# ruc98/Distributed-Data-Parallel-ML-Training

Measured on AMD Instinct MI355X. Metric: images/sec (whole node) VGG-11 CIFAR-10, higher is better.
Workload: dtype bf16; 1 GPU; model=vgg11, global_batch=256, per_gpu_batch=256, parallelism=dp1, hipgraph=True, buckets=1, grad_comm=fp32, comm=inline, optimizer=SGD(lr=0.1, momentum=0.9, wd=1e-4) fused

## Files before the change

### distributed-data-parallel-ml-training_amd/_build.py

```python
import concurrent.futures as cf
import glob
import os
import shutil
import subprocess
import sys
import sysconfig

PKG_DIR = os.path.dirname(os.path.abspath(__file__))
REPO = os.path.dirname(PKG_DIR)
CSRC = os.path.join(PKG_DIR, "csrc")
ARCH = os.environ.get("DDP_AMD_ARCH", "gfx950")
ROCM = os.environ.get("ROCM_PATH", "/opt/rocm")


def _hipcc():
    for c in (os.path.join(ROCM, "bin", "hipcc"), shutil.which("hipcc")):
        if c and os.path.exists(c):
            return c
    raise RuntimeError("hipcc not found (ROCm toolchain required to build ddp_amd)")


def _includes():
    import pybind11
    return ["-I" + CSRC, "-I" + os.path.join(CSRC, "kernels"), "-I" + pybind11.get_include(),
            "-I" + sysconfig.get_paths()["include"], "-I" + os.path.join(ROCM, "include")]


VARIANTS = {"release": ("_native", "native", []),
            "det": ("_native_det", "native_det", ["-DDDP_AMD_DETERMINISTIC"])}


def ext_path(variant="release"):
    suffix = sysconfig.get_config_var("EXT_SUFFIX") or ".so"
    return os.path.join(PKG_DIR, VARIANTS[variant][0] + suffix)


def _newest_header():
    hs = glob.glob(os.path.join(CSRC, "**", "*.h"), recursive=True)
    return max((os.path.getmtime(h) for h in hs), default=0.0)


def _deps(obj):
    d = obj + ".d"
    if not os.path.exists(d):
        return None
    with open(d) as f:
        text = f.read().replace("\\\n", " ")
    parts = text.split(":", 1)
    return [t for t in parts[1].split()] if len(parts) == 2 else None


def _compile(cmd, src, obj, hdr_time, verbose):
    if os.path.exists(obj):
        t = os.path.getmtime(obj)
        deps = _deps(obj)
        newest = (max([os.path.getmtime(x) for x in deps if os.path.exists(x)] + [0.0])
                  if deps is not None else hdr_time)
        if deps is not None and any(not os.path.exists(x) for x in deps):
            newest = hdr_time
        if t >= os.path.getmtime(src) and t >= newest:
            return obj, False
    if verbose:
        print("[ddp_amd build]", os.path.relpath(src, PKG_DIR), flush=True)
    r = subprocess.run(cmd, capture_output=True, text=True)
    if r.returncode != 0:
        raise RuntimeError(f"compile failed: {src}\n{r.stdout}\n{r.stderr}")
    return obj, True


def _sources():
    return (sorted(glob.glob(os.path.join(CSRC, "kernels", "*.hip")))
            + sorted(glob.glob(os.path.join(CSRC, "runtime", "*.cpp"))) + [os.path.join(CSRC, "bind.cpp")])


def up_to_date(variant="release"):
    out = ext_path(variant)
    if not os.path.exists(out):
        return False
    newest = max([_newest_header()] + [os.path.getmtime(s) for s in _sources()])
    return os.path.getmtime(out) >= newest


def build(verbose=True, jobs=None, variants=("release", "det")):
    for v in variants:
        _build_variant(v, verbose, jobs)
    return ext_path()


def _build_variant(variant, verbose=True, jobs=None):
    stem, objdir, defines = VARIANTS[variant]
    BUILD = os.path.join(REPO, "build", objdir)
    if not os.path.isdir(BUILD) and up_to_date(variant):
        return ext_path(variant)
    hipcc = _hipcc()
    os.makedirs(BUILD, exist_ok=True)
    inc = _includes()
    debug = os.environ.get("DDP_AMD_DEBUG_BUILD", "0") == "1"
    common = (["-O1", "-g", "-DDDP_AMD_DEBUG"] if debug else ["-O3"]) + \
        ["-std=c++17", "-fPIC", "-Wno-unused-result"] + defines
    hdr_time = _newest_header()
    tasks = []
    for src in sorted(glob.glob(os.path.join(CSRC, "kernels", "*.hip"))):
        obj = os.path.join(BUILD, os.path.basename(src) + ".o")
        cmd = [hipcc, f"--offload-arch={ARCH}", "-x", "hip", *common, *inc, "-c", src, "-o", obj,
               "-MMD", "-MF", obj + ".d"]
        tasks.append((cmd, src, obj))
    host_srcs = sorted(glob.glob(os.path.join(CSRC, "runtime", "*.cpp"))) + [os.path.join(CSRC, "bind.cpp")]
    for src in host_srcs:
        obj = os.path.join(BUILD, os.path.basename(src) + ".o")
        cmd = [hipcc, "-x", "c++", "-D__HIP_PLATFORM_AMD__", *common, "-fvisibility=hidden", *inc,
               "-c", src, "-o", obj, "-MMD", "-MF", obj + ".d"]
        tasks.append((cmd, src, obj))
    jobs = jobs or min(8, os.cpu_count() or 4)
    changed = False
    with cf.ThreadPoolExecutor(max_workers=jobs) as ex:
        futs = [ex.submit(_compile, c, s, o, hdr_time, verbose) for c, s, o in tasks]
        objs = []
        for f in futs:
            o, ch = f.result()
            objs.append(o)
            changed |= ch
    out = ext_path(variant)
    if changed or not os.path.exists(out) or os.path.getmtime(out) < max(os.path.getmtime(o) for o in objs):
        tmp = out + ".tmp"
        cmd = [hipcc, f"--offload-arch={ARCH}", "-shared", "-fPIC", *objs, "-o", tmp,
               "-L" + os.path.join(ROCM, "lib"), "-lrccl", "-lamdhip64"]
        r = subprocess.run(cmd, capture_output=True, text=True)
        if r.returncode != 0:
            raise RuntimeError(f"link failed\n{r.stdout}\n{r.stderr}")
        os.replace(tmp, out)
        if verbose:
            print("[ddp_amd build] linked", os.path.relpath(out, REPO), flush=True)
    return out


if __name__ == "__main__":
    build(verbose=True)
    sys.exit(0)
```

### distributed-data-parallel-ml-training_amd/csrc/bind.cpp

```cpp
#include <hip/hip_runtime.h>
#include <pybind11/pybind11.h>
#include <pybind11/stl.h>

#include <stdexcept>
#include <string>
#include <tuple>
#include <vector>

#include "runtime/comm.h"

namespace py = pybind11;
using ddp_amd::BucketSpec;
using ddp_amd::RcclComm;
using ddp_amd::Reducer;

#include "kernels/api.h"

template <typename T>
static T* P(uintptr_t v) { return reinterpret_cast<T*>(v); }
static hipStream_t S(uintptr_t v) { return reinterpret_cast<hipStream_t>(v); }
static void check(int rc, const char* what) {
  if (rc != 0) {
    std::string msg = std::string(what) + " failed: ";
    msg += (rc > 0) ? hipGetErrorString((hipError_t)rc) : "invalid arguments";
// ... 307 lines not shown
    a.running_mean = P<float>(running_mean); a.running_var = P<float>(running_var);
    a.momentum = momentum; a.use_running = use_running;
    if (rcoef) {
      ddp_amd::BnArgs r{};
      r.C = C; r.eps = reps; r.momentum = rmomentum;
      r.stats = P<float>(rstats); r.gamma = P<float>(rgamma); r.beta = P<float>(rbeta);
      r.coef = P<float>(rcoef);
      r.running_mean = P<float>(rrunning_mean); r.running_var = P<float>(rrunning_var);
      a.rcoef = r.coef;
      check(ddp_bn_act_fwd_res(&a, &r, S(st)), "bn_act_fwd (shortcut BN)");
      return;
    }
    check(ddp_bn_act_fwd(&a, S(st)), "bn_act_fwd");
  }, py::arg("N"), py::arg("H"), py::arg("W"), py::arg("C"), py::arg("pool"), py::arg("relu"),
     py::arg("eps"), py::arg("z"), py::arg("res"), py::arg("stats"), py::arg("gamma"),
     py::arg("beta"), py::arg("out"), py::arg("stream"), py::arg("running_mean") = 0,
     py::arg("running_var") = 0, py::arg("momentum") = 0.1f, py::arg("use_running") = 0,
     py::arg("coef") = 0, py::arg("mask") = 0, py::arg("rstats") = 0, py::arg("rgamma") = 0,
     py::arg("rbeta") = 0, py::arg("rcoef") = 0, py::arg("rrunning_mean") = 0,
     py::arg("rrunning_var") = 0, py::arg("reps") = 1e-5f, py::arg("rmomentum") = 0.1f);
  m.def("maxpool_fwd", [](uintptr_t x, int N, int H, int W, int C, int KH, int KW, int stride,
                          int pad, int Ho, int Wo, uintptr_t y, uintptr_t idx, uintptr_t st) {
    check(ddp_maxpool_fwd(P<void>(x), N, H, W, C, KH, KW, stride, pad, Ho, Wo, P<void>(y),
                          P<void>(idx), S(st)), "maxpool_fwd");
  });
  m.def("maxpool_bwd", [](uintptr_t dy, uintptr_t idx, int N, int H, int W, int C, int KH, int KW,
                          int stride, int pad, int Ho, int Wo, uintptr_t dx, uintptr_t st) {
    check(ddp_maxpool_bwd(P<void>(dy), P<void>(idx), N, H, W, C, KH, KW, stride, pad, Ho, Wo,
                          P<void>(dx), S(st)), "maxpool_bwd");
  });
  m.def("avgpool_fwd", [](uintptr_t x, int N, int HW, int C, uintptr_t y, uintptr_t st) {
    check(ddp_avgpool_fwd(P<void>(x), N, HW, C, P<void>(y), S(st)), "avgpool_fwd");
  });
  m.def("avgpool_bwd", [](uintptr_t dy, int N, int HW, int C, uintptr_t dx, uintptr_t st) {
    check(ddp_avgpool_bwd(P<void>(dy), N, HW, C, P<void>(dx), S(st)), "avgpool_bwd");
  });
  m.def("colsum", [](uintptr_t dl, int B, int J, uintptr_t db, uintptr_t st) {
    check(ddp_colsum(P<void>(dl), B, J, P<float>(db), S(st)), "colsum");
  });
  m.def("bn_act_bwd", [](int N, int H, int W, int C, int pool, int relu, float eps, uintptr_t z,
                         uintptr_t res, uintptr_t stats, uintptr_t gamma, uintptr_t beta,
                         uintptr_t dout, uintptr_t sums, uintptr_t dz, uintptr_t dres,
                         uintptr_t dgamma, uintptr_t dbeta, uintptr_t dbias, uintptr_t st,
                         uintptr_t coef, int sums_ready, uintptr_t mask, uintptr_t rcoef,
                         uintptr_t rsums, uintptr_t rdz, uintptr_t rdgamma, uintptr_t rdbeta) {
    ddp_amd::BnArgs a{};
    a.coef = P<float>(coef);
    a.sums_ready = sums_ready;
    a.mask = P<unsigned char>(mask);
    a.N = N; a.H = H; a.W = W; a.C = C; a.pool = pool; a.relu = relu; a.eps = eps;
    a.z = P<unsigned short>(z); a.res = P<unsigned short>(res); a.stats = P<float>(stats);
    a.gamma = P<float>(gamma); a.beta = P<float>(beta); a.dout = P<unsigned short>(dout);
    a.sums = P<float>(sums); a.dz = P<unsigned short>(dz); a.dres = P<unsigned short>(dres);
    a.dgamma = P<float>(dgamma); a.dbeta = P<float>(dbeta); a.dbias = P<float>(dbias);
    if (rcoef) {
      a.rcoef = P<float>(rcoef); a.rsums = P<float>(rsums); a.rdz = P<unsigned short>(rdz);
      a.rdgamma = P<float>(rdgamma); a.rdbeta = P<float>(rdbeta);
      check(ddp_bn_act_bwd_res(&a, S(st)), "bn_act_bwd (shortcut BN)");
      return;
    }
    check(ddp_bn_act_bwd(&a, S(st)), "bn_act_bwd");
  }, py::arg("N"), py::arg("H"), py::arg("W"), py::arg("C"), py::arg("pool"), py::arg("relu"),
     py::arg("eps"), py::arg("z"), py::arg("res"), py::arg("stats"), py::arg("gamma"),
     py::arg("beta"), py::arg("dout"), py::arg("sums"), py::arg("dz"), py::arg("dres"),
     py::arg("dgamma"), py::arg("dbeta"), py::arg("dbias"), py::arg("stream"), py::arg("coef"),
     py::arg("sums_ready") = 0, py::arg("mask") = 0, py::arg("rcoef") = 0, py::arg("rsums") = 0,
     py::arg("rdz") = 0, py::arg("rdgamma") = 0, py::arg("rdbeta") = 0);
  m.def("bn_pool3_fwd", [](int N, int H, int W, int C, int relu, float eps, uintptr_t z,
                           uintptr_t stats, uintptr_t gamma, uintptr_t beta, uintptr_t out,
                           uintptr_t idx, uintptr_t st, uintptr_t running_mean,
                           uintptr_t running_var, float momentum, int use_running, uintptr_t coef) {
    ddp_amd::BnArgs a{};
    a.N = N; a.H = H; a.W = W; a.C = C; a.relu = relu; a.eps = eps;
    a.z = P<unsigned short>(z); a.stats = P<float>(stats); a.gamma = P<float>(gamma);
    a.beta = P<float>(beta); a.out = P<unsigned short>(out); a.coef = P<float>(coef);
    a.running_mean = P<float>(running_mean); a.running_var = P<float>(running_var);
    a.momentum = momentum; a.use_running = use_running;
    check(ddp_bn_pool3_fwd(&a, P<unsigned char>(idx), S(st)), "bn_pool3_fwd");
  });
  m.def("bn_pool3_bwd", [](int N, int H, int W, int C, int relu, float eps, uintptr_t z,
                           uintptr_t dout, uintptr_t idx, uintptr_t sums, uintptr_t dz,
                           uintptr_t dgamma, uintptr_t dbeta, uintptr_t st, uintptr_t coef) {
    ddp_amd::BnArgs a{};
    a.N = N; a.H = H; a.W = W; a.C = C; a.relu = relu; a.eps = eps;
    a.z = P<unsigned short>(z); a.dout = P<unsigned short>(dout); a.sums = P<float>(sums);
    a.dz = P<unsigned short>(dz); a.dgamma = P<float>(dgamma); a.dbeta = P<float>(dbeta);
    a.coef = P<float>(coef);
    check(ddp_bn_pool3_bwd(&a, P<unsigned char>(idx), S(st)), "bn_pool3_bwd");
  });
  m.def("bn_bwd_local_ok", [](int N, int H, int W, int C, int pool) {
    return ddp_bn_bwd_local_ok(N, H, W, C, pool) != 0;
  });
  m.def("bn_bwd_local_set", [](long long max_loads) { ddp_bn_bwd_local_set(max_loads); });
  m.def("conv_epi_stage_set", [](int on) { ddp_conv_epi_stage_set(on); });

  m.def("linear_ce_fwd", [](uintptr_t x, uintptr_t W, uintptr_t b, uintptr_t labels, int B, int F,
                            int J, uintptr_t logits, uintptr_t dlogits, uintptr_t loss_sum,
                            uintptr_t correct, uintptr_t st, uintptr_t loss_acc) {
    check(ddp_linear_ce_fwd(P<void>(x), P<float>(W), P<float>(b), P<long long>(labels), B, F, J,
                            P<float>(logits), P<float>(dlogits), P<float>(loss_sum),
                            P<int>(correct), P<float>(loss_acc), S(st)), "linear_ce_fwd");
  }, py::arg("x"), py::arg("W"), py::arg("b"), py::arg("labels"), py::arg("B"), py::arg("F"),
     py::arg("J"), py::arg("logits"), py::arg("dlogits"), py::arg("loss_sum"), py::arg("correct"),
     py::arg("stream"), py::arg("loss_acc") = 0);
  m.def("bn_pool_linear_ce_fwd", [](uintptr_t z, uintptr_t stats, uintptr_t gamma, uintptr_t beta,
                                    float eps, int relu, uintptr_t coef, uintptr_t y, uintptr_t W,
                                    uintptr_t b, uintptr_t labels, int B, int F, int J,
                                    uintptr_t dlogits, uintptr_t loss_sum, uintptr_t st,
                                    uintptr_t loss_acc) {
    ddp_amd::HeadBnIn h{P<unsigned short>(z), P<float>(stats), P<float>(gamma), P<float>(beta),
                        eps, relu, P<float>(coef), P<unsigned short>(y)};
    check(ddp_bn_pool_linear_ce_fwd(&h, P<float>(W), P<float>(b), P<long long>(labels), B, F, J,
                                    P<float>(dlogits), P<float>(loss_sum), nullptr,
                                    P<float>(loss_acc), S(st)), "bn_pool_linear_ce_fwd");
  }, py::arg("z"), py::arg("stats"), py::arg("gamma"), py::arg("beta"), py::arg("eps"),
     py::arg("relu"), py::arg("coef"), py::arg("y"), py::arg("W"), py::arg("b"), py::arg("labels"),
     py::arg("B"), py::arg("F"), py::arg("J"), py::arg("dlogits"), py::arg("loss_sum"),
     py::arg("stream"), py::arg("loss_acc") = 0);
  m.def("linear_bwd", [](uintptr_t dlogits, uintptr_t x, uintptr_t W, int B, int F, int J,
                         uintptr_t gscale, uintptr_t dx, uintptr_t dW, uintptr_t db,
                         uintptr_t st) {
    check(ddp_linear_bwd(P<float>(dlogits), P<void>(x), P<float>(W), B, F, J, P<float>(gscale),
                         P<void>(dx), P<float>(dW), P<float>(db), S(st)), "linear_bwd");
  });
  m.def("softmax_ce", [](uintptr_t logits, int bf16, uintptr_t labels, int B, int J,
                         uintptr_t loss_sum, uintptr_t correct, uintptr_t dlogits,
                         int dlogits_bf16, uintptr_t st) {
    check(ddp_softmax_ce(P<void>(logits), bf16, P<long long>(labels), B, J, P<float>(loss_sum),
                         P<int>(correct), P<void>(dlogits), dlogits_bf16, S(st)), "softmax_ce");
  });

  m.def("sgd", [](uintptr_t p, uintptr_t g, uintptr_t buf, size_t n, float lr, float momentum,
                  float wd, float grad_scale, int nesterov, uintptr_t st, uintptr_t sched) {
    check(ddp_sgd(P<float>(p), P<float>(g), P<float>(buf), n, lr, momentum, wd, grad_scale,
                  nesterov, P<const ddp_amd::LrSched>(sched), S(st)), "sgd");
  }, py::arg("p"), py::arg("g"), py::arg("buf"), py::arg("n"), py::arg("lr"), py::arg("momentum"),
     py::arg("wd"), py::arg("grad_scale"), py::arg("nesterov"), py::arg("stream"),
     py::arg("sched") = 0);
  m.def("conv_options", [](int stages) { ddp_conv_options(stages); }, py::arg("stages") = 2);
  m.def("conv_tune_set", [](int mode, int M, int N, int K, int tile, int splits, int stages) {
    ddp_conv_tune_set(mode, M, N, K, tile, splits, stages);
  }, py::arg("mode"), py::arg("M"), py::arg("N"), py::arg("K"), py::arg("tile"),
     py::arg("splits"), py::arg("stages") = 0);
  m.def("conv_tune_clear", []() { ddp_conv_tune_clear(); });
  m.def("conv_wgrad_pm_set", [](int on) { ddp_conv_wgrad_pm_set(on); });
  m.def("conv_rows_pm_set", [](int on) { ddp_conv_rows_pm_set(on); });
  m.def("bn_fold_bwd_mb", [](int mb) { ddp_bn_fold_bwd_mb(mb); });
  m.def("bn_fold_grid", [](int blocks) { ddp_bn_fold_grid(blocks); });
  m.def("conv_pair_tune_set", [](int M, int N, int K, int hw, int tile, int sd, int sw) {
    ddp_conv_pair_tune_set(M, N, K, hw, tile, sd, sw);
  });
  m.def("conv_force_tile", [](int t, int stages) { ddp_conv_force_tile(t, stages); },
        py::arg("tile_plus_one"), py::arg("stages") = 0);
  m.def("pack_conv_weights", [](std::vector<std::tuple<uintptr_t, uintptr_t, uintptr_t, int, int,
                                                       int, int, int, int>> descs, uintptr_t st) {
    std::vector<ddp_amd::PackDesc> d;
    for (auto& t : descs) {
      ddp_amd::PackDesc x;
      x.p = P<float>(std::get<0>(t));
      x.wc = P<unsigned short>(std::get<1>(t));
      x.wt = P<unsigned short>(std::get<2>(t));
      x.K = std::get<3>(t); x.Cr = std::get<4>(t); x.C = std::get<5>(t);
      x.R = std::get<6>(t); x.S = std::get<7>(t);
      x.krsc = std::get<8>(t);
      d.push_back(x);
    }
    check(ddp_pack_conv_weights(d.data(), (int)d.size(), S(st)), "pack_conv_weights");
  });
  m.def("sgd_pack", [](uintptr_t items, int n_items, uintptr_t descs, uintptr_t p, uintptr_t g,
                       uintptr_t buf, float lr, float momentum, float wd, float grad_scale,
                       int nesterov, uintptr_t st, int zero_grad, uintptr_t counter, int delta,
                       uintptr_t skip, uintptr_t shadow, uintptr_t slot, uintptr_t done,
                       uintptr_t signal, uintptr_t sched, int sched_advance, uintptr_t lars_side,
                       uintptr_t lars_tensors, uintptr_t lars_partial, uintptr_t lars_trust,
                       float lars_eta, float lars_eps) {
    check(ddp_sgd_pack(P<void>(items), n_items, P<long long>(descs), P<float>(p), P<float>(g),
                       P<float>(buf), lr, momentum, wd, grad_scale, nesterov, zero_grad,
                       P<int>(counter), delta, P<const unsigned>(skip), P<unsigned short>(shadow),
                       P<float>(slot), P<unsigned>(done), P<unsigned>(signal),
                       P<ddp_amd::LrSched>(sched), sched_advance, P<void>(lars_side),
                       P<void>(lars_tensors), P<void>(lars_partial), P<float>(lars_trust),
                       lars_eta, lars_eps, S(st)),
          "sgd_pack");
  }, py::arg("items"), py::arg("n_items"), py::arg("descs"), py::arg("p"), py::arg("g"),
     py::arg("buf"), py::arg("lr"), py::arg("momentum"), py::arg("wd"), py::arg("grad_scale"),
     py::arg("nesterov"), py::arg("stream"), py::arg("zero_grad") = 0, py::arg("counter") = 0,
     py::arg("delta") = 0, py::arg("skip") = 0, py::arg("shadow") = 0, py::arg("slot") = 0,
     py::arg("done") = 0, py::arg("signal") = 0, py::arg("sched") = 0,
     py::arg("sched_advance") = 0, py::arg("lars_side") = 0, py::arg("lars_tensors") = 0,
     py::arg("lars_partial") = 0, py::arg("lars_trust") = 0, py::arg("lars_eta") = 0.f,
     py::arg("lars_eps") = 0.f);
  m.def("lars_norms", [](uintptr_t items, int n_items, uintptr_t p, uintptr_t g, float grad_scale,
                         uintptr_t partial, uintptr_t st) {
    check(ddp_lars_norms(P<void>(items), n_items, P<float>(p), P<float>(g), grad_scale,
                         P<void>(partial), S(st)), "lars_norms");
  }, py::arg("items"), py::arg("n_items"), py::arg("p"), py::arg("g"), py::arg("grad_scale"),
     py::arg("partial"), py::arg("stream"));
  m.def("shard_tail", [](uintptr_t segs, int n_segs, uintptr_t src, uintptr_t dst,
                         std::vector<std::tuple<uintptr_t, uintptr_t, uintptr_t, int, int, int,
                                                int, int, int>> descs,
                         uintptr_t done, uintptr_t signal, uintptr_t skip, uintptr_t st) {
    std::vector<ddp_amd::PackDesc> d;
    for (auto& t : descs) {
      ddp_amd::PackDesc x;
      x.p = P<float>(std::get<0>(t));
      x.wc = P<unsigned short>(std::get<1>(t));
      x.wt = P<unsigned short>(std::get<2>(t));
      x.K = std::get<3>(t); x.Cr = std::get<4>(t); x.C = std::get<5>(t);
      x.R = std::get<6>(t); x.S = std::get<7>(t);
      x.krsc = std::get<8>(t);
      d.push_back(x);
    }
    check(ddp_shard_tail(P<void>(segs), n_segs, P<float>(src), P<float>(dst), d.data(),
                         (int)d.size(), P<unsigned>(done), P<unsigned>(signal),
                         P<const unsigned>(skip), S(st)), "shard_tail");
  });
  m.def("seg_copy_f32", [](uintptr_t table, int n, uintptr_t src, uintptr_t dst, uintptr_t st) {
    check(ddp_seg_copy_f32(P<void>(table), n, P<float>(src), P<float>(dst), S(st)), "seg_copy_f32");
  });
  m.def("sgd_tile_dims", [](int RS) {
    int tk, tc;
    ddp_sgd_tile_dims(RS, &tk, &tc);
    return std::make_pair(tk, tc);
  });
  m.def("counter_add", [](uintptr_t c, int delta, uintptr_t st, uintptr_t sched, int sched_mode) {
    check(ddp_counter_add(P<int>(c), delta, P<ddp_amd::LrSched>(sched), sched_mode, S(st)),
          "counter_add");
  }, py::arg("c"), py::arg("delta"), py::arg("stream"), py::arg("sched") = 0,
     py::arg("sched_mode") = 0);

  m.def("synth_generate", [](uintptr_t images, uintptr_t labels, int n, int pix_per_img,
                             unsigned int seed, int classes, uintptr_t st) {
    check(ddp_synth_generate(P<unsigned char>(images), P<int>(labels), n, pix_per_img, seed,
                             classes, S(st)), "synth_generate");
  });
  m.def("augment", [](uintptr_t images, uintptr_t labels, uintptr_t indices, uintptr_t cursor,
                      int L, int B, int H, int W, int Cp, int pad, int flip, unsigned int seed,
                      unsigned int epoch, std::vector<float> mean, std::vector<float> std_,
                      uintptr_t x, uintptr_t y, uintptr_t st, uintptr_t zero, size_t zero_n,
                      uintptr_t sched) {
    ddp_amd::AugArgs a{};
    a.sched = P<ddp_amd::LrSched>(sched);
    a.zero = P<float>(zero);
    a.zero_n = zero ? zero_n : 0;
    a.images = P<unsigned char>(images); a.labels = P<int>(labels); a.indices = P<int>(indices);
    a.cursor = P<int>(cursor); a.L = L; a.B = B; a.H = H; a.W = W; a.Cp = Cp; a.pad = pad;
    a.flip = flip; a.seed = seed; a.epoch = epoch;
    for (int c = 0; c < 3; ++c) { a.mean[c] = mean.at(c); a.inv_std[c] = 1.f / std_.at(c); }
    a.x = P<unsigned short>(x); a.y = P<long long>(y);
    check(ddp_augment(&a, S(st)), "augment");
  }, py::arg("images"), py::arg("labels"), py::arg("indices"), py::arg("cursor"), py::arg("L"),
     py::arg("B"), py::arg("H"), py::arg("W"), py::arg("Cp"), py::arg("pad"), py::arg("flip"),
     py::arg("seed"), py::arg("epoch"), py::arg("mean"), py::arg("std"), py::arg("x"),
     py::arg("y"), py::arg("stream"), py::arg("zero") = 0, py::arg("zero_n") = 0,
     py::arg("sched") = 0);
  m.def("nchw_to_nhwc", [](uintptr_t x, int N, int C, int H, int W, int Cp, uintptr_t out,
                           uintptr_t st) {
    check(ddp_nchw_to_nhwc(P<float>(x), N, C, H, W, Cp, P<void>(out), S(st)), "nchw_to_nhwc");
  });
  m.def("mean_ws", [](uintptr_t in, size_t n, int ws, uintptr_t out, uintptr_t st) {
    check(ddp_mean_ws(P<float>(in), n, ws, P<float>(out), S(st)), "mean_ws");
  });
  m.def("comm_standin", [](uintptr_t x, size_t n, int blocks, float usec, float scale, uintptr_t st,
                           int passes) {
    check(ddp_comm_standin(P<float>(x), n, blocks, usec, scale, passes, S(st)), "comm_standin");
  }, py::arg("x"), py::arg("n"), py::arg("blocks"), py::arg("usec"), py::arg("scale"),
     py::arg("stream"), py::arg("passes") = 1);
  m.def("flag_signal", [](uintptr_t flag, uintptr_t st) {
    check(ddp_flag_signal(P<unsigned>(flag), S(st)), "flag_signal");
  });
  m.def("flag_wait", [](uintptr_t flag, uintptr_t expected, uintptr_t err, float timeout_s,
                        uintptr_t st) {
    check(ddp_flag_wait(P<unsigned>(flag), P<unsigned>(expected), P<unsigned>(err), timeout_s,
                        S(st)),
          "flag_wait");
  });
  m.def("pack_bf16", [](uintptr_t x, size_t n, uintptr_t y, uintptr_t st) {
    check(ddp_pack_bf16(P<float>(x), n, P<unsigned short>(y), S(st)), "pack_bf16");
  });
  m.def("unpack_bf16", [](uintptr_t y, size_t n, uintptr_t x, uintptr_t st) {
    check(ddp_unpack_bf16(P<unsigned short>(y), n, P<float>(x), S(st)), "unpack_bf16");
  });
  m.def("memset_async", [](uintptr_t p, int value, size_t n, uintptr_t st) {
    check((int)hipMemsetAsync(P<void>(p), value, n, S(st)), "hipMemsetAsync");
  });
  m.def("memcpy_async", [](uintptr_t dst, uintptr_t src, size_t n, uintptr_t st) {
    check((int)hipMemcpyAsync(P<void>(dst), P<void>(src), n, hipMemcpyDeviceToDevice, S(st)),
          "hipMemcpyAsync");
  });
  m.def("copy_bytes", [](uintptr_t dst, uintptr_t src, size_t n, uintptr_t st) {
    check(ddp_copy_bytes(P<void>(dst), P<void>(src), n, S(st)), "copy_bytes");
  });
  m.def("fill_bytes", [](uintptr_t dst, int value, size_t n, uintptr_t st) {
    check(ddp_fill_bytes(P<void>(dst), value, n, S(st)), "fill_bytes");
  });
  m.def("scale", [](uintptr_t x, size_t n, float s, uintptr_t st) {
    check(ddp_scale(P<float>(x), n, s, S(st)), "scale");
  });

  m.def("plan_buckets", [](std::vector<size_t> offsets, std::vector<size_t> numels,
                           size_t elem_bytes, size_t cap, size_t cap_first) {
    auto b = ddp_amd::plan_buckets(offsets, numels, elem_bytes, cap, cap_first);
    std::vector<std::tuple<int, int, size_t, size_t>> out;
    for (auto& x : b) out.emplace_back(x.first_param, x.last_param, x.offset, x.count);
    return out;
  });
// ... 103 lines not shown
```

### distributed-data-parallel-ml-training_amd/csrc/kernels/api.h

```cpp
#pragma once
#include <hip/hip_runtime.h>
#include <stddef.h>
#include <stdint.h>

namespace ddp_amd {

#ifdef DDP_AMD_DETERMINISTIC
constexpr int kStatRep = 4096;
constexpr bool kDeterministic = true;
#else
constexpr int kStatRep = 16;
constexpr bool kDeterministic = false;
#endif

struct ConvGeom {
  int N, H, W, C;
  int K;
  int R, S, stride, pad;
  int P, Q;
  int Creal;
  int wkrsc;
};

struct BnArgs {
// ... 72 lines not shown
  const float* beta;
  float eps;
  int relu;
  float* coef;
  unsigned short* y;
};

struct LrSched {
  unsigned step;
  unsigned n;
  unsigned next;
  unsigned pad;
};

struct SgdFuse {
  float* p;
  float* buf;
  unsigned short* wc;
  float lr, momentum, wd, grad_scale;
  int nesterov;
  const LrSched* sched;
};

struct L0Io {
  const void* x;
  const void* wc;
  const float* bias;
  float eps;
  int relu;
  float* stats;
  const float* gamma;
  const float* beta;
  float* coef;
  void* y;
  const void* dy;
  float* sums;
  void* dz;
  void* code;
  void* zw;
  float* dgamma;
  float* dbeta;
  int sums_ready;
  float* dw;
  float* ws;
  size_t ws_elems;
};

struct PackDesc {
  const float* p;
  unsigned short* wc;
  unsigned short* wt;
  int K, Cr, C, R, S;
  int krsc;
};

struct AugArgs {
  const unsigned char* images;
  const int* labels;
  const int* indices;
  const int* cursor;
  int L, B, H, W, Cp, pad, flip;
  uint32_t seed, epoch;
  float mean[3], inv_std[3];
  unsigned short* x;
  long long* y;
  float* zero;
  size_t zero_n;
  LrSched* sched;
};

}

extern "C" {
int ddp_conv_fwd(const ddp_amd::ConvGeom* g, const void* x, const void* wc, const float* bias,
                 void* y, float* stats, float* ws, size_t ws_elems, int splits, hipStream_t st);
int ddp_conv_fwd_bn(const ddp_amd::ConvGeom* g, const void* x, const void* wc, const float* bias,
                    void* z, float* stats, float* ws, size_t ws_elems, const ddp_amd::BnFwdFuse* bn,
                    hipStream_t st);
int ddp_conv_fwd_finish(const ddp_amd::ConvGeom* g, float* ws, int splits, const float* bias,
                        void* z, float* stats, const ddp_amd::BnFwdFuse* bn, int* bn_done,
                        hipStream_t st);
int ddp_conv_fwd_tr(const ddp_amd::ConvGeom* g, const void* x, const void* wc, const float* bias,
                    void* z, float* stats, float* ws, size_t ws_elems,
                    const ddp_amd::BnFwdFuse* bn, int* bn_done, const ddp_amd::TrFwdIn* in,
                    hipStream_t st);
int ddp_conv_tr_would_serve(const ddp_amd::ConvGeom* g, size_t ws_elems, int in_mode);
void ddp_conv_tr_set(int mode, int M, int K, int C, int H, int bm, int bn, int splits, int stages);
int ddp_conv_tr_geometry(int BM, int N, int H, int W, int* out7);
int ddp_linear_head_bwd_bn(const float* dl, const float* W, const void* x, int B, int F, int J,
                           const float* gscale, const ddp_amd::BnBwdFuse* bn,
                           const ddp_amd::BnBwdApply* ba, float* dW, float* db, hipStream_t st);
void ddp_conv_bn_fuse_rows(int rows);
int ddp_conv_dgrad(const ddp_amd::ConvGeom* g, const void* dy, const void* wt, void* dx,
                   float* ws, size_t ws_elems, int splits, int accumulate, hipStream_t st);
int ddp_conv_dgrad_acc(const ddp_amd::ConvGeom* g, const void* dy, const void* wt, void* dx,
                       float* ws, size_t ws_elems, int splits, const void* acc_dy,
                       const unsigned char* acc_mask, hipStream_t st);
int ddp_conv_dgrad_bn(const ddp_amd::ConvGeom* g, const void* dy, const void* wt, void* dx,
                      float* ws, size_t ws_elems, int splits, const ddp_amd::BnBwdFuse* bn,
                      const ddp_amd::BnBwdApply* ba, int* bn_done, hipStream_t st);
int ddp_conv_wgrad(const ddp_amd::ConvGeom* g, const void* dy, const void* x, float* dw,
                   float* ws, size_t ws_elems, int splits, hipStream_t st);
int ddp_bn_act_fwd(const ddp_amd::BnArgs* a, hipStream_t st);
int ddp_bn_act_bwd(const ddp_amd::BnArgs* a, hipStream_t st);
int ddp_bn_act_fwd_res(const ddp_amd::BnArgs* a, const ddp_amd::BnArgs* r, hipStream_t st);
int ddp_bn_act_bwd_res(const ddp_amd::BnArgs* a, hipStream_t st);
int ddp_bn_bwd_local_ok(int N, int H, int W, int C, int pool);
void ddp_bn_bwd_local_set(long long max_loads);
int ddp_bn_pool_linear_ce_fwd(const ddp_amd::HeadBnIn* bn, const float* W, const float* b,
                              const long long* labels, int B, int F, int J, float* dlogits,
                              float* loss_sum, int* correct, float* loss_acc, hipStream_t st);
int ddp_linear_ce_fwd(const void* x, const float* W, const float* b, const long long* labels,
                      int B, int F, int J, float* logits, float* dlogits, float* loss_sum,
                      int* correct, float* loss_acc, hipStream_t st);
int ddp_linear_bwd(const float* dlogits, const void* x, const float* W, int B, int F, int J,
                   const float* gscale, void* dx, float* dW, float* db, hipStream_t st);
int ddp_softmax_ce(const void* logits, int logits_bf16, const long long* labels, int B, int J,
                   float* loss_sum, int* correct, void* dlogits, int dlogits_bf16,
                   hipStream_t st);
int ddp_sgd(float* p, const float* g, float* buf, size_t n, float lr, float momentum, float wd,
            float grad_scale, int nesterov, const ddp_amd::LrSched* sched, hipStream_t st);
int ddp_conv_fwd_smallk(const ddp_amd::ConvGeom* g, const void* x, const void* wc,
                        const float* bias, void* y, float* stats, hipStream_t st);
void ddp_conv_options(int stages);
void ddp_conv_epi_stage_set(int on);
int ddp_bn_pool3_fwd(const ddp_amd::BnArgs* a, unsigned char* idx, hipStream_t st);
int ddp_bn_pool3_bwd(const ddp_amd::BnArgs* a, const unsigned char* idx, hipStream_t st);
void ddp_conv_pair_mode(int mode, int items);
void ddp_sgd_fuse_register(float* dw, const ddp_amd::SgdFuse* f, int clear);
void ddp_sgd_fuse_begin();
int ddp_l0_ok(const ddp_amd::ConvGeom* g);
int ddp_l0_fwd(const ddp_amd::ConvGeom* g, const ddp_amd::L0Io* io, hipStream_t st);
int ddp_l0_bwd(const ddp_amd::ConvGeom* g, const ddp_amd::L0Io* io, hipStream_t st);
int ddp_conv_wgrad_final(const ddp_amd::ConvGeom* g, const void* dy, const void* x, float* dw,
                         float* ws, size_t ws_elems, int splits, hipStream_t st);
int ddp_sgd_fuse_taken(uintptr_t* out, int cap);
int ddp_sgd_fuse_take_final(const float* dw, ddp_amd::SgdFuse* out);
int ddp_sgd_fuse_taken_master(uintptr_t* out, int cap);
void ddp_conv_pair_force(int splits_dg, int splits_wg, int tile);
int ddp_conv_bwd_pair(const ddp_amd::ConvGeom* g, const void* dy, const void* wc, void* dx,
                      const void* x, float* dw, float* ws, size_t ws_elems,
                      const ddp_amd::BnBwdFuse* bn, const ddp_amd::BnBwdApply* ba, int* bn_done,
                      hipStream_t st);
void ddp_conv_tune_set(int mode, int M, int N, int K, int tile, int splits, int stages);
void ddp_conv_pair_tune_set(int M, int N, int K, int hw, int tile, int sd, int sw);
void ddp_conv_wgrad_pm_set(int on);
void ddp_conv_rows_pm_set(int on);
void ddp_bn_fold_bwd_mb(int mb);
void ddp_bn_fold_grid(int blocks);
int ddp_conv_dense2x2_ok(const ddp_amd::ConvGeom* g);
void ddp_conv_dense2x2_set(int on);
void ddp_conv_tune_clear();
void ddp_conv_force_tile(int tile_plus_one, int stages);
int ddp_pack_conv_weights(const ddp_amd::PackDesc* descs, int n, hipStream_t st);
int ddp_sgd_pack(const void* items, int n_items, const long long* descs, float* p, float* g,
                 float* buf, float lr, float momentum, float wd, float grad_scale, int nesterov,
                 int zero_grad, int* counter, int delta, const unsigned* skip,
                 unsigned short* shadow, float* slot, unsigned* done, unsigned* signal,
                 ddp_amd::LrSched* sched, int sched_advance, const void* lars_side,
                 const void* lars_tensors, const void* lars_partial, float* lars_trust,
                 float lars_eta, float lars_eps, hipStream_t st);
int ddp_lars_norms(const void* items, int n_items, const float* p, const float* g,
                   float grad_scale, void* partial, hipStream_t st);
int ddp_shard_tail(const void* segs, int n_segs, const float* src, float* dst,
                   const ddp_amd::PackDesc* pack, int n_pack, unsigned* done, unsigned* signal,
                   const unsigned* skip, hipStream_t st);
void ddp_sgd_tile_dims(int RS, int* TK, int* TC);
int ddp_counter_add(int* c, int delta, ddp_amd::LrSched* sched, int sched_mode, hipStream_t st);
int ddp_synth_generate(unsigned char* images, int* labels, int n, int pix_per_img,
                       unsigned int seed, int classes, hipStream_t st);
int ddp_augment(const ddp_amd::AugArgs* a, hipStream_t st);
int ddp_nchw_to_nhwc(const float* x, int N, int C, int H, int W, int Cp, void* out,
                     hipStream_t st);
int ddp_maxpool_fwd(const void* x, int N, int H, int W, int C, int KH, int KW, int stride,
                    int pad, int Ho, int Wo, void* y, void* idx, hipStream_t st);
int ddp_maxpool_bwd(const void* dy, const void* idx, int N, int H, int W, int C, int KH, int KW,
                    int stride, int pad, int Ho, int Wo, void* dx, hipStream_t st);
int ddp_avgpool_fwd(const void* x, int N, int HW, int C, void* y, hipStream_t st);
int ddp_avgpool_bwd(const void* dy, int N, int HW, int C, void* dx, hipStream_t st);
int ddp_colsum(const void* dl, int B, int J, float* db, hipStream_t st);
int ddp_mean_ws(const float* in, size_t n, int ws, float* out, hipStream_t st);
int ddp_scale(float* x, size_t n, float s, hipStream_t st);
int ddp_copy_bytes(void* dst, const void* src, size_t n, hipStream_t st);
int ddp_fill_bytes(void* dst, int value, size_t n, hipStream_t st);
int ddp_comm_standin(float* x, size_t n, int blocks, float usec, float scale, int passes,
                     hipStream_t st);
int ddp_flag_signal(unsigned* flag, hipStream_t st);
int ddp_flag_wait(const unsigned* flag, unsigned* expected, unsigned* err, float timeout_s,
                  hipStream_t st);
int ddp_pack_bf16(const float* x, size_t n, unsigned short* y, hipStream_t st);
int ddp_seg_copy_f32(const void* table, int n, const float* src, float* dst, hipStream_t st);
int ddp_unpack_bf16(const unsigned short* y, size_t n, float* x, hipStream_t st);
}
```

### distributed-data-parallel-ml-training_amd/csrc/kernels/common.h

```cpp
#pragma once
#include <hip/hip_runtime.h>
#include <stdint.h>
#include <cstdlib>

#include "api.h"

namespace ddp_amd {

typedef __bf16 bf16x8 __attribute__((ext_vector_type(8)));
typedef float f32x4 __attribute__((ext_vector_type(4)));
typedef float f32x16 __attribute__((ext_vector_type(16)));
typedef unsigned short u16x8 __attribute__((ext_vector_type(8)));

constexpr int kWave = 64;

#ifdef DDP_AMD_DEBUG
#define DDP_DEVICE_CHECK(cond)                                                              \
  do {                                                                                      \
    if (!(cond)) {                                                                          \
      printf("[ddp_amd debug] %s:%d check failed: %s (block %d thread %d)\n", __FILE__,     \
             __LINE__, #cond, (int)blockIdx.x, (int)threadIdx.x);                           \
      return;                                                                               \
    }                                                                                       \
  } while (0)
#else
#define DDP_DEVICE_CHECK(cond) \
  do {                        \
  } while (0)
#endif

__device__ __forceinline__ int stat_rep(int b) {
#ifdef DDP_AMD_DETERMINISTIC
  return b < kStatRep ? b : 0;
#else
  return b % kStatRep;
#endif
}
__device__ __forceinline__ float stat_val(float v, int b) {
#ifdef DDP_AMD_DETERMINISTIC
  return b < kStatRep ? v : __builtin_nanf("");
#else
  (void)b;
  return v;
#endif
}

__device__ __forceinline__ float sgd_update1(float p, float g, float& b, float lr, float momentum,
                                             float wd, float grad_scale, int nesterov) {
  float d = __builtin_fmaf(wd, p, g * grad_scale);
  if (momentum != 0.f) {
    b = __builtin_fmaf(momentum, b, d);
    d = nesterov ? __builtin_fmaf(momentum, b, d) : b;
  }
  return __builtin_fmaf(-lr, d, p);
}

__device__ __forceinline__ float sched_lr(const LrSched* s) {
  const unsigned k = __hip_atomic_load(&s->step, __ATOMIC_RELAXED, __HIP_MEMORY_SCOPE_AGENT);
  const unsigned n = s->n;
  return reinterpret_cast<const float*>(s + 1)[k < n ? k : n - 1];
}
__device__ __forceinline__ float sched_lr_block(const LrSched* s, float lr) {
  if (!s) return lr;
  __shared__ float s_lr;
  if (threadIdx.x == 0) s_lr = sched_lr(s);
  __syncthreads();
  return s_lr;
}

__device__ __forceinline__ float bf2f(unsigned short h) {
  return __uint_as_float(((unsigned int)h) << 16);
}
__device__ __forceinline__ unsigned short f2bf(float f) {
  __bf16 b = (__bf16)f;
  return __builtin_bit_cast(unsigned short, b);
}
__device__ __forceinline__ float round_bf(float f) { return bf2f(f2bf(f)); }

__device__ __forceinline__ u16x8 ld8(const unsigned short* p) {
  return *reinterpret_cast<const u16x8*>(p);
}
__device__ __forceinline__ void st8(unsigned short* p, u16x8 v) {
  *reinterpret_cast<u16x8*>(p) = v;
}

template <int CTRL>
__device__ __forceinline__ float dpp_f(float v) {
  return __int_as_float(__builtin_amdgcn_update_dpp(0, __float_as_int(v), CTRL, 0xF, 0xF, false));
}
__device__ __forceinline__ float dpp_sum16(float v) {
  v += dpp_f<0xB1>(v);
  v += dpp_f<0x4E>(v);
  v += dpp_f<0x141>(v);
  v += dpp_f<0x140>(v);
  return v;
}
__device__ __forceinline__ float lane_f(float v, int l) {
  return __int_as_float(__builtin_amdgcn_readlane(__float_as_int(v), l));
}
__device__ __forceinline__ float wave_sum(float v) {
  v = dpp_sum16(v);
  return (lane_f(v, 0) + lane_f(v, 16)) + (lane_f(v, 32) + lane_f(v, 48));
}
__device__ __forceinline__ float wave_max(float v) {
  v = fmaxf(v, dpp_f<0xB1>(v));
  v = fmaxf(v, dpp_f<0x4E>(v));
  v = fmaxf(v, dpp_f<0x141>(v));
  v = fmaxf(v, dpp_f<0x140>(v));
  return fmaxf(fmaxf(lane_f(v, 0), lane_f(v, 16)), fmaxf(lane_f(v, 32), lane_f(v, 48)));
}

__device__ __forceinline__ int xcd_remap(int orig, int nwg) {
  const int nx = 8;
  if (nwg < nx) return orig;
  const int q = nwg / nx, r = nwg % nx;
  const int xcd = orig % nx, idx = orig / nx;
  return (xcd < r ? xcd * (q + 1) : r * (q + 1) + (xcd - r) * q) + idx;
}

__host__ __device__ __forceinline__ uint32_t hash_u32(uint32_t x) {
  x ^= x >> 16; x *= 0x7feb352du;
  x ^= x >> 15; x *= 0x846ca68bu;
  x ^= x >> 16;
  return x;
}
__host__ __device__ __forceinline__ uint32_t hash3(uint32_t a, uint32_t b, uint32_t c) {
  return hash_u32(a ^ hash_u32(b ^ hash_u32(c + 0x9e3779b9u)));
}

}
```

### distributed-data-parallel-ml-training_amd/csrc/kernels/conv_igemm.hip

```cpp
#include "common.h"
#include "api.h"
#include "linear_blocks.h"
#include <algorithm>
#include <map>
#include <set>
#include <cstdlib>

namespace ddp_amd {

enum { MODE_FWD = 0, MODE_DGRAD = 1, MODE_WGRAD = 2 };

typedef short v4i16 __attribute__((ext_vector_type(4)));
typedef short short8_t __attribute__((ext_vector_type(8)));
typedef __attribute__((address_space(3))) v4i16 lds_v4i16;

struct FastDiv {
  unsigned mul;
  int sh;
};
__device__ __forceinline__ int fast_div(int x, FastDiv d) {
  return (int)((__umulhi((unsigned)x, d.mul) + (unsigned)x) >> d.sh);
}
__global__ __launch_bounds__(256) void zero16_kernel(uint4* __restrict__ p, size_t n16) {
  for (size_t i = blockIdx.x * 256ull + threadIdx.x; i < n16; i += (size_t)gridDim.x * 256)
    p[i] = (uint4){0u, 0u, 0u, 0u};
}

__device__ __forceinline__ void ld8f_conv(const float* p, float* v) {
  const float4 a = reinterpret_cast<const float4*>(p)[0];
  const float4 b = reinterpret_cast<const float4*>(p)[1];
  v[0] = a.x; v[1] = a.y; v[2] = a.z; v[3] = a.w;
  v[4] = b.x; v[5] = b.y; v[6] = b.z; v[7] = b.w;
}

struct ConvArgs {
  ConvGeom g;
  const unsigned short* a;
  const unsigned short* b;
  unsigned short* out;
  float* dw;
  float* ws;
  const float* bias;
  float* stats;
  int Mg, Ng, Kg;
  int splits;
  int ksteps_per_split;
  int phase;
  int pa, pb, Hp, Wp, r0, s0, Rt, St, qa, qb;
  int accumulate;
  int a_bytes, b_bytes;
  FastDiv dPQ, dQ;
  int has_bnf;
  BnBwdFuse bnf;
  const BnFwdFuse* bnfwd;
  int* bnfwd_done;
  const BnBwdApply* bnapply;
  int* bnapply_done;
  int epi_stage;
  int d2x2;
  int d2C, d2K;
  int no_finish;
  const unsigned short* acc_dy;
  const unsigned char* acc_mask;
  SgdFuse sgd;
  int pixmajor;
};

__device__ __forceinline__ uint2 acc_old4(const unsigned short* dx, const unsigned short* acc_dy,
                                          const unsigned char* acc_mask, size_t e) {
  if (!acc_mask) return *reinterpret_cast<const uint2*>(dx + e);
  uint2 v = *reinterpret_cast<const uint2*>(acc_dy + e);
  const unsigned mb = (unsigned)acc_mask[e >> 3] >> (e & 4);
  v.x &= ((mb & 1u) ? 0xFFFFu : 0u) | ((mb & 2u) ? 0xFFFF0000u : 0u);
  v.y &= ((mb & 4u) ? 0xFFFFu : 0u) | ((mb & 8u) ? 0xFFFF0000u : 0u);
  return v;
}
__device__ __forceinline__ u16x8 acc_old8(const unsigned short* dx, const unsigned short* acc_dy,
                                          const unsigned char* acc_mask, size_t e) {
  if (!acc_mask) return ld8(dx + e);
  u16x8 v = ld8(acc_dy + e);
  const unsigned mb = acc_mask[e >> 3];
#pragma unroll
  for (int i = 0; i < 8; ++i) v[i] = ((mb >> i) & 1u) ? v[i] : (unsigned short)0;
  return v;
}

__device__ __forceinline__ int fdiv(int x, int d, float inv) {
  int q = (int)((float)x * inv);
  const int r = x - q * d;
  q += (r < 0) ? -1 : (r >= d ? 1 : 0);
  return q;
}

struct RowInfo {
  int base;
  int h0, w0;
};

template <int MODE>
__device__ __forceinline__ RowInfo row_info(const ConvArgs& A, int row) {
  const ConvGeom& g = A.g;
  RowInfo ri{0, -(1 << 24), 0};
  if (row >= A.Mg) return ri;
  if (MODE == MODE_FWD) {
    const int pq = g.P * g.Q;
    const int n = fast_div(row, A.dPQ), rem = row - n * pq;
    const int p = fast_div(rem, A.dQ), q = rem - p * g.Q;
    ri.base = n * g.H * g.W * g.C;
    ri.h0 = p * g.stride - g.pad;
    ri.w0 = q * g.stride - g.pad;
  } else if (A.phase) {
    const int hw = A.Hp * A.Wp;
    const int n = fast_div(row, A.dPQ), rem = row - n * hw;
    const int i = fast_div(rem, A.dQ), j = rem - i * A.Wp;
    ri.base = n * g.P * g.Q * g.K;
    ri.h0 = i + A.qa;
    ri.w0 = j + A.qb;
  } else {
    const int hw = g.H * g.W;
    const int n = fast_div(row, A.dPQ), rem = row - n * hw;
    const int h = fast_div(rem, A.dQ), w = rem - h * g.W;
    ri.base = n * g.P * g.Q * g.K;
    ri.h0 = h + g.pad;
    ri.w0 = w + g.pad;
  }
  return ri;
}

struct KInfo {
  int r, s, c;
  bool ok;
};

__device__ __forceinline__ int rk_off(int row, int chunk) {
  return row * 64 + ((chunk ^ ((row >> 1) & 7)) << 3);
}
template <int NCOL>
__device__ __forceinline__ int mc_swz(int m) {
  if (NCOL >= 128) return (((m & 3) | (((m >> 3) & 1) << 2)) << 1) & (NCOL / 8 - 1);
  return ((((m >> 1) & 1) | (((m >> 3) & 1) << 1)) << 1);
}
template <int NCOL>
__device__ __forceinline__ int swz_row_step(int i) {
  return NCOL >= 256 ? ((i & 1) << 3) : 0;
}
template <int NCOL>
__device__ __forceinline__ int mc_off(int m, int col) {
  return m * NCOL + (((col >> 3) ^ mc_swz<NCOL>(m)) << 3) + (col & 7);
}

constexpr unsigned kOOB = 0x80000000u;
__device__ __forceinline__ __amdgpu_buffer_rsrc_t make_rsrc(const void* base, int bytes) {
  return __builtin_amdgcn_make_buffer_rsrc(const_cast<void*>(base), (short)0, bytes, 0x00020000);
}

typedef __attribute__((address_space(3))) void lds_void;

__device__ __forceinline__ void dma_buf(__amdgpu_buffer_rsrc_t rs, int byte_off,
                                        unsigned short* lds_wave_base) {
  __builtin_amdgcn_raw_ptr_buffer_load_lds(rs, (lds_void*)lds_wave_base, 16, byte_off, 0, 0, 0);
}
__device__ __forceinline__ void dma_buf_s(__amdgpu_buffer_rsrc_t rs, int byte_off, int soff,
                                          unsigned short* lds_wave_base) {
  __builtin_amdgcn_raw_ptr_buffer_load_lds(rs, (lds_void*)lds_wave_base, 16, byte_off,
                                           __builtin_amdgcn_readfirstlane(soff), 0, 0);
}

template <int N>
__device__ __forceinline__ void wait_dma_barrier() {
  asm volatile("s_waitcnt vmcnt(%0)\n\ts_barrier" ::"n"(N) : "memory");
}

template <int BM, int BN, int NST>
struct ConvSmem {
  static constexpr int elems = NST * (BM + BN) * 64;
};

template <int MODE, int BM, int BN, int NST, int BNF = 0, bool XSTAT = false, bool SGDM = false>
__device__ __forceinline__ void conv_igemm_body(const ConvArgs& args, unsigned short* smem,
                                                const int bid, const int nblk) {
  constexpr int BK = 64;
  constexpr int WTM = BM / 2, WTN = BN / 2;
  constexpr bool kOldBnf = BNF == 1 || (BNF == 2 && BM == 64 && BN == 64);
  constexpr int TM = WTM / 16, TN = WTN / 16;
  constexpr int CA = BM * BK / 8 / 256;
  constexpr int CB = BN * BK / 8 / 256;
  constexpr int TILE_A = BM * BK, TILE_B = BN * BK;
  constexpr int STAGE = TILE_A + TILE_B;
  static_assert(CA >= 1 && CB >= 1, "tile too small for 256 threads");
  static_assert(NST >= 2 && NST <= 4, "2..4 LDS stages");

  const int tid = threadIdx.x;
  const int lane = tid & 63;
  const int wid = __builtin_amdgcn_readfirstlane(tid >> 6);
  const int wm = wid >> 1, wn = wid & 1;
  DDP_DEVICE_CHECK(blockDim.x == 256 && args.g.C % 8 == 0 && args.g.K % 8 == 0);
  DDP_DEVICE_CHECK(args.splits >= 1 && args.ksteps_per_split >= 1);

  const int tiles_n = (args.Ng + BN - 1) / BN;
  const int tiles_m = (args.Mg + BM - 1) / BM;
  const int tiles = tiles_m * tiles_n;
  const int nitems = tiles * args.splits;
  const int ksteps = (args.Kg + BK - 1) / BK;

  f32x4 acc[TM][TN];
  const ConvGeom& gg = args.g;

  constexpr int NA = (MODE != MODE_WGRAD) ? CA : 1;
  int a_off[CA];
  int a_h0[NA], a_w0[NA];
  int b_off[CB];
  int kr = 0, ks_ = 0, kc = 0;
  KInfo xk;
  int xk_same = 0;
  int wp[CB], wq[CB];
  int w_rr = 0, w_ss = 0, w_lim = 0;
  const bool wsame = MODE == MODE_WGRAD && gg.stride == 1 && gg.P == gg.H && gg.Q == gg.W;
  const int w_dq = wsame ? BK % gg.Q : 0;
  const int w_dp = wsame ? (BK / gg.Q) % gg.P : 0;
  const int w_dm = wsame ? 2 * BK * gg.C : 0;
  const bool pm = MODE == MODE_WGRAD && args.pixmajor;
  const bool pmr = MODE != MODE_WGRAD && args.pixmajor;
  int pmr_pq = 0, pmr_n0 = 0, pmr_row0 = 0, pmr_t = 0;
  unsigned pmr_mask = 0;
  int pm_p = 0, pm_q = 0, pm_qlo = 0, pm_qhi = 0, pm_n0 = 0, pm_r = 0, pm_s = 0;
  int row0 = 0, col0 = 0, zsplit = 0, ks_begin = 0, ks_end = 0, cur_tile = 0;
  int d2pos = 0;
  const bool phase = MODE == MODE_DGRAD && args.phase;
  const int Sdec = phase ? args.St : gg.S;
  const int cdim = MODE == MODE_FWD ? gg.C : gg.K;
  const bool fast = MODE != MODE_WGRAD && (cdim % BK) == 0;
  const int lcA = (MODE != MODE_WGRAD) ? ((tid & 7) ^ ((tid >> 4) & 7))
                                       : ((tid % (BM / 8)) ^ mc_swz<BM>(tid / (BM / 8)));
  constexpr bool BKM = MODE != MODE_FWD;
  const int lcB = !BKM ? lcA : ((tid % (BN / 8)) ^ mc_swz<BN>(tid / (BN / 8)));
  const __amdgpu_buffer_rsrc_t rsA = make_rsrc(args.a, args.a_bytes);
  const __amdgpu_buffer_rsrc_t rsB = make_rsrc(args.b, args.b_bytes);

  auto setup = [&](int item) {
    zsplit = item / tiles;
    const int tile = xcd_remap(item - zsplit * tiles, tiles);
    cur_tile = tile;
    const int tm = tile / tiles_n;
    const int tn = tile - tm * tiles_n;
    row0 = tm * BM;
    col0 = tn * BN;
    ks_begin = zsplit * args.ksteps_per_split;
    ks_end = min(ksteps, ks_begin + args.ksteps_per_split);
    if (MODE != MODE_WGRAD) {
      if (pmr) {
        pmr_pq = row0 / gg.N;
        pmr_n0 = row0 - pmr_pq * gg.N;
        pmr_row0 = row0;
        const int img = MODE == MODE_FWD ? gg.H * gg.W * gg.C : gg.P * gg.Q * gg.K;
#pragma unroll
        for (int i = 0; i < CA; ++i) a_off[i] = 2 * (((tid >> 3) + 32 * i) * img + lcA * 8);
      } else {
#pragma unroll
        for (int i = 0; i < CA; ++i) {
          const RowInfo ri = row_info<MODE>(args, row0 + (tid >> 3) + 32 * i);
          a_h0[i] = ri.h0;
          a_w0[i] = ri.w0;
          const int e = (MODE == MODE_FWD) ? ri.base + (ri.h0 * gg.W + ri.w0) * gg.C
                                           : ri.base + (ri.h0 * gg.Q + ri.w0) * gg.K;
          a_off[i] = 2 * (e + (fast ? lcA * 8 : 0));
        }
      }
      if (MODE == MODE_FWD && args.d2x2) {
        d2pos = col0 / args.d2K;
#pragma unroll
        for (int i = 0; i < CB; ++i) {
          const int col = col0 + (tid >> 3) + 32 * i;
          b_off[i] = col < args.Ng ? 2 * ((col - d2pos * args.d2K) * 9 * args.d2C + lcB * 8)
                                   : (int)kOOB;
        }
      } else if (MODE == MODE_FWD) {
#pragma unroll
        for (int i = 0; i < CB; ++i) {
          const int col = col0 + (tid >> 3) + 32 * i;
          b_off[i] = col < args.Ng ? 2 * (col * args.Kg + lcB * 8) : (int)kOOB;
        }
      } else if (args.d2x2) {
        d2pos = col0 / args.d2C;
#pragma unroll
        for (int i = 0; i < CB; ++i) {
          const int col = col0 + (lcB ^ swz_row_step<BN>(i)) * 8;
          b_off[i] = col < args.Ng ? 2 * (((tid + i * 256) / (BN / 8)) * 9 * args.d2C + col -
                                          d2pos * args.d2C)
                                   : (int)kOOB;
        }
      } else {
#pragma unroll
        for (int i = 0; i < CB; ++i) {
          const int col = col0 + (lcB ^ swz_row_step<BN>(i)) * 8;
          b_off[i] = col < args.Ng ? 2 * (((tid + i * 256) / (BN / 8)) * gg.R * gg.S * gg.C + col)
                                   : (int)kOOB;
        }
      }
      if (pmr) {
        const int pp = pmr_pq / gg.Q, qq = pmr_pq - pp * gg.Q, kb = cdim / BK;
        unsigned m = 0;
        for (int r = 0; r < gg.R; ++r)
          for (int s2 = 0; s2 < gg.S; ++s2) {
            const bool ok = MODE == MODE_FWD
                ? (unsigned)(pp + r - gg.pad) < (unsigned)gg.H && (unsigned)(qq + s2 - gg.pad) < (unsigned)gg.W
                : (unsigned)(pp - r + gg.pad) < (unsigned)gg.P && (unsigned)(qq - s2 + gg.pad) < (unsigned)gg.Q;
            if (ok) m |= 1u << (r * gg.S + s2);
          }
        pmr_mask = m;
        const int V = __builtin_popcount(m) * kb;
        const int per = (V + args.splits - 1) / args.splits;
        ks_begin = min(V, zsplit * per);
        ks_end = min(V, ks_begin + per);
        int jv = ks_begin / kb;
        unsigned mm = m;
        for (; jv > 0 && mm; --jv) mm &= mm - 1;
        pmr_t = mm ? __builtin_ctz(mm) : 0;
        kc = (ks_begin - (ks_begin / kb) * kb) * BK;
        kr = pmr_t / gg.S;
        ks_ = pmr_t - kr * gg.S;
      } else {
        const int kk = ks_begin * BK + (fast ? 0 : lcA * 8);
        const int rs = kk / cdim;
        kc = kk - rs * cdim;
        kr = rs / Sdec;
        ks_ = rs - kr * Sdec;
      }
    } else {
      constexpr int NCA = BM / 8;
#pragma unroll
      for (int i = 0; i < CA; ++i) {
        const int kout = row0 + (lcA ^ swz_row_step<BM>(i)) * 8;
        a_off[i] = kout < args.Mg ? 2 * (((tid + i * 256) / NCA) * gg.K + kout) : (int)kOOB;
      }
      const int j = col0 + lcB * 8;
      const int rs = j / gg.C;
      xk.c = j - rs * gg.C;
      xk.r = rs / gg.S;
      xk.s = rs - xk.r * gg.S;
      xk.ok = j < args.Ng;
      if (pm) {
        const int t = col0 / gg.C;
        pm_r = t / gg.S;
        pm_s = t - pm_r * gg.S;
        const int PQ = gg.P * gg.Q, nb = gg.N / BK;
        const int p_lo = max(0, gg.pad - pm_r), p_hi = min(gg.P, gg.H + gg.pad - pm_r);
        pm_qlo = max(0, gg.pad - pm_s);
        pm_qhi = min(gg.Q, gg.W + gg.pad - pm_s);
        const int nq = max(0, pm_qhi - pm_qlo);
        const int V = max(0, p_hi - p_lo) * nq * nb;
        const int per = (V + args.splits - 1) / args.splits;
        ks_begin = min(V, zsplit * per);
        ks_end = min(V, ks_begin + per);
        const int jv = ks_begin / nb;
        pm_p = p_lo + (nq ? jv / nq : 0);
        pm_q = pm_qlo + (nq ? jv - (jv / nq) * nq : 0);
        pm_n0 = (ks_begin - jv * nb) * BK;
        constexpr int NCA = BM / 8;
        constexpr int NCB = BN / 8;
#pragma unroll
        for (int i = 0; i < CA; ++i) {
          const int kout = row0 + (lcA ^ swz_row_step<BM>(i)) * 8;
          a_off[i] = kout < args.Mg ? 2 * (((tid + i * 256) / NCA) * PQ * gg.K + kout) : (int)kOOB;
        }
#pragma unroll
        for (int i = 0; i < CB; ++i)
          b_off[i] = 2 * (((tid + i * 256) / NCB) * gg.H * gg.W * gg.C + (j - t * gg.C));
      }
      if (!xk.ok) xk.r = -(1 << 20);
      xk_same = xk.ok ? 2 * (((xk.r - gg.pad) * gg.W + (xk.s - gg.pad)) * gg.C + xk.c) : 0;
      if (wsame && !pm) {
        constexpr int NCB = BN / 8;
        const int pq = gg.P * gg.Q;
        w_rr = xk.r - gg.pad;
        w_ss = xk.s - gg.pad;
        w_lim = args.Kg * (2 * gg.C) + xk_same;
#pragma unroll
        for (int i = 0; i < CB; ++i) {
          const int m = ks_begin * BK + (tid + i * 256) / NCB;
          const int rem = m % pq;
          wp[i] = rem / gg.Q;
          wq[i] = rem - wp[i] * gg.Q;
          b_off[i] = m * (2 * gg.C) + xk_same;
        }
      }
    }
  };

  auto issue = [&](int ks, int buf) {
    unsigned short* As = smem + buf * STAGE;
    unsigned short* Bs = As + TILE_A;
    const int k0 = ks * BK;
    if (MODE != MODE_WGRAD && pmr) {
      const int pp = pmr_pq / gg.Q, qq = pmr_pq - pp * gg.Q;
      const int hh = MODE == MODE_FWD ? pp + kr - gg.pad : pp - kr + gg.pad;
      const int ww = MODE == MODE_FWD ? qq + ks_ - gg.pad : qq - ks_ + gg.pad;
      const int sa = MODE == MODE_FWD ? 2 * (((pmr_n0 * gg.H + hh) * gg.W + ww) * cdim + kc)
                                      : 2 * (((pmr_n0 * gg.P + hh) * gg.Q + ww) * cdim + kc);
#pragma unroll
      for (int i = 0; i < CA; ++i) dma_buf_s(rsA, a_off[i], sa, As + (wid * 64 + 256 * i) * 8);
      const int boff = MODE == MODE_FWD ? 2 * (pmr_t * cdim + kc)
                                        : 2 * ((kc * gg.R * gg.S + kr * gg.S + ks_) * gg.C);
#pragma unroll
      for (int i = 0; i < CB; ++i) dma_buf(rsB, b_off[i] + boff, Bs + (wid * 64 + 256 * i) * 8);
      kc += BK;
      if (kc == cdim) {
        kc = 0;
        const unsigned rest = pmr_mask & ~((2u << pmr_t) - 1u);
        pmr_t = rest ? __builtin_ctz(rest) : pmr_t;
        kr = pmr_t / gg.S;
        ks_ = pmr_t - kr * gg.S;
      }
    } else if (MODE != MODE_WGRAD) {
      const int W_ = MODE == MODE_FWD ? gg.W : gg.Q;
      if (fast) {
        const int tap = 2 * (MODE == MODE_FWD ? (kr * W_ + ks_) * cdim + kc : kc - (kr * W_ + ks_) * cdim);
#pragma unroll
        for (int i = 0; i < CA; ++i) {
          bool ok;
          if (MODE == MODE_FWD)
            ok = (unsigned)(a_h0[i] + kr) < (unsigned)gg.H && (unsigned)(a_w0[i] + ks_) < (unsigned)gg.W;
          else
            ok = (unsigned)(a_h0[i] - kr) < (unsigned)gg.P && (unsigned)(a_w0[i] - ks_) < (unsigned)gg.Q;
          dma_buf(rsA, ok ? a_off[i] + tap : (int)kOOB, As + (wid * 64 + 256 * i) * 8);
        }
        int boff;
        if (args.d2x2) {
          const int pix = MODE == MODE_FWD ? kc / args.d2C : kc / args.d2K;
          const int ch = kc - pix * (MODE == MODE_FWD ? args.d2C : args.d2K);
          const int pq = MODE == MODE_FWD ? d2pos : pix, hw = MODE == MODE_FWD ? pix : d2pos;
          const int tap = ((hw >> 1) - (pq >> 1) + 1) * 3 + ((hw & 1) - (pq & 1) + 1);
          boff = MODE == MODE_FWD ? 2 * (tap * args.d2C + ch) : 2 * ((ch * 9 + tap) * args.d2C);
        } else if (MODE == MODE_FWD) {
          boff = 2 * k0;
        } else {
          const int rr = phase ? args.r0 + gg.stride * kr : kr, ss = phase ? args.s0 + gg.stride * ks_ : ks_;
          boff = 2 * ((kc * gg.R * gg.S + rr * gg.S + ss) * gg.C);
        }
#pragma unroll
        for (int i = 0; i < CB; ++i) dma_buf(rsB, b_off[i] + boff, Bs + (wid * 64 + 256 * i) * 8);
        kc += BK;
        if (kc == cdim) {
          kc = 0;
          if (++ks_ == Sdec) { ks_ = 0; ++kr; }
        }
      } else {
        const int kk = k0 + lcA * 8;
        const bool kok = kk < args.Kg;
        const int tap = 2 * (MODE == MODE_FWD ? (kr * W_ + ks_) * cdim + kc : kc - (kr * W_ + ks_) * cdim);
#pragma unroll
        for (int i = 0; i < CA; ++i) {
          bool ok;
          if (MODE == MODE_FWD)
            ok = (unsigned)(a_h0[i] + kr) < (unsigned)gg.H && (unsigned)(a_w0[i] + ks_) < (unsigned)gg.W;
          else
            ok = (unsigned)(a_h0[i] - kr) < (unsigned)gg.P && (unsigned)(a_w0[i] - ks_) < (unsigned)gg.Q;
          dma_buf(rsA, (kok && ok) ? a_off[i] + tap : (int)kOOB, As + (wid * 64 + 256 * i) * 8);
        }
        if (MODE == MODE_FWD) {
#pragma unroll
          for (int i = 0; i < CB; ++i)
            dma_buf(rsB, kok ? b_off[i] + 2 * k0 : (int)kOOB, Bs + (wid * 64 + 256 * i) * 8);
        } else {
          const int RSC = gg.R * gg.S * gg.C;
#pragma unroll
          for (int i = 0; i < CB; ++i) {
            const int m = (tid + i * 256) / (BN / 8);
            const int kkr = k0 + m;
            const int tap = kkr / gg.K, kout = kkr - tap * gg.K;
            const int tr = tap / Sdec, ts = tap - tr * Sdec;
            const int rr = phase ? args.r0 + gg.stride * tr : tr, ss = phase ? args.s0 + gg.stride * ts : ts;
            const int off = b_off[i] - 2 * m * RSC + 2 * ((kout * gg.R * gg.S + rr * gg.S + ss) * gg.C);
            dma_buf(rsB, (kkr < args.Kg && b_off[i] != (int)kOOB) ? off : (int)kOOB,
                    Bs + (wid * 64 + 256 * i) * 8);
          }
        }
        kc += BK;
        while (kc >= cdim) {
          kc -= cdim;
          if (++ks_ == Sdec) { ks_ = 0; ++kr; }
        }
      }
    } else {
      constexpr int NCB = BN / 8;
      if (pm) {
        const int PQ = gg.P * gg.Q;
        const int sa = 2 * ((pm_n0 * PQ + pm_p * gg.Q + pm_q) * gg.K);
        const int sb = 2 * ((pm_n0 * gg.H + pm_p + pm_r - gg.pad) * gg.W + pm_q + pm_s - gg.pad) * gg.C;
#pragma unroll
        for (int i = 0; i < CA; ++i) dma_buf_s(rsA, a_off[i], sa, As + (wid * 64 + 256 * i) * 8);
#pragma unroll
        for (int i = 0; i < CB; ++i) dma_buf_s(rsB, b_off[i], sb, Bs + (wid * 64 + 256 * i) * 8);
        pm_n0 += BK;
        if (pm_n0 == gg.N) {
          pm_n0 = 0;
          if (++pm_q == pm_qhi) {
            pm_q = pm_qlo;
            ++pm_p;
          }
        }
        return;
      }
      const int ka = 2 * k0 * gg.K;
#pragma unroll
      for (int i = 0; i < CA; ++i)
        dma_buf(rsA, a_off[i] + ka, As + (wid * 64 + 256 * i) * 8);
      if (wsame) {
#pragma unroll
        for (int i = 0; i < CB; ++i) {
          const bool ok = b_off[i] < w_lim && (unsigned)(wp[i] + w_rr) < (unsigned)gg.H &&
                          (unsigned)(wq[i] + w_ss) < (unsigned)gg.W;
          dma_buf(rsB, ok ? b_off[i] : (int)kOOB, Bs + (wid * 64 + 256 * i) * 8);
          b_off[i] += w_dm;
          int q = wq[i] + w_dq;
          const int cq = q >= gg.Q ? 1 : 0;
          q -= cq ? gg.Q : 0;
          int pp = wp[i] + w_dp + cq;
          pp -= pp >= gg.P ? gg.P : 0;
          wq[i] = q;
          wp[i] = pp;
        }
      } else {
#pragma unroll
        for (int i = 0; i < CB; ++i) {
          const int m = k0 + (tid + i * 256) / NCB;
          const int n = fast_div(m, args.dPQ);
          const int rem = m - n * (gg.P * gg.Q);
          const int p = fast_div(rem, args.dQ);
          const int q = rem - p * gg.Q;
          const int h = p * gg.stride - gg.pad + xk.r, w = q * gg.stride - gg.pad + xk.s;
          const bool ok = m < args.Kg && (unsigned)h < (unsigned)gg.H && (unsigned)w < (unsigned)gg.W;
          dma_buf(rsB, ok ? 2 * (((n * gg.H + h) * gg.W + w) * gg.C + xk.c) : (int)kOOB,
                  Bs + (wid * 64 + 256 * i) * 8);
        }
      }
    }
  };

  int fa_off[TM], fb_off[TN];
  {
    const int g = lane >> 4, q = (lane >> 2) & 3, p = lane & 3;
    const int m0 = 8 * g + q;
#pragma unroll
    for (int i = 0; i < TM; ++i)
      fa_off[i] = MODE != MODE_WGRAD ? rk_off(wm * WTM + i * 16 + (lane & 15), lane >> 4)
                                     : mc_off<BM>(m0, wm * WTM + i * 16 + 4 * p);
#pragma unroll
    for (int j = 0; j < TN; ++j)
      fb_off[j] = !BKM ? rk_off(wn * WTN + j * 16 + (lane & 15), lane >> 4)
                       : mc_off<BN>(m0, wn * WTN + j * 16 + 4 * p);
  }

  auto load_frags = [&](int buf, int kk, bf16x8 (&fa)[TM], bf16x8 (&fb)[TN]) {
    const unsigned short* As = smem + buf * STAGE;
    const unsigned short* Bs = As + TILE_A;
    if (MODE != MODE_WGRAD) {
#pragma unroll
      for (int i = 0; i < TM; ++i)
        fa[i] = *reinterpret_cast<const bf16x8*>(As + (fa_off[i] ^ (kk ? 32 : 0)));
    } else {
#pragma unroll
      for (int i = 0; i < TM; ++i) {
        const unsigned short* base = As + fa_off[i] + kk * BM;
        v4i16 lo = __builtin_amdgcn_ds_read_tr16_b64_v4i16((lds_v4i16*)base);
        v4i16 hi = __builtin_amdgcn_ds_read_tr16_b64_v4i16((lds_v4i16*)(base + 4 * BM));
        const short8_t v = __builtin_shufflevector(lo, hi, 0, 1, 2, 3, 4, 5, 6, 7);
        fa[i] = __builtin_bit_cast(bf16x8, v);
      }
    }
    if (!BKM) {
#pragma unroll
      for (int j = 0; j < TN; ++j)
        fb[j] = *reinterpret_cast<const bf16x8*>(Bs + (fb_off[j] ^ (kk ? 32 : 0)));
    } else {
#pragma unroll
      for (int j = 0; j < TN; ++j) {
        const unsigned short* base = Bs + fb_off[j] + kk * BN;
        v4i16 lo = __builtin_amdgcn_ds_read_tr16_b64_v4i16((lds_v4i16*)base);
        v4i16 hi = __builtin_amdgcn_ds_read_tr16_b64_v4i16((lds_v4i16*)(base + 4 * BN));
        const short8_t v = __builtin_shufflevector(lo, hi, 0, 1, 2, 3, 4, 5, 6, 7);
        fb[j] = __builtin_bit_cast(bf16x8, v);
      }
    }
  };
  auto mma = [&](const bf16x8 (&fa)[TM], const bf16x8 (&fb)[TN]) {
#pragma unroll
    for (int i = 0; i < TM; ++i)
#pragma unroll
      for (int j = 0; j < TN; ++j)
        acc[i][j] = __builtin_amdgcn_mfma_f32_16x16x32_bf16(fb[j], fa[i], acc[i][j], 0, 0, 0);
  };

  constexpr int SCPR = BN / 8;
  float run_s[XSTAT ? 8 : 1], run_ss[XSTAT ? 8 : 1];
#pragma unroll
  for (int e = 0; e < (XSTAT ? 8 : 1); ++e) { run_s[e] = 0.f; run_ss[e] = 0.f; }
  int run_col = -1;
  auto flush_stats = [&](const int c0, float (&fs)[8], float (&fss)[8]) {
#pragma unroll
    for (int m = SCPR; m < 64; m *= 2)
#pragma unroll
      for (int e = 0; e < 8; ++e) {
        fs[e] += __shfl_xor(fs[e], m);
        fss[e] += __shfl_xor(fss[e], m);
      }
    __syncthreads();
    float* sl = reinterpret_cast<float*>(smem);
    if (lane < SCPR) {
#pragma unroll
      for (int e = 0; e < 8; ++e) {
        sl[(wid * 2 + 0) * BN + lane * 8 + e] = fs[e];
        sl[(wid * 2 + 1) * BN + lane * 8 + e] = fss[e];
      }
    }
    __syncthreads();
    float* st = args.stats + stat_rep(bid) * 2 * args.Ng;
    for (int k = tid; k < 2 * BN; k += 256) {
      const int which = k / BN, cl = k - which * BN;
      if (c0 + cl >= args.Ng) continue;
      const float t = sl[(0 * 2 + which) * BN + cl] + sl[(1 * 2 + which) * BN + cl] +
                      sl[(2 * 2 + which) * BN + cl] + sl[(3 * 2 + which) * BN + cl];
      atomicAdd(st + which * args.Ng + c0 + cl, stat_val(t, bid));
    }
// ... 66 lines not shown
        }
        unsigned short* dst = args.out + orow * args.Ng + col;
        u16x8 o;
        if (MODE == MODE_DGRAD && args.accumulate) {
          const u16x8 old = acc_old8(args.out, args.acc_dy, args.acc_mask, orow * args.Ng + col);
#pragma unroll
          for (int e = 0; e < 8; ++e) o[e] = f2bf(v[e] + bf2f(old[e]));
        } else {
#pragma unroll
          for (int e = 0; e < 8; ++e) o[e] = f2bf(v[e] + bv[e]);
        }
        st8(dst, o);
        if (MODE == MODE_FWD && red) {
#pragma unroll
          for (int e = 0; e < 8; ++e) {
            const float rv = bf2f(o[e]);
            if constexpr (XSTAT) {
              run_s[e] += rv;
              run_ss[e] += rv * rv;
            } else {
              s[e] += rv;
              ss[e] += rv * rv;
            }
          }
        }
      }
    }
    if (!XSTAT && MODE == MODE_FWD && red) flush_stats(col0, s, ss);
    return;
  }
  if (red) __syncthreads();
  if (MODE != MODE_WGRAD && !(BM == 64 && BN == 64) && !split &&
      !(MODE == MODE_DGRAD && args.accumulate) && BNF == 2) {
    const int cbase = col0 + wn * WTN + cq;
    const bool has_bias = MODE == MODE_FWD && args.bias != nullptr;
    int ro[TM];
#pragma unroll
    for (int i = 0; i < TM; ++i) {
      const int row = row0 + wm * WTM + i * 16 + rl;
      int orow = row;
      if (phase) {
        const int hw = args.Hp * args.Wp;
        const int n = fast_div(row, args.dPQ), rem = row - n * hw;
        const int pi = fast_div(rem, args.dQ), pj = rem - pi * args.Wp;
        orow = (n * g.H + args.pa + g.stride * pi) * g.W + args.pb + g.stride * pj;
      } else if (pmr) {
        orow = (pmr_n0 + row - pmr_row0) * (g.P * g.Q) + pmr_pq;
      }
      ro[i] = row < args.Mg ? orow * args.Ng + cbase : -1;
    }
    float* sl = reinterpret_cast<float*>(smem);
#pragma unroll
    for (int j = 0; j < TN; ++j) {
      if (cbase + j * 16 >= args.Ng) continue;
      float4 bj = {0.f, 0.f, 0.f, 0.f};
      if (has_bias) bj = *reinterpret_cast<const float4*>(args.bias + cbase + j * 16);
      float s[4] = {0.f, 0.f, 0.f, 0.f}, ss[4] = {0.f, 0.f, 0.f, 0.f};
      float4 bsc = {0.f, 0.f, 0.f, 0.f}, bsh = bsc, bmu = bsc, bis = bsc;
      if (MODE == MODE_DGRAD && BNF == 2 && red) {
        const float* cf = args.bnf.coef + cbase + j * 16;
        bsc = *reinterpret_cast<const float4*>(cf + 0 * args.Ng);
        bsh = *reinterpret_cast<const float4*>(cf + 1 * args.Ng);
        bmu = *reinterpret_cast<const float4*>(cf + 2 * args.Ng);
        bis = *reinterpret_cast<const float4*>(cf + 3 * args.Ng);
      }
#pragma unroll
      for (int i = 0; i < TM; ++i) {
        if (ro[i] < 0) continue;
        const f32x4 v = acc[i][j];
        uint2 pk;
        pk.x = (unsigned)f2bf(v[0] + bj.x) | ((unsigned)f2bf(v[1] + bj.y) << 16);
        pk.y = (unsigned)f2bf(v[2] + bj.z) | ((unsigned)f2bf(v[3] + bj.w) << 16);
        *reinterpret_cast<uint2*>(args.out + ro[i] + j * 16) = pk;
        if (MODE == MODE_FWD && red) {
          const float r0 = __uint_as_float(pk.x << 16), r1 = __uint_as_float(pk.x & 0xffff0000u);
          const float r2 = __uint_as_float(pk.y << 16), r3 = __uint_as_float(pk.y & 0xffff0000u);
          s[0] += r0; s[1] += r1; s[2] += r2; s[3] += r3;
          ss[0] += r0 * r0; ss[1] += r1 * r1; ss[2] += r2 * r2; ss[3] += r3 * r3;
        }
        if (MODE == MODE_DGRAD && BNF == 2 && red) {
          const uint2 zz = *reinterpret_cast<const uint2*>(args.bnf.z + ro[i] + j * 16);
          const float gv[4] = {__uint_as_float(pk.x << 16), __uint_as_float(pk.x & 0xffff0000u),
                               __uint_as_float(pk.y << 16), __uint_as_float(pk.y & 0xffff0000u)};
          const float zf[4] = {__uint_as_float(zz.x << 16), __uint_as_float(zz.x & 0xffff0000u),
                               __uint_as_float(zz.y << 16), __uint_as_float(zz.y & 0xffff0000u)};
          const float fsc[4] = {bsc.x, bsc.y, bsc.z, bsc.w}, fsh[4] = {bsh.x, bsh.y, bsh.z, bsh.w};
          const float fmu[4] = {bmu.x, bmu.y, bmu.z, bmu.w}, fis[4] = {bis.x, bis.y, bis.z, bis.w};
#pragma unroll
          for (int t = 0; t < 4; ++t) {
            const float y = zf[t] * fsc[t] + fsh[t];
            const float dyb = (args.bnf.relu && !(y > 0.f)) ? 0.f : gv[t];
            s[t] += dyb;
            ss[t] += dyb * ((zf[t] - fmu[t]) * fis[t]);
          }
        }
      }
      if (red) {
#pragma unroll
        for (int t = 0; t < 4; ++t) {
          s[t] = dpp_sum16(s[t]);
          ss[t] = dpp_sum16(ss[t]);
        }
        float* slot = sl + ((((wm * 2 + wn) * TN + j) * 4 + (lane >> 4)) * 8);
        if (rl == 0) {
#pragma unroll
          for (int t = 0; t < 4; ++t) {
            slot[t] = s[t];
            slot[4 + t] = ss[t];
          }
        }
      }
    }
    if (red) {
      __syncthreads();
      if (wm == 0 && rl == 0) {
        float* st = (MODE == MODE_FWD ? args.stats : args.bnf.sums) +
                    stat_rep(bid) * 2 * args.Ng;
#pragma unroll
        for (int j = 0; j < TN; ++j) {
          const int col = cbase + j * 16;
          if (col >= args.Ng) continue;
          const float* s0 = sl + (((wn * TN + j) * 4 + (lane >> 4)) * 8);
          const float* s1 = sl + ((((2 + wn) * TN + j) * 4 + (lane >> 4)) * 8);
#pragma unroll
          for (int t = 0; t < 4; ++t) {
            atomicAdd(st + col + t, stat_val(s0[t] + s1[t], bid));
            atomicAdd(st + args.Ng + col + t, stat_val(s0[4 + t] + s1[4 + t], bid));
          }
        }
      }
    }
    return;
  }
  float sgd_lr = 0.f;
  if (SGDM && MODE == MODE_WGRAD) sgd_lr = args.sgd.sched ? sched_lr(args.sgd.sched) : args.sgd.lr;
#pragma unroll
  for (int j = 0; j < TN; ++j) {
    const int col = col0 + wn * WTN + j * 16 + cq;
    const bool cok = col < args.Ng;
    float4 bias = {0.f, 0.f, 0.f, 0.f};
    if (MODE == MODE_FWD && !split && args.bias && cok)
      bias = (float4){args.bias[col], args.bias[col + 1], args.bias[col + 2], args.bias[col + 3]};
    float s[4] = {0.f, 0.f, 0.f, 0.f}, ss[4] = {0.f, 0.f, 0.f, 0.f};
    float4 bsc = {0.f, 0.f, 0.f, 0.f}, bsh = bsc, bmu = bsc, bis = bsc;
    if (MODE == MODE_DGRAD && kOldBnf && red && cok) {
      const float* cf = args.bnf.coef;
      bsc = *reinterpret_cast<const float4*>(cf + 0 * args.Ng + col);
      bsh = *reinterpret_cast<const float4*>(cf + 1 * args.Ng + col);
      bmu = *reinterpret_cast<const float4*>(cf + 2 * args.Ng + col);
      bis = *reinterpret_cast<const float4*>(cf + 3 * args.Ng + col);
    }
    int wrs = 0, wc = 0;
    if (MODE == MODE_WGRAD) {
      wrs = col / g.C;
      wc = col - wrs * g.C;
    }
#pragma unroll
    for (int i = 0; i < TM; ++i) {
      const int row = row0 + wm * WTM + i * 16 + rl;
      if (!cok || row >= args.Mg) continue;
      const f32x4 v = acc[i][j];
      if (MODE == MODE_WGRAD && !split) {
        if (SGDM && g.wkrsc && g.Creal == g.C && args.sgd.p) {
          const size_t e = ((size_t)row * g.R * g.S + wrs) * g.C + wc;
          float4 pv = *reinterpret_cast<const float4*>(args.sgd.p + e);
          float4 bv = *reinterpret_cast<const float4*>(args.sgd.buf + e);
          const SgdFuse& h = args.sgd;
          pv.x = sgd_update1(pv.x, v[0], bv.x, sgd_lr, h.momentum, h.wd, h.grad_scale, h.nesterov);
          pv.y = sgd_update1(pv.y, v[1], bv.y, sgd_lr, h.momentum, h.wd, h.grad_scale, h.nesterov);
          pv.z = sgd_update1(pv.z, v[2], bv.z, sgd_lr, h.momentum, h.wd, h.grad_scale, h.nesterov);
          pv.w = sgd_update1(pv.w, v[3], bv.w, sgd_lr, h.momentum, h.wd, h.grad_scale, h.nesterov);
          *reinterpret_cast<float4*>(args.sgd.p + e) = pv;
          *reinterpret_cast<float4*>(args.sgd.buf + e) = bv;
        } else if (g.wkrsc && g.Creal == g.C) {
          float* d = args.dw + ((size_t)row * g.R * g.S + wrs) * g.C + wc;
          float4 o = *reinterpret_cast<float4*>(d);
          o.x += v[0]; o.y += v[1]; o.z += v[2]; o.w += v[3];
          *reinterpret_cast<float4*>(d) = o;
        } else {
#pragma unroll
          for (int t = 0; t < 4; ++t) {
            if (wc + t >= g.Creal) break;
            const size_t di = g.wkrsc ? ((size_t)row * g.R * g.S + wrs) * g.Creal + wc + t
                                      : ((size_t)row * g.Creal + wc + t) * g.R * g.S + wrs;
            args.dw[di] += v[t];
          }
        }
      } else if (split) {
        const size_t srow = pmr ? (size_t)(pmr_n0 + row - pmr_row0) * (g.P * g.Q) + pmr_pq : (size_t)row;
        *reinterpret_cast<float4*>(slab + srow * args.Ng + col) = (float4){v[0], v[1], v[2], v[3]};
      } else {
        const unsigned short h0 = f2bf(v[0] + bias.x), h1 = f2bf(v[1] + bias.y);
        const unsigned short h2 = f2bf(v[2] + bias.z), h3 = f2bf(v[3] + bias.w);
        uint2 pk;
        pk.x = (unsigned)h0 | ((unsigned)h1 << 16);
        pk.y = (unsigned)h2 | ((unsigned)h3 << 16);
        size_t orow = row;
        if (phase) {
          const int hw = args.Hp * args.Wp;
          const int n = fast_div(row, args.dPQ), rem = row - n * hw;
          const int i = fast_div(rem, args.dQ), j = rem - i * args.Wp;
          orow = ((size_t)n * gg.H + args.pa + gg.stride * i) * gg.W + args.pb + gg.stride * j;
        } else if (pmr) {
          orow = (size_t)(pmr_n0 + row - pmr_row0) * (gg.P * gg.Q) + pmr_pq;
        }
        if (MODE == MODE_DGRAD && args.accumulate) {
          uint2* dst = reinterpret_cast<uint2*>(args.out + orow * args.Ng + col);
          const uint2 old = acc_old4(args.out, args.acc_dy, args.acc_mask, orow * args.Ng + col);
          pk.x = (unsigned)f2bf(v[0] + bf2f((unsigned short)(old.x & 0xffff))) |
                 ((unsigned)f2bf(v[1] + bf2f((unsigned short)(old.x >> 16))) << 16);
          pk.y = (unsigned)f2bf(v[2] + bf2f((unsigned short)(old.y & 0xffff))) |
                 ((unsigned)f2bf(v[3] + bf2f((unsigned short)(old.y >> 16))) << 16);
          *dst = pk;
        } else {
          *reinterpret_cast<uint2*>(args.out + orow * args.Ng + col) = pk;
        }
        if (MODE == MODE_FWD) {
          const float r0 = bf2f(h0), r1 = bf2f(h1), r2 = bf2f(h2), r3 = bf2f(h3);
          s[0] += r0; s[1] += r1; s[2] += r2; s[3] += r3;
          ss[0] += r0 * r0; ss[1] += r1 * r1; ss[2] += r2 * r2; ss[3] += r3 * r3;
        }
        if (MODE == MODE_DGRAD && kOldBnf && red) {
          const float gv[4] = {bf2f(h0), bf2f(h1), bf2f(h2), bf2f(h3)};
          const float fsc[4] = {bsc.x, bsc.y, bsc.z, bsc.w}, fsh[4] = {bsh.x, bsh.y, bsh.z, bsh.w};
          const float fmu[4] = {bmu.x, bmu.y, bmu.z, bmu.w}, fis[4] = {bis.x, bis.y, bis.z, bis.w};
          const BnBwdFuse& f = args.bnf;
          const int hw = g.H * g.W;
          const int n = fast_div((int)orow, args.dPQ), rem = (int)orow - n * hw;
          const int h = fast_div(rem, args.dQ), w = rem - h * g.W;
          const int np = f.pool ? 4 : 1;
          float zf[4][4];
#pragma unroll
          for (int d = 0; d < 4; ++d) {
            if (d >= np) break;
            const int zh = f.pool ? 2 * h + (d >> 1) : h, zw = f.pool ? 2 * w + (d & 1) : w;
            const uint2 zz = *reinterpret_cast<const uint2*>(
                f.z + (((size_t)n * f.Hz + zh) * f.Wz + zw) * args.Ng + col);
            zf[d][0] = bf2f((unsigned short)(zz.x & 0xffff));
            zf[d][1] = bf2f((unsigned short)(zz.x >> 16));
            zf[d][2] = bf2f((unsigned short)(zz.y & 0xffff));
            zf[d][3] = bf2f((unsigned short)(zz.y >> 16));
          }
#pragma unroll
          for (int t = 0; t < 4; ++t) {
            float best = -INFINITY, yarg = 0.f, zarg = 0.f;
#pragma unroll
            for (int d = 0; d < 4; ++d) {
              if (d >= np) break;
              const float y = zf[d][t] * fsc[t] + fsh[t];
              const float yr = f.relu ? fmaxf(y, 0.f) : y;
              if (d == 0 || yr > best || yr != yr) { best = yr; yarg = y; zarg = zf[d][t]; }
            }
            const float dyb = (f.relu && !(yarg > 0.f)) ? 0.f : gv[t];
            s[t] += dyb;
            ss[t] += dyb * ((zarg - fmu[t]) * fis[t]);
          }
        }
      }
    }
    if (red) {
#pragma unroll
      for (int t = 0; t < 4; ++t) {
        s[t] = dpp_sum16(s[t]);
        ss[t] = dpp_sum16(ss[t]);
      }
      float* slot = reinterpret_cast<float*>(smem) + (((wn * TN + j) * 4 + (lane >> 4)) * 8);
      if (wm == 1 && rl == 0) {
#pragma unroll
        for (int t = 0; t < 4; ++t) {
          slot[t] = s[t];
          slot[4 + t] = ss[t];
        }
      }
      stat_s[j][0] = s[0]; stat_s[j][1] = s[1]; stat_s[j][2] = s[2]; stat_s[j][3] = s[3];
      stat_ss[j][0] = ss[0]; stat_ss[j][1] = ss[1]; stat_ss[j][2] = ss[2]; stat_ss[j][3] = ss[3];
    }
  }
  if (red) {
    __syncthreads();
    if (wm == 0 && rl == 0) {
      float* st = (MODE == MODE_FWD ? args.stats : args.bnf.sums) +
                  stat_rep(bid) * 2 * args.Ng;
#pragma unroll
      for (int j = 0; j < TN; ++j) {
        const int col = col0 + wn * WTN + j * 16 + cq;
        if (col >= args.Ng) continue;
        const float* slot = reinterpret_cast<const float*>(smem) + (((wn * TN + j) * 4 + (lane >> 4)) * 8);
#pragma unroll
        for (int t = 0; t < 4; ++t) {
          atomicAdd(st + col + t, stat_val(stat_s[j][t] + slot[t], bid));
          atomicAdd(st + args.Ng + col + t, stat_val(stat_ss[j][t] + slot[4 + t], bid));
        }
      }
    }
  }
  };

  constexpr int DMA = CA + CB;
  for (int item = bid; item < nitems; item += nblk) {
    setup(item);
#pragma unroll
    for (int i = 0; i < TM; ++i)
#pragma unroll
      for (int j = 0; j < TN; ++j) acc[i][j] = (f32x4){0.f, 0.f, 0.f, 0.f};
    const int kb = ks_begin, ke = ks_end;
#pragma unroll
    for (int s = 0; s < NST - 1; ++s)
      if (kb + s < ke) issue(kb + s, s);
    int stage = 0;
    for (int ks = kb; ks < ke; ++ks) {
      const int ahead = ke - 1 - ks;
      if (NST >= 4 && ahead >= 2) wait_dma_barrier<(NST >= 4 ? 2 : 0) * DMA>();
      else if (NST >= 3 && ahead >= 1) wait_dma_barrier<(NST >= 3 ? 1 : 0) * DMA>();
      else wait_dma_barrier<0>();
      bf16x8 fa0[TM], fb0[TN], fa1[TM], fb1[TN];
      load_frags(stage, 0, fa0, fb0);
      if (ks + NST - 1 < ke) issue(ks + NST - 1, stage == 0 ? NST - 1 : stage - 1);
      load_frags(stage, 32, fa1, fb1);
      mma(fa0, fb0);
      mma(fa1, fb1);
      stage = stage + 1 == NST ? 0 : stage + 1;
    }
    epilogue(row0, col0, zsplit, args.splits > 1);
    if (item + nblk < nitems) wait_dma_barrier<0>();
  }
  if constexpr (XSTAT) {
    if (MODE == MODE_FWD && run_col >= 0)
      flush_stats(run_col, *reinterpret_cast<float(*)[8]>(run_s),
                  *reinterpret_cast<float(*)[8]>(run_ss));
  }
}

#ifndef DDP_CONV_WAVES_PER_EU
#define DDP_CONV_WAVES_PER_EU 2
#endif
template <int MODE, int BM, int BN, int NST, int BNF = 0, bool XSTAT = false>
__global__ __launch_bounds__(256) __attribute__((amdgpu_waves_per_eu(DDP_CONV_WAVES_PER_EU)))
void conv_igemm_kernel(ConvArgs args) {
  extern __shared__ __attribute__((aligned(16))) unsigned short smem[];
  conv_igemm_body<MODE, BM, BN, NST, BNF, XSTAT>(args, smem, blockIdx.x, gridDim.x);
}

template <int MODE, int BM, int BN, int NST>
__global__ __launch_bounds__(256) __attribute__((amdgpu_waves_per_eu(2)))
void conv_igemm_bnf2_kernel(ConvArgs args) {
  extern __shared__ __attribute__((aligned(16))) unsigned short smem[];
  conv_igemm_body<MODE, BM, BN, NST, 2>(args, smem, blockIdx.x, gridDim.x);
}

template <int BM, int BN, int NST, int BNF, bool SGDM = false>
__global__ __launch_bounds__(256) void conv_bwd_pair_kernel(ConvArgs dg, ConvArgs wg, int n_dg) {
  __shared__ __attribute__((aligned(16))) unsigned short smem[ConvSmem<BM, BN, NST>::elems];
  if ((int)blockIdx.x < n_dg)
    conv_igemm_body<MODE_DGRAD, BM, BN, NST, BNF>(dg, smem, blockIdx.x, n_dg);
  else
    conv_igemm_body<MODE_WGRAD, BM, BN, NST, 0, false, SGDM>(wg, smem, blockIdx.x - n_dg,
                                                           gridDim.x - n_dg);
}
struct RowMap {
  int stride, Hp, Wp, H, W, pa, pb;
};

__device__ __forceinline__ size_t map_row(const RowMap& m, int row) {
  if (m.stride == 0) return row;
  const int hw = m.Hp * m.Wp;
  const int n = row / hw, rem = row - n * hw;
  const int i = rem / m.Wp, j = rem - i * m.Wp;
  return ((size_t)n * m.H + m.pa + m.stride * i) * m.W + m.pb + m.stride * j;
}

constexpr int kSlabBatch = 8;
__device__ __forceinline__ void sum_slabs8(const float* p, size_t slab, int z0, int z1, float* v) {
  for (int zb = z0; zb < z1; zb += kSlabBatch) {
    float4 a[kSlabBatch], b[kSlabBatch];
#pragma unroll
    for (int u = 0; u < kSlabBatch; ++u) {
      if (zb + u < z1) {
        const float4* src = reinterpret_cast<const float4*>(p + (size_t)(zb + u) * slab);
        a[u] = src[0];
        b[u] = src[1];
      }
    }
#pragma unroll
    for (int u = 0; u < kSlabBatch; ++u) {
      if (zb + u < z1) {
        v[0] += a[u].x; v[1] += a[u].y; v[2] += a[u].z; v[3] += a[u].w;
        v[4] += b[u].x; v[5] += b[u].y; v[6] += b[u].z; v[7] += b[u].w;
      }
    }
  }
}

struct FinishArgs {
  const float* ws;
  int splits;
  unsigned short* out;
  const float* bias;
  float* stats;
  int Mg, Ng;
  RowMap rmap;
  int accumulate;
  BnBwdFuse bnf;
  int H, W;
  const unsigned short* acc_dy;
  const unsigned char* acc_mask;
};

template <bool BNF>
__device__ __forceinline__ void splitk_finish_body(const FinishArgs& fa, float* red_, int bx,
                                                   int by, int gx) {
  const float* ws = fa.ws;
  const int splits = fa.splits, Mg = fa.Mg, Ng = fa.Ng, accumulate = fa.accumulate;
  const int H = fa.H, W = fa.W;
  unsigned short* out = fa.out;
  const float* bias = fa.bias;
  float* stats = fa.stats;
  const RowMap rmap = fa.rmap;
  const BnBwdFuse& bnf = fa.bnf;
  float (*red)[8][256] = reinterpret_cast<float (*)[8][256]>(red_);
  constexpr bool has_bnf = BNF;
  const int G = Ng / 8;
  const int Gb = G < 256 ? G : 256;
  const int cgl = threadIdx.x % Gb, prow = threadIdx.x / Gb, prows = 256 / Gb;
  const int cg = by * Gb + cgl;
  const bool active = prow < prows && cg < G;
  const size_t slab = (size_t)Mg * Ng;
  float s[8], ss[8], bv[8];
  float fsc[8], fsh[8], fmu[8], fis[8];
#pragma unroll
  for (int e = 0; e < 8; ++e) {
    s[e] = 0.f;
    ss[e] = 0.f;
    bv[e] = (bias && cg < G) ? bias[cg * 8 + e] : 0.f;
    fsc[e] = fsh[e] = fmu[e] = fis[e] = 0.f;
  }
  if (has_bnf && cg < G) {
#pragma unroll
    for (int e = 0; e < 8; ++e) {
      fsc[e] = bnf.coef[0 * Ng + cg * 8 + e];
      fsh[e] = bnf.coef[1 * Ng + cg * 8 + e];
      fmu[e] = bnf.coef[2 * Ng + cg * 8 + e];
      fis[e] = bnf.coef[3 * Ng + cg * 8 + e];
    }
    stats = bnf.sums;
  }
  for (int row = bx * prows + prow; active && row < Mg; row += gx * prows) {
    float v[8];
#pragma unroll
    for (int e = 0; e < 8; ++e) v[e] = bv[e];
    sum_slabs8(ws + (size_t)row * Ng + cg * 8, slab, 0, splits, v);
    unsigned short* dst = out + map_row(rmap, row) * Ng + cg * 8;
    if (accumulate) {
      const u16x8 old = acc_old8(out, fa.acc_dy, fa.acc_mask, map_row(rmap, row) * Ng + cg * 8);
#pragma unroll
      for (int e = 0; e < 8; ++e) v[e] += bf2f(old[e]);
    }
    u16x8 o;
#pragma unroll
    for (int e = 0; e < 8; ++e) {
      o[e] = f2bf(v[e]);
      const float r = bf2f(o[e]);
      if (!has_bnf) {
        s[e] += r;
        ss[e] += r * r;
      }
    }
    st8(dst, o);
    if (has_bnf && bnf.code) {
      const int c0 = cg * 8;
      const unsigned* cw = bnf.code + (size_t)row * 16 + ((c0 & 15) >> 2) * 4 + (c0 >> 4);
      const unsigned w0 = cw[0], w1 = cw[4];
      const u16x8 zz = ld8(bnf.z + (size_t)row * Ng + c0);
#pragma unroll
      for (int e = 0; e < 8; ++e) {
        const unsigned code = ((e < 4 ? w0 : w1) >> (8 * (e & 3))) & 0xFFu;
        const float d = code < 4u ? bf2f(o[e]) : 0.f;
// ... 380 lines not shown
                                                              int ndx, int nfx) {
  if ((int)blockIdx.x < ndx) {
    linear_dx_bnbwd_body<RPT>(dl, Wt, B, F, J, gscale, bn, ba, blockIdx.x);
  } else {
    const int t = blockIdx.x - ndx;
    linear_dw_block(dl, x, B, F, J, gscale, dW, db, t % nfx, t / nfx);
  }
}

constexpr int kWgFinishGroup = kDeterministic ? (1 << 30) : 32;
__global__ __launch_bounds__(256) void wgrad_finish_kernel(const float* ws, int splits, int K,
                                                           int R, int S, int C, int Creal,
                                                           float* dw) {
  extern __shared__ __attribute__((aligned(16))) float row[];
  const int k = blockIdx.x;
  const int RS = R * S, RSC = RS * C;
  const size_t slab = (size_t)K * RSC;
  const int z0 = blockIdx.y * kWgFinishGroup, z1 = min(splits, z0 + kWgFinishGroup);
  for (int j = threadIdx.x; j < RSC; j += blockDim.x) {
    float v = 0.f;
    for (int z = z0; z < z1; ++z) v += ws[z * slab + (size_t)k * RSC + j];
    row[j] = v;
  }
  __syncthreads();
  float* out = dw + (size_t)k * Creal * RS;
  const bool single = gridDim.y == 1;
  for (int c = threadIdx.x; c < Creal; c += blockDim.x) {
    for (int rs = 0; rs < RS; ++rs) {
      const float v = row[rs * C + c];
      if (single) out[c * RS + rs] += v;
      else atomicAdd(out + c * RS + rs, v);
    }
  }
}

__device__ __forceinline__ float sgd_step1(float p, float g, float& b, const SgdFuse& h,
                                           float lr) {
  return sgd_update1(p, g, b, lr, h.momentum, h.wd, h.grad_scale, h.nesterov);
}

constexpr int kWgFinishGroupKrsc = kDeterministic ? (1 << 30) : 16;
__device__ __forceinline__ void wgrad_finish_krsc_body(const float* __restrict__ ws, int splits,
                                                       int K, int RS, int C, int Creal,
                                                       float* __restrict__ dw, int bx, int by,
                                                       int gx, int gy, const SgdFuse& sg) {
  const size_t slab = (size_t)K * RS * C;
  const size_t n4 = slab / 4;
  const int z0 = by * kWgFinishGroupKrsc, z1 = min(splits, z0 + kWgFinishGroupKrsc);
  const bool single = gy == 1;
  const bool opt = single && sg.p != nullptr;
  const float lr = opt ? sched_lr_block(sg.sched, sg.lr) : sg.lr;
  for (size_t i = bx * (size_t)blockDim.x + threadIdx.x; i < n4;
       i += (size_t)gx * blockDim.x) {
    float4 v = reinterpret_cast<const float4*>(ws + z0 * slab)[i];
    for (int zb = z0 + 1; zb < z1; zb += kSlabBatch) {
      float4 a[kSlabBatch];
#pragma unroll
      for (int u = 0; u < kSlabBatch; ++u)
        if (zb + u < z1) a[u] = reinterpret_cast<const float4*>(ws + (size_t)(zb + u) * slab)[i];
#pragma unroll
      for (int u = 0; u < kSlabBatch; ++u)
        if (zb + u < z1) { v.x += a[u].x; v.y += a[u].y; v.z += a[u].z; v.w += a[u].w; }
    }
    const float vv[4] = {v.x, v.y, v.z, v.w};
    if (opt) {
      if (Creal == C) {
        float4 pv = reinterpret_cast<float4*>(sg.p)[i];
        float4 bv = reinterpret_cast<float4*>(sg.buf)[i];
        pv.x = sgd_step1(pv.x, v.x, bv.x, sg, lr);
        pv.y = sgd_step1(pv.y, v.y, bv.y, sg, lr);
        pv.z = sgd_step1(pv.z, v.z, bv.z, sg, lr);
        pv.w = sgd_step1(pv.w, v.w, bv.w, sg, lr);
        reinterpret_cast<float4*>(sg.p)[i] = pv;
        reinterpret_cast<float4*>(sg.buf)[i] = bv;
        uint2 pk;
        pk.x = (unsigned)f2bf(pv.x) | ((unsigned)f2bf(pv.y) << 16);
        pk.y = (unsigned)f2bf(pv.z) | ((unsigned)f2bf(pv.w) << 16);
        *reinterpret_cast<uint2*>(sg.wc + i * 4) = pk;
      } else {
        const size_t e = i * 4;
        const int c = (int)(e % C);
        const size_t krs = e / C;
#pragma unroll
        for (int t = 0; t < 4; ++t) {
          if (c + t >= Creal) continue;
          const size_t mi = krs * Creal + c + t;
          float b = sg.buf[mi];
          const float np = sgd_step1(sg.p[mi], vv[t], b, sg, lr);
          sg.p[mi] = np;
          sg.buf[mi] = b;
          sg.wc[e + t] = f2bf(np);
        }
      }
      continue;
    }
    if (Creal == C) {
      if (single) {
        float4* o = reinterpret_cast<float4*>(dw) + i;
        float4 d = *o;
        d.x += v.x; d.y += v.y; d.z += v.z; d.w += v.w;
        *o = d;
      } else {
#pragma unroll
        for (int t = 0; t < 4; ++t) unsafeAtomicAdd(dw + i * 4 + t, vv[t]);
      }
    } else {
      const size_t e = i * 4;
      const int c = (int)(e % C);
      const size_t krs = e / C;
#pragma unroll
      for (int t = 0; t < 4; ++t) {
        if (c + t >= Creal) continue;
        if (single) dw[krs * Creal + c + t] += vv[t];
        else unsafeAtomicAdd(dw + krs * Creal + c + t, vv[t]);
      }
    }
  }
}

__global__ __launch_bounds__(256) void wgrad_finish_krsc_kernel(const float* __restrict__ ws,
                                                                int splits, int K, int RS, int C,
                                                                int Creal, float* __restrict__ dw,
                                                                SgdFuse sg) {
  wgrad_finish_krsc_body(ws, splits, K, RS, C, Creal, dw, blockIdx.x, blockIdx.y, gridDim.x,
                         gridDim.y, sg);
}

struct WgFinishArgs {
  const float* ws;
  int splits, K, RS, C, Creal;
  float* dw;
  int gx, gy;
  SgdFuse sgd;
};

template <bool BNF>
__global__ __launch_bounds__(256) void bwd_pair_finish_kernel(FinishArgs fa, int dgx, int dgy,
                                                              WgFinishArgs wa) {
  __shared__ float red[2 * 8 * 256];
  const int b = blockIdx.x;
  if (b < dgx * dgy) {
    splitk_finish_body<BNF>(fa, red, b % dgx, b / dgx, dgx);
  } else {
    const int w = b - dgx * dgy;
    wgrad_finish_krsc_body(wa.ws, wa.splits, wa.K, wa.RS, wa.C, wa.Creal, wa.dw, w % wa.gx,
                           w / wa.gx, wa.gx, wa.gy, wa.sgd);
  }
}

}

using namespace ddp_amd;

static FastDiv make_fastdiv(int d) {
  FastDiv f;
  int sh = 0;
  while ((1ll << sh) < d) ++sh;
  f.sh = sh;
  f.mul = (unsigned)((((1ull << sh) - (unsigned long long)d) << 32) / (unsigned long long)d + 1);
  return f;
}

static bool fits_buffer(size_t elems) { return elems * 2 < (size_t)kOOB; }

static int g_stages = 2;
constexpr int kNumCUs = 256;
static int g_epi_stage = 1;
static bool epi_stage_enabled() { return g_epi_stage != 0; }
extern "C" void ddp_conv_epi_stage_set(int on) { g_epi_stage = on ? 1 : 0; }

static int pick_splits(int tiles, int ksteps, size_t slab, const ConvArgs& a, size_t ws_elems) {
  if (a.splits > 0) return std::max(1, std::min(a.splits, ksteps));

  if (a.ws == nullptr) return 1;
  int s = (512 + tiles - 1) / tiles;
  s = std::max(1, std::min(s, ksteps / 4));
  s = (int)std::min<size_t>((size_t)s, std::max<size_t>(1, ws_elems / slab));
  return s;
}

static double tile_cost(int BM, int BN, const ConvArgs& a, size_t ws_elems, int* splits_out) {
  const int tiles = ((a.Mg + BM - 1) / BM) * ((a.Ng + BN - 1) / BN);
  const int ksteps = (a.Kg + 63) / 64;
  const size_t slab = (size_t)a.Mg * a.Ng;
  const int splits = pick_splits(tiles, ksteps, slab, a, ws_elems);
  *splits_out = splits;
  const double eff = (BM == 128 && BN == 128) ? 1.0 : ((BM == 64 && BN == 64) ? 0.55 : 0.8);
  const int resident = (BM == 128 && BN == 128) ? 2 : ((BM == 64 && BN == 64) ? 4 : 3);
  const double blocks = (double)tiles * splits;
  const double fill = std::min(1.0, blocks / (256.0 * resident));
  const double work = (double)tiles * BM * BN * ksteps * 64.0;
  const double t_mfma = work / (eff * fill) / 1.0e15 * 2.0;
  double t_split = 0.0;
  if (splits > 1) t_split = 8.0 * splits * (double)slab / 4.0e12 + 3.0e-6;
  return t_mfma + t_split;
}

static int stages_for(int BM, int BN) {
  if (g_stages <= 2) return 2;
  if (BM == 128 && BN == 128) return g_stages >= 4 ? 4 : 2;
  if (BM == 64 && BN == 64) return g_stages >= 4 ? 4 : 3;
  return 3;
}

static int fwd_stat_grid() {
  constexpr int g = 2048;
  return (kDeterministic ? std::min(g, kStatRep) : g) / 8 * 8;
}

template <int MODE, int BM, int BN, int NST, int BNF>
static void launch_gemm_t(const ConvArgs& a, int items, hipStream_t st) {
  constexpr int kStageBytes = (BM + BN) * 64 * 2;
  constexpr int kTileBytes = BM * BN * 2;
  const int stages = std::max(1, std::min(NST, a.ksteps_per_split));
  size_t lds = (size_t)stages * kStageBytes;
  if (a.epi_stage && lds < (size_t)kTileBytes) lds = kTileBytes;
  int grid = items;
  if (MODE == MODE_FWD && a.stats && a.splits <= 1 && a.epi_stage && !(BM == 64 && BN == 64) &&
      fwd_stat_grid() > 0 && items > fwd_stat_grid())
    grid = fwd_stat_grid();
  void (*kern)(ConvArgs);
  if constexpr (BNF == 2 && MODE == MODE_DGRAD) kern = conv_igemm_bnf2_kernel<MODE, BM, BN, NST>;
  else if constexpr (MODE == MODE_FWD && BNF == 0 && !(BM == 64 && BN == 64))
    kern = grid < items ? conv_igemm_kernel<MODE, BM, BN, NST, 0, true>
                        : conv_igemm_kernel<MODE, BM, BN, NST, 0, false>;
  else kern = conv_igemm_kernel<MODE, BM, BN, NST, BNF>;
  static bool attr[2] = {false, false};
  if (!attr[grid < items]) {
    (void)hipFuncSetAttribute(reinterpret_cast<const void*>(kern),
                              hipFuncAttributeMaxDynamicSharedMemorySize,
                              std::max(NST * kStageBytes, kTileBytes));
    attr[grid < items] = true;
  }
  hipLaunchKernelGGL(kern, dim3(grid), dim3(256), lds, st, a);
}

template <int MODE, int BM, int BN, int NST>
static void launch_gemm(const ConvArgs& a, int items, hipStream_t st) {
  if constexpr (MODE == MODE_DGRAD) {
    if (a.has_bnf && a.splits <= 1)
      return a.bnf.pool ? launch_gemm_t<MODE, BM, BN, NST, 1>(a, items, st)
                        : launch_gemm_t<MODE, BM, BN, NST, 2>(a, items, st);
  }
  launch_gemm_t<MODE, BM, BN, NST, 0>(a, items, st);
}

static int g_wgrad_pm = 1, g_rows_pm = 1;
extern "C" void ddp_conv_wgrad_pm_set(int mode) { g_wgrad_pm = std::max(0, std::min(2, mode)); }
extern "C" void ddp_conv_rows_pm_set(int mode) { g_rows_pm = std::max(0, std::min(4, mode)); }
template <int MODE>
static bool rows_pixmajor_ok(const ConvArgs& a, int BM) {
  const ConvGeom& g = a.g;
  const int cdim = MODE == MODE_FWD ? g.C : g.K;
  const bool any_pq = g_rows_pm == 2 || g_rows_pm == 4;
  if (g_rows_pm >= 3 && g.R * g.S == 1) return false;
  return g_rows_pm && !a.d2x2 && !a.phase && !a.accumulate && g.stride == 1 && g.P == g.H &&
         g.Q == g.W && cdim % 64 == 0 && g.N % BM == 0 && (any_pq || g.P * g.Q <= 64) &&
         g.R * g.S <= 32 && g.Creal == g.C && a.Mg == g.N * g.P * g.Q;
}
static bool wgrad_pixmajor_ok(const ConvArgs& a, int BN) {
  const ConvGeom& g = a.g;
  return g_wgrad_pm && g.stride == 1 && g.P == g.H && g.Q == g.W && g.N % 64 == 0 &&
         (g_wgrad_pm == 2 || g.P * g.Q <= 64) && g.C % BN == 0 && g.Creal == g.C && a.Ng == g.R * g.S * g.C &&
         a.Kg == g.N * g.P * g.Q;
}

template <int MODE, int BM, int BN>
static int prepare_cfg(ConvArgs& a, int splits) {
  constexpr int BK = 64;
  const int tiles = ((a.Mg + BM - 1) / BM) * ((a.Ng + BN - 1) / BN);
  const int ksteps = (a.Kg + BK - 1) / BK;
  const int per = (ksteps + splits - 1) / splits;
  splits = (ksteps + per - 1) / per;
  a.splits = splits;
  a.ksteps_per_split = per;
  a.epi_stage = MODE != MODE_WGRAD && epi_stage_enabled();
  a.pixmajor = MODE == MODE_WGRAD ? wgrad_pixmajor_ok(a, BN) : rows_pixmajor_ok<MODE>(a, BM);
  if (MODE == MODE_DGRAD) {
    const int hh = a.phase ? a.Hp : a.g.H, ww = a.phase ? a.Wp : a.g.W;
    a.dPQ = make_fastdiv(std::max(1, hh * ww));
    a.dQ = make_fastdiv(std::max(1, ww));
  } else {
    a.dPQ = make_fastdiv(std::max(1, a.g.P * a.g.Q));
    a.dQ = make_fastdiv(std::max(1, a.g.Q));
  }
  return tiles * splits;
}

static bool needs_finish(int mode, const ConvArgs& a) {
  (void)mode;
  return a.splits > 1;
}

static int finish_rows_per_thread(int Mg, int rows_per_block) {
  return (Mg + rows_per_block - 1) / rows_per_block <= 128 ? 1 : 2;
}

static void dg_finish_grid(const ConvArgs& a, int* bx_out, int* chunks_out) {
  const int G = a.Ng / 8;
  const int Gb = G < 256 ? G : 256;
  const int chunks = (G + Gb - 1) / Gb;
  const int rows_per_block = std::max(1, 256 / Gb);
  const int rpt = finish_rows_per_thread(a.Mg, rows_per_block);
  int bx = (a.Mg + rows_per_block * rpt - 1) / (rows_per_block * rpt);
  *bx_out = std::max(1, std::min(bx, 2048 / chunks + 1));
  *chunks_out = chunks;
}

static FinishArgs finish_args(int mode, const ConvArgs& a) {
  RowMap rm{0, 0, 0, 0, 0, 0, 0};
  if (a.phase) rm = RowMap{a.g.stride, a.Hp, a.Wp, a.g.H, a.g.W, a.pa, a.pb};
  const bool fwd = mode == MODE_FWD;
  return FinishArgs{a.ws, a.splits, a.out, fwd ? a.bias : nullptr, fwd ? a.stats : nullptr,
                    a.Mg, a.Ng, rm, a.accumulate, a.bnf, a.g.H, a.g.W, a.acc_dy, a.acc_mask};
}

static std::map<const float*, SgdFuse> g_sgd_reg;
static std::set<const float*> g_sgd_taken;
static std::set<const float*> g_sgd_master;
static SgdFuse sgd_fuse_master(const float* dw) {
  if (g_sgd_reg.empty()) return SgdFuse{};
  auto it = g_sgd_reg.find(dw);
  if (it == g_sgd_reg.end()) return SgdFuse{};
  g_sgd_master.insert(dw);
  return it->second;
}
static bool g_sgd_allow = false;
static SgdFuse sgd_fuse_for(const float* dw, int groups) {
  if (!g_sgd_allow || groups != 1 || g_sgd_reg.empty()) return SgdFuse{};
  auto it = g_sgd_reg.find(dw);
  if (it == g_sgd_reg.end()) return SgdFuse{};
  g_sgd_taken.insert(dw);
  return it->second;
}

static WgFinishArgs wg_finish_args(const ConvArgs& a) {
  const size_t n4 = (size_t)a.Mg * a.Ng / 4;
  const int groups = (a.splits + kWgFinishGroupKrsc - 1) / kWgFinishGroupKrsc;
  const int bx = (int)std::min<size_t>((n4 + 255) / 256, std::max(1, 2048 / groups));
  return WgFinishArgs{a.ws, a.splits, a.g.K, a.g.R * a.g.S, a.g.C, a.g.Creal, a.dw, bx, groups,
                      sgd_fuse_for(a.dw, groups)};
}

static int g_bn_fuse_rows = 128;
static int bn_fuse_max_rows() { return g_bn_fuse_rows; }
static int bn_bwd_fuse_max_rows() { return bn_fuse_max_rows(); }

static bool bnbwd_fusable(const ConvArgs& a) {
  return a.has_bnf && a.bnapply && a.splits > 1 && !a.phase && !a.accumulate &&
         a.Mg <= bn_bwd_fuse_max_rows() && a.Mg <= kBnBwdFuseMaxRows && a.Ng % 16 == 0 &&
         a.g.stride == 1 &&
         (!a.bnf.pool || (a.bnf.Hz == 2 * a.g.H && a.bnf.Wz == 2 * a.g.W)) &&
         (a.bnf.pool || (a.bnf.Hz == a.g.H && a.bnf.Wz == a.g.W));
}

template <int RPT, bool POOL>
__global__ __launch_bounds__(256) void bwd_pair_finish_bnbwd_kernel(FinishArgs fa, BnBwdApply ba,
                                                                    int dgx, WgFinishArgs wa) {
  __shared__ float wred[4][2][8];
  const int b = blockIdx.x;
  if (b < dgx) {
    finish_bnbwd_body<RPT, POOL>(fa, ba, wred, b);
  } else {
    const int w = b - dgx;
    wgrad_finish_krsc_body(wa.ws, wa.splits, wa.K, wa.RS, wa.C, wa.Creal, wa.dw, w % wa.gx,
                           w / wa.gx, wa.gx, wa.gy, wa.sgd);
  }
}

template <int RPT, bool POOL>
static void launch_bnbwd_t(const FinishArgs& fa, const BnBwdApply& ba, int dgx,
                           const WgFinishArgs* wa, hipStream_t st) {
  if (wa)
    hipLaunchKernelGGL((bwd_pair_finish_bnbwd_kernel<RPT, POOL>), dim3(dgx + wa->gx * wa->gy),
                       dim3(256), 0, st, fa, ba, dgx, *wa);
  else
    hipLaunchKernelGGL((splitk_finish_bnbwd_kernel<RPT, POOL>), dim3(dgx), dim3(256), 0, st, fa, ba);
}

static bool launch_finish_bnbwd(const ConvArgs& a, hipStream_t st, const WgFinishArgs* wa) {
  if (!bnbwd_fusable(a)) return false;
  const FinishArgs fa = finish_args(MODE_DGRAD, a);
  const BnBwdApply& ba = *a.bnapply;
  const int dgx = a.Ng / 16, rpt = (a.Mg + 127) / 128;
  if (a.bnf.pool) {
    if (rpt <= 1) launch_bnbwd_t<1, true>(fa, ba, dgx, wa, st);
    else if (rpt <= 2) launch_bnbwd_t<2, true>(fa, ba, dgx, wa, st);
    else launch_bnbwd_t<4, true>(fa, ba, dgx, wa, st);
  } else {
    if (rpt <= 1) launch_bnbwd_t<1, false>(fa, ba, dgx, wa, st);
    else if (rpt <= 2) launch_bnbwd_t<2, false>(fa, ba, dgx, wa, st);
    else launch_bnbwd_t<4, false>(fa, ba, dgx, wa, st);
  }
  if (a.bnapply_done) *a.bnapply_done = 1;
  return true;
}

static bool launch_finish_bnfwd(const ConvArgs& a, hipStream_t st) {
  const BnFwdFuse& bf = *a.bnfwd;
  if (a.Mg > kBnFwdFuseMaxRows || a.Mg > bn_fuse_max_rows() || a.Ng % 16 || a.accumulate ||
      a.phase)
    return false;
  if (bf.P * bf.Q <= 0 || a.Mg % (bf.P * bf.Q)) return false;
  if (bf.pool && (bf.P % 2 || bf.Q % 2)) return false;
  const FinishArgs fa = finish_args(MODE_FWD, a);
  const dim3 grid(a.Ng / 16);
  const size_t lds = bf.pool ? (size_t)a.Mg * 16 * sizeof(float) : 0;
  static const bool attr = [] {
    (void)hipFuncSetAttribute(reinterpret_cast<const void*>(splitk_finish_bnfwd_kernel<8>),
                              hipFuncAttributeMaxDynamicSharedMemorySize,
                              kBnFwdFuseMaxRows * 16 * sizeof(float));
    return true;
  }();
  (void)attr;
  const int rpt = (a.Mg + 127) / 128;
  if (rpt <= 1) hipLaunchKernelGGL(splitk_finish_bnfwd_kernel<1>, grid, dim3(256), lds, st, fa, bf);
  else if (rpt <= 2) hipLaunchKernelGGL(splitk_finish_bnfwd_kernel<2>, grid, dim3(256), lds, st, fa, bf);
  else if (rpt <= 4) hipLaunchKernelGGL(splitk_finish_bnfwd_kernel<4>, grid, dim3(256), lds, st, fa, bf);
  else hipLaunchKernelGGL(splitk_finish_bnfwd_kernel<8>, grid, dim3(256), lds, st, fa, bf);
  if (a.bnfwd_done) *a.bnfwd_done = 1;
  return true;
}

template <int MODE>
static void launch_finish(const ConvArgs& a, hipStream_t st) {
  if (!needs_finish(MODE, a)) return;
  if (MODE == MODE_WGRAD && a.g.wkrsc) {
    const WgFinishArgs w = wg_finish_args(a);
    hipLaunchKernelGGL(wgrad_finish_krsc_kernel, dim3(w.gx, w.gy), dim3(256), 0, st, a.ws,
                       a.splits, a.g.K, a.g.R * a.g.S, a.g.C, a.g.Creal, a.dw, w.sgd);
  } else if (MODE == MODE_WGRAD) {
    const int groups = (a.splits + kWgFinishGroup - 1) / kWgFinishGroup;
    const size_t lds = sizeof(float) * a.g.R * a.g.S * a.g.C;
    hipLaunchKernelGGL(wgrad_finish_kernel, dim3(a.g.K, groups), dim3(256), lds, st, a.ws,
                       a.splits, a.g.K, a.g.R, a.g.S, a.g.C, a.g.Creal, a.dw);
  } else {
    if (MODE == MODE_FWD && a.bnfwd && launch_finish_bnfwd(a, st)) return;
    if (MODE == MODE_DGRAD && a.has_bnf && a.bnapply && launch_finish_bnbwd(a, st, nullptr)) return;
    int bx, chunks;
    dg_finish_grid(a, &bx, &chunks);
    const FinishArgs fa = finish_args(MODE, a);
    if (MODE == MODE_DGRAD && a.has_bnf)
      hipLaunchKernelGGL(splitk_finish_kernel<true>, dim3(bx, chunks), dim3(256), 0, st, fa);
    else
      hipLaunchKernelGGL(splitk_finish_kernel<false>, dim3(bx, chunks), dim3(256), 0, st, fa);
  }
}

template <int MODE, int BM, int BN>
static void launch_cfg(ConvArgs& a, int splits, hipStream_t st, int nst_req = 0) {
  const int items = prepare_cfg<MODE, BM, BN>(a, splits);
  constexpr int kStageBytes = (BM + BN) * 64 * 2;
  constexpr int kMaxStages = kStageBytes * 4 <= 163840 ? 4 : (kStageBytes * 3 <= 163840 ? 3 : 2);
  int nst = nst_req >= 2 && nst_req <= 4 ? nst_req : stages_for(BM, BN);
  nst = std::min(nst, kMaxStages);
  if constexpr (kMaxStages >= 4) {
    if (nst == 4) { launch_gemm<MODE, BM, BN, 4>(a, items, st); goto launched; }
  }
  if constexpr (kMaxStages >= 3) {
    if (nst == 3) { launch_gemm<MODE, BM, BN, 3>(a, items, st); goto launched; }
  }
  launch_gemm<MODE, BM, BN, 2>(a, items, st);
launched:
  if (!a.no_finish) launch_finish<MODE>(a, st);
}

struct TuneKey {
  int mode, M, N, K;
  int hw = 0;
  bool operator<(const TuneKey& o) const {
    if (mode != o.mode) return mode < o.mode;
    if (M != o.M) return M < o.M;
    if (N != o.N) return N < o.N;
    if (K != o.K) return K < o.K;
    return hw < o.hw;
  }
};
struct TuneVal {
  int tile, splits, stages;
};
static std::map<TuneKey, TuneVal> g_tuned;
static std::map<TuneKey, TuneVal> g_pair_tuned;
static int g_pair_force_dg = 0, g_pair_force_wg = 0;
static int g_force_tile = 0;
static int g_force_stages = 0;

constexpr int kNumTiles = 8;

template <int MODE>
static bool tile_ok(int tile) {
  if (MODE == MODE_WGRAD && (tile == 5 || tile == 7)) return false;
  return tile >= 0 && tile < kNumTiles;
}

template <int MODE>
static void plan_mode(ConvArgs& a, size_t ws_elems, int* best_out, int* sp, int* nst_out) {
  const double c[4] = {tile_cost(128, 128, a, ws_elems, &sp[0]), tile_cost(128, 64, a, ws_elems, &sp[1]),
                       tile_cost(64, 128, a, ws_elems, &sp[2]), tile_cost(64, 64, a, ws_elems, &sp[3])};
  int best = 0, nst = g_force_stages;
  for (int i = 1; i < 4; ++i)
    if (c[i] < c[best]) best = i;
  if (g_force_tile >= 1 && g_force_tile <= kNumTiles && tile_ok<MODE>(g_force_tile - 1)) {
    best = g_force_tile - 1;
    if (best >= 4) {
      static const int bmn[4][2] = {{256, 64}, {64, 256}, {256, 128}, {128, 256}};
      tile_cost(bmn[best - 4][0], bmn[best - 4][1], a, ws_elems, &sp[best]);
    }
  } else if (a.splits <= 0) {
    auto it = g_tuned.find(TuneKey{MODE, a.Mg, a.Ng, a.Kg});
    if (it != g_tuned.end() && tile_ok<MODE>(it->second.tile)) {
      const size_t slab = (size_t)a.Mg * a.Ng;
      const int ksteps = (a.Kg + 63) / 64;
      int spl = std::max(1, std::min(it->second.splits, ksteps));
      if (spl > 1 && (size_t)spl * slab > ws_elems) spl = std::max<int>(1, (int)(ws_elems / slab));
      if (ws_elems == 0) spl = 1;
      best = it->second.tile;
      sp[best] = spl;
      nst = it->second.stages;
    }
  }
  *best_out = best;
  *nst_out = nst;
}

template <int MODE>
static void launch_mode(ConvArgs& a, size_t ws_elems, hipStream_t st) {
  int sp[kNumTiles], best, nst;
  plan_mode<MODE>(a, ws_elems, &best, sp, &nst);
  switch (best) {
    case 0: launch_cfg<MODE, 128, 128>(a, sp[0], st, nst); break;
    case 1: launch_cfg<MODE, 128, 64>(a, sp[1], st, nst); break;
    case 2: launch_cfg<MODE, 64, 128>(a, sp[2], st, nst); break;
    case 3: launch_cfg<MODE, 64, 64>(a, sp[3], st, nst); break;
    case 4: launch_cfg<MODE, 256, 64>(a, sp[4], st, nst); break;
    case 6: launch_cfg<MODE, 256, 128>(a, sp[6], st, nst); break;
    default:
      if constexpr (MODE != MODE_WGRAD) {
        if (best == 5) launch_cfg<MODE, 64, 256>(a, sp[5], st, nst);
        else launch_cfg<MODE, 128, 256>(a, sp[7], st, nst);
      }
      break;
  }
}

extern "C" void ddp_conv_options(int stages) { g_stages = stages; }

extern "C" void ddp_conv_tune_set(int mode, int M, int N, int K, int tile, int splits, int stages) {
  if (mode == 3) {
    g_pair_tuned[TuneKey{MODE_DGRAD, M, N, K}] = {tile >= 0 && tile < 6 ? tile : 1,
                                                  std::max(1, splits), std::max(1, stages)};
    return;
  }
  if (tile < 0 || tile >= kNumTiles) return;
  g_tuned[TuneKey{mode, M, N, K}] = {tile, std::max(1, splits), stages};
}
extern "C" void ddp_conv_pair_tune_set(int M, int N, int K, int hw, int tile, int sd, int sw) {
  g_pair_tuned[TuneKey{MODE_DGRAD, M, N, K, hw}] = {tile >= 0 && tile < 6 ? tile : 1,
                                                    std::max(1, sd), std::max(1, sw)};
}
extern "C" void ddp_conv_tune_clear() {
  g_tuned.clear();
  g_pair_tuned.clear();
}
static int g_pair_force_tile_req = 0;
extern "C" void ddp_conv_pair_force(int splits_dg, int splits_wg, int tile) {
  g_pair_force_dg = splits_dg;
  g_pair_force_wg = splits_wg;
  g_pair_force_tile_req = tile;
}
extern "C" void ddp_conv_force_tile(int tile_plus_one, int stages) {
  g_force_tile = tile_plus_one;
  g_force_stages = stages;
}

static int g_dense2x2 = 1;
static bool dense2x2_on() { return g_dense2x2 != 0; }
extern "C" void ddp_conv_dense2x2_set(int on) { g_dense2x2 = on ? 1 : 0; }
extern "C" int ddp_conv_dense2x2_ok(const ConvGeom* g) {
  return dense2x2_on() && g->R == 3 && g->S == 3 && g->stride == 1 && g->pad == 1 &&
         g->H == 2 && g->W == 2 && g->P == 2 && g->Q == 2 && g->C % 64 == 0 && g->K % 64 == 0 &&
         g->Creal == g->C && fits_buffer((size_t)g->K * 9 * g->C) &&
         fits_buffer((size_t)g->N * 4 * std::max(g->C, g->K));
}
static void dense2x2_args(ConvArgs& a, const ConvGeom* g, int mode) {
  a.g = *g;
  a.g.H = a.g.W = a.g.P = a.g.Q = 1;
  a.g.R = a.g.S = 1;
  a.g.pad = 0;
  a.g.C = a.g.Creal = 4 * g->C;
  a.g.K = 4 * g->K;
  a.Mg = g->N;
  a.Ng = mode == MODE_FWD ? 4 * g->K : 4 * g->C;
  a.Kg = mode == MODE_FWD ? 4 * g->C : 4 * g->K;
  a.d2x2 = 1;
  a.d2C = g->C;
  a.d2K = g->K;
  a.a_bytes = (int)(2 * (size_t)g->N * a.Kg);
  a.b_bytes = (int)(2 * (size_t)g->K * 9 * g->C);
}
static int dense2x2_splits(const ConvArgs& a, size_t ws_elems) {
  const int tiles = ((a.Mg + 63) / 64) * ((a.Ng + 63) / 64), ksteps = a.Kg / 64;
  int sp = std::max(2, std::min((512 + tiles - 1) / tiles, ksteps / 4));
  const size_t slab = (size_t)a.Mg * a.Ng;
  if ((size_t)sp * slab > ws_elems) sp = (int)(ws_elems / slab);
  return sp >= 2 ? sp : 0;
}
static ConvArgs finish_view(const ConvArgs& a, const ConvGeom* g, int mode) {
  if (!a.d2x2) return a;
  ConvArgs f = a;
  f.g = *g;
  f.d2x2 = 0;
  f.Mg = g->N * g->P * g->Q;
  f.Ng = mode == MODE_FWD ? g->K : g->C;
  f.Kg = 9 * (mode == MODE_FWD ? g->C : g->K);
  return f;
}

static int conv_fwd_dense(const ConvGeom* g, const void* x, const void* wc, const float* bias,
                          void* y, float* stats, float* ws, size_t ws_elems, const BnFwdFuse* bn,
                          int* bn_done, hipStream_t st) {
  if (!ddp_conv_dense2x2_ok(g) || ws == nullptr) return -1;
  ConvArgs a{};
  dense2x2_args(a, g, MODE_FWD);
  a.a = (const unsigned short*)x;
  a.b = (const unsigned short*)wc;
  a.out = (unsigned short*)y;
  a.ws = ws;
  a.splits = dense2x2_splits(a, ws_elems);
  if (a.splits < 2) return -1;
  a.no_finish = 1;
  launch_mode<MODE_FWD>(a, ws_elems, st);
  ConvArgs f = finish_view(a, g, MODE_FWD);
  f.no_finish = 0;
  f.bias = bias;
  f.stats = stats;
  if (bn && f.Mg <= kBnFwdFuseMaxRows) {
    f.bnfwd = bn;
    f.bnfwd_done = bn_done;
  }
  launch_finish<MODE_FWD>(f, st);
  return (int)hipGetLastError();
}

extern "C" int ddp_conv_fwd(const ConvGeom* g, const void* x, const void* wc, const float* bias,
                            void* y, float* stats, float* ws, size_t ws_elems, int splits,
                            hipStream_t st) {
  if (g->C % 8 || g->K % 8) return -1;
  {
    const int r = conv_fwd_dense(g, x, wc, bias, y, stats, ws, ws_elems, nullptr, nullptr, st);
    if (r >= 0) return r;
  }
  ConvArgs a{};
  a.g = *g;
  a.a = (const unsigned short*)x;
  a.b = (const unsigned short*)wc;
  a.out = (unsigned short*)y;
  a.ws = ws;
  a.bias = bias;
  a.stats = stats;
  a.Mg = g->N * g->P * g->Q;
  a.Ng = g->K;
  a.Kg = g->R * g->S * g->C;
  a.splits = splits;
// ... 442 lines not shown
```

### distributed-data-parallel-ml-training_amd/csrc/kernels/conv_tr.hip

```cpp
#include "common.h"
#include "api.h"

#include <algorithm>
#include <cstdlib>
#include <map>
#include <tuple>

namespace ddp_amd {
namespace tr {

typedef __attribute__((address_space(3))) void lds_void;

constexpr unsigned kOOB = 0x80000000u;

__device__ __forceinline__ __amdgpu_buffer_rsrc_t make_rsrc(const void* base, int bytes) {
  return __builtin_amdgcn_make_buffer_rsrc(const_cast<void*>(base), (short)0, bytes, 0x00020000);
}

__device__ __forceinline__ void dma(__amdgpu_buffer_rsrc_t rs, unsigned byte_off, unsigned short* lds) {
  __builtin_amdgcn_raw_ptr_buffer_load_lds(rs, (lds_void*)lds, 16, (int)byte_off, 0, 0, 0);
}

template <int N>
__device__ __forceinline__ void wait_dma_barrier() {
  asm volatile("s_waitcnt vmcnt(%0)\n\ts_barrier" ::"n"(N) : "memory");
}

template <int NBMAX, int CBn, int NLn>
__device__ __forceinline__ void wait_stage(int bafter, bool anext) {
  if constexpr (NBMAX > 0) {
    if (bafter >= NBMAX) {
      if (anext) wait_dma_barrier<NBMAX * CBn + NLn>();
      else wait_dma_barrier<NBMAX * CBn>();
      return;
    }
    wait_stage<NBMAX - 1, CBn, NLn>(bafter, anext);
  } else {
    wait_dma_barrier<0>();
  }
}

__device__ __forceinline__ int rk_off(int row, int chunk) {
  return row * 64 + ((chunk ^ ((row >> 1) & 7)) << 3);
}

__host__ __device__ __forceinline__ int plane_base(int c, int plane) { return c * plane + 4 * (c >> 1); }

struct Args {
  int N, H, W, C, K;
  const unsigned short* x;
  const unsigned short* wc;
  const float* bias;
  unsigned short* z;
  float* stats;
  float* ws;
  int splits, cbps;
  int imgs, rows, bands;
  int imgp, plane, zslot;
  int x_bytes, w_bytes;
  int tiles_m, tiles_n;
  int abuf_elems;
  const unsigned short* zin;
  const float* in_stats;
  const float* in_gamma;
  const float* in_beta;
  float in_eps;
  int in_relu;
  float* in_coef;
  unsigned short* y_out;
  int z_bytes;
};

template <int BM, int BN, int NST, int NL, int IN>
#ifndef DDP_TR_WAVES_PER_EU
#define DDP_TR_WAVES_PER_EU 1
#endif
__global__ __launch_bounds__(256) __attribute__((amdgpu_waves_per_eu(DDP_TR_WAVES_PER_EU)))
void conv_tr_fwd_kernel(Args a) {
  constexpr int WTM = BM / 2, WTN = BN / 2, TM = WTM / 16, TN = WTN / 16;
  constexpr int CB = BN * 64 / 8 / 256;
  constexpr int BTILE = BN * 64;
  static_assert(CB >= 1 && TM >= 1 && TN >= 1, "tile");
  static_assert(NST >= 3 && NST <= 9, "the next patch is issued at tap 0: at most one in the window");
  extern __shared__ __attribute__((aligned(16))) unsigned short smem[];
  const int aelems = a.abuf_elems;
  unsigned short* abuf = smem;
  unsigned short* bring = smem + 2 * aelems;
  float* cf = reinterpret_cast<float*>(bring + NST * BTILE);
  constexpr int NP = IN == 2 ? 4 : 1;
  constexpr bool BNIN = IN == 1 || IN == 2;

  const int tid = threadIdx.x, lane = tid & 63;
  const int wid = __builtin_amdgcn_readfirstlane(tid >> 6);
  const int wm = wid >> 1, wn = wid & 1;
  const int W = a.W, H = a.H, C = a.C, K = a.K;
  const int M = a.N * H * W;
  const int ncb = C / 64;

  const int tiles = a.tiles_m * a.tiles_n;
  const int item = blockIdx.x;
  const int sp = item / tiles;
  const int tile = xcd_remap(item - sp * tiles, tiles);
  const int tm = tile / a.tiles_n;
  const int tn = tile - tm * a.tiles_n;
  const int row0 = tm * BM, col0 = tn * BN;
  const int cb0 = sp * a.cbps, cb1 = min(ncb, cb0 + a.cbps);
  const int nsteps = (cb1 - cb0) * 9;
  const int n0 = (tm / a.bands) * a.imgs;
  const int h0 = (tm % a.bands) * a.rows;

  const __amdgpu_buffer_rsrc_t rsA = IN ? make_rsrc(a.zin, a.z_bytes) : make_rsrc(a.x, a.x_bytes);
  if (BNIN) {
    const int Hz = IN == 2 ? 2 * H : H, Wz = IN == 2 ? 2 * W : W;
    const float Mz = (float)a.N * Hz * Wz;
    for (int c = tid; c < C; c += 256) {
      float s1 = 0.f, s2 = 0.f;
#pragma unroll
      for (int r = 0; r < kStatRep; ++r) {
        s1 += a.in_stats[r * 2 * C + c];
        s2 += a.in_stats[r * 2 * C + C + c];
      }
      const float mu = s1 / Mz;
      const float var = fmaxf(s2 / Mz - mu * mu, 0.f);
      const float is = rsqrtf(var + a.in_eps);
      const float sc = a.in_gamma[c] * is, sh = a.in_beta[c] - mu * sc;
      cf[c] = sc;
      cf[C + c] = sh;
      if (blockIdx.x == 0) {
        a.in_coef[0 * C + c] = sc;
        a.in_coef[1 * C + c] = sh;
        a.in_coef[2 * C + c] = mu;
        a.in_coef[3 * C + c] = is;
      }
    }
    __syncthreads();
  }
  const __amdgpu_buffer_rsrc_t rsB = make_rsrc(a.wc, a.w_bytes);

  unsigned asrc[NL];
  int adst[NL];
  int ydst[NL];
  const bool write_y = BNIN && tn == 0;
  {
    const int pw = (a.rows + 2) * W;
    const int npix = a.imgs * pw;
#pragma unroll
    for (int u = 0; u < NL; ++u) {
      const int it = u * 256 + tid;
      const int px = it >> 3, c = it & 7;
      unsigned off = kOOB;
      int dst = -1, yd = -1;
      if (px < npix) {
        const int img = px / pw, loc = px - img * pw;
        const int hr = loc / W, wc = loc - hr * W;
        const int h = h0 + hr - 1;
        if (h >= 0 && h < H) {
          const int n = n0 + img;
          if (IN == 2)
            off = (unsigned)(2 * (((n * 2 * H + 2 * h) * 2 * W + 2 * wc) * C + c * 8));
          else
            off = (unsigned)(2 * (((n * H + h) * W + wc) * C + c * 8));
          if (write_y && hr >= 1 && hr <= a.rows) yd = ((n * H + h) * W + wc) * C + c * 8;
        }
        dst = (plane_base(c, a.plane) + img * a.imgp + loc) * 16;
      }
      asrc[u] = off;
      adst[u] = dst;
      ydst[u] = yd;
    }
  }
  typedef int v4i __attribute__((ext_vector_type(4)));
  v4i areg[NL][NP];
  const unsigned pofs[4] = {0u, (unsigned)(2 * C), (unsigned)(2 * 2 * W * C),
                            (unsigned)(2 * (2 * W * C + C))};
  auto load_a = [&](int cb) {
    const unsigned coff = (unsigned)(cb * 128);
#pragma unroll
    for (int u = 0; u < NL; ++u)
#pragma unroll
      for (int d = 0; d < NP; ++d)
        areg[u][d] = __builtin_amdgcn_raw_buffer_load_b128(rsA, (int)(asrc[u] + coff + pofs[d]), 0, 0);
  };
  auto store_a = [&](int buf, int cb) {
    char* dst = reinterpret_cast<char*>(abuf + buf * aelems);
    float sc[8], sh[8];
    if (BNIN) {
      const int c0 = cb * 64 + (tid & 7) * 8;
#pragma unroll
      for (int e = 0; e < 8; ++e) {
        sc[e] = cf[c0 + e];
        sh[e] = cf[C + c0 + e];
      }
    }
#pragma unroll
    for (int u = 0; u < NL; ++u) {
      if (adst[u] < 0) continue;
      v4i v = areg[u][0];
      if (BNIN) {
        if (asrc[u] == kOOB) {
          v = (v4i){0, 0, 0, 0};
        } else {
          float best[8];
#pragma unroll
          for (int d = 0; d < NP; ++d) {
            const v4i q = areg[u][d];
#pragma unroll
            for (int e = 0; e < 8; ++e) {
              const unsigned w32 = (unsigned)q[e >> 1];
              const float zf = __uint_as_float((e & 1) ? (w32 & 0xffff0000u) : (w32 << 16));
              float y = zf * sc[e] + sh[e];
              if (a.in_relu) y = fmaxf(y, 0.f);
              if (d == 0 || y > best[e] || y != y) best[e] = y;
            }
          }
#pragma unroll
          for (int e = 0; e < 4; ++e)
            v[e] = (int)((unsigned)f2bf(best[2 * e]) | ((unsigned)f2bf(best[2 * e + 1]) << 16));
          if (ydst[u] >= 0)
            *reinterpret_cast<v4i*>(a.y_out + ydst[u] + cb * 64) = v;
        }
      }
      *reinterpret_cast<v4i*>(dst + adst[u]) = v;
    }
  };
  const int lcB = (tid & 7) ^ ((tid >> 4) & 7);
  unsigned boff[CB];
#pragma unroll
  for (int i = 0; i < CB; ++i) {
    const int col = col0 + (tid >> 3) + 32 * i;
    boff[i] = col < K ? (unsigned)(2 * (col * 9 * C + lcB * 8)) : kOOB;
  }

  auto issue_b = [&](int j, int slot) {
    const int cb = cb0 + j / 9, t = j - (j / 9) * 9;
    const unsigned k0 = (unsigned)(2 * (t * C + cb * 64));
    unsigned short* dst = bring + slot * BTILE;
#pragma unroll
    for (int i = 0; i < CB; ++i) dma(rsB, boff[i] + k0, dst + (wid * 64 + 256 * i) * 8);
  };

  int fa_base[TM];
  unsigned col_ok[TM];
#pragma unroll
  for (int i = 0; i < TM; ++i) {
    const int m = wm * WTM + i * 16 + (lane & 15);
    const int per_img = a.rows * W;
    const int img = m / per_img, rem = m - img * per_img;
    const int rr = rem / W, cc = rem - rr * W;
    const int pix = img * a.imgp + rr * W + cc;
    fa_base[i] = (plane_base(lane >> 4, a.plane) + pix) * 16;
    col_ok[i] = (cc >= 1 ? 1u : 0u) | (cc <= W - 2 ? 2u : 0u);
  }
  const int kk_a = (plane_base(4, a.plane) - plane_base(0, a.plane)) * 16;
  int fb_off[TN];
#pragma unroll
  for (int j = 0; j < TN; ++j) fb_off[j] = rk_off(wn * WTN + j * 16 + (lane & 15), lane >> 4);

  f32x4 acc[TM][TN];
#pragma unroll
  for (int i = 0; i < TM; ++i)
#pragma unroll
    for (int j = 0; j < TN; ++j) acc[i][j] = (f32x4){0.f, 0.f, 0.f, 0.f};

  auto compute = [&](int t, int abuf_i, int slot) {
    const char* Ab = reinterpret_cast<const char*>(abuf + abuf_i * aelems);
    const unsigned short* Bs = bring + slot * BTILE;
    const int r = t / 3, s = t - r * 3;
    const int trow = r * W * 16, tcol = (s - 1) * 16;
#pragma unroll
    for (int kk = 0; kk < 64; kk += 32) {
      bf16x8 fa[TM], fb[TN];
#pragma unroll
      for (int i = 0; i < TM; ++i) {
        const bool ok = s == 1 || (col_ok[i] & (s == 0 ? 1u : 2u));
        const int off = fa_base[i] + trow + (ok ? tcol : 0) + (kk ? kk_a : 0);
        fa[i] = *reinterpret_cast<const bf16x8*>(Ab + off);
        if (s != 1 && !ok) fa[i] = (bf16x8){};
      }
#pragma unroll
      for (int j = 0; j < TN; ++j) fb[j] = *reinterpret_cast<const bf16x8*>(Bs + (fb_off[j] ^ (kk ? 32 : 0)));
#pragma unroll
      for (int i = 0; i < TM; ++i)
#pragma unroll
        for (int j = 0; j < TN; ++j)
          acc[i][j] = __builtin_amdgcn_mfma_f32_16x16x32_bf16(fb[j], fa[i], acc[i][j], 0, 0, 0);
    }
  };

  load_a(cb0);
#pragma unroll
  for (int s = 0; s < NST - 1; ++s)
    if (s < nsteps) issue_b(s, s);
  store_a(0, cb0);

  const int ncbl = cb1 - cb0;
  int slot = 0;
  for (int cbl = 0; cbl < ncbl; ++cbl) {
    const bool more = cbl + 1 < ncbl;
#pragma unroll
    for (int t = 0; t < 9; ++t) {
      const int j = cbl * 9 + t;
      const int bafter = min(NST - 2, nsteps - 1 - j);
      const bool anext = (t >= 1 && t <= NST - 2) && more;
      if (t == 0) asm volatile("s_waitcnt lgkmcnt(0)" ::: "memory");
      wait_stage<NST - 2, CB, NL * NP>(bafter, anext);
      if (t == 0 && more) load_a(cb0 + cbl + 1);
      if (j + NST - 1 < nsteps) issue_b(j + NST - 1, slot == 0 ? NST - 1 : slot - 1);
      compute(t, cbl & 1, slot);
      if (t == 8 && more) store_a((cbl + 1) & 1, cb0 + cbl + 1);
      slot = slot + 1 == NST ? 0 : slot + 1;
    }
  }

  const int rl = lane & 15, cq = 4 * (lane >> 4);
  const int cbase = col0 + wn * WTN + cq;
  if (a.splits > 1) {
    float* slab = a.ws + (size_t)sp * M * K;
#pragma unroll
    for (int i = 0; i < TM; ++i) {
      const int row = row0 + wm * WTM + i * 16 + rl;
      if (row >= M) continue;
#pragma unroll
      for (int j = 0; j < TN; ++j) {
        const int col = cbase + j * 16;
        if (col >= K) continue;
        const f32x4 v = acc[i][j];
        *reinterpret_cast<float4*>(slab + (size_t)row * K + col) = (float4){v[0], v[1], v[2], v[3]};
      }
    }
    return;
  }
  const bool red = a.stats != nullptr;
  float* sl = reinterpret_cast<float*>(smem);
  if (red) __syncthreads();
#pragma unroll
  for (int j = 0; j < TN; ++j) {
    const int col = cbase + j * 16;
    float4 bj = {0.f, 0.f, 0.f, 0.f};
    if (a.bias != nullptr && col < K) bj = *reinterpret_cast<const float4*>(a.bias + col);
    float s[4] = {0.f, 0.f, 0.f, 0.f}, ss[4] = {0.f, 0.f, 0.f, 0.f};
#pragma unroll
    for (int i = 0; i < TM; ++i) {
      const int row = row0 + wm * WTM + i * 16 + rl;
      if (row >= M || col >= K) continue;
      const f32x4 v = acc[i][j];
      uint2 pk;
      pk.x = (unsigned)f2bf(v[0] + bj.x) | ((unsigned)f2bf(v[1] + bj.y) << 16);
      pk.y = (unsigned)f2bf(v[2] + bj.z) | ((unsigned)f2bf(v[3] + bj.w) << 16);
      *reinterpret_cast<uint2*>(a.z + (size_t)row * K + col) = pk;
      if (red) {
        const float r0 = __uint_as_float(pk.x << 16), r1 = __uint_as_float(pk.x & 0xffff0000u);
        const float r2 = __uint_as_float(pk.y << 16), r3 = __uint_as_float(pk.y & 0xffff0000u);
        s[0] += r0; s[1] += r1; s[2] += r2; s[3] += r3;
        ss[0] += r0 * r0; ss[1] += r1 * r1; ss[2] += r2 * r2; ss[3] += r3 * r3;
      }
    }
    if (red) {
#pragma unroll
      for (int q = 0; q < 4; ++q) {
        s[q] = dpp_sum16(s[q]);
        ss[q] = dpp_sum16(ss[q]);
      }
      float* st = sl + ((((wm * 2 + wn) * TN + j) * 4 + (lane >> 4)) * 8);
      if (rl == 0) {
#pragma unroll
        for (int q = 0; q < 4; ++q) {
          st[q] = s[q];
          st[4 + q] = ss[q];
        }
      }
    }
  }
  if (!red) return;
  __syncthreads();
  if (wm == 0 && rl == 0) {
    float* st = a.stats + stat_rep(blockIdx.x) * 2 * K;
#pragma unroll
    for (int j = 0; j < TN; ++j) {
      const int col = cbase + j * 16;
      if (col >= K) continue;
      const float* s0 = sl + (((wn * TN + j) * 4 + (lane >> 4)) * 8);
      const float* s1 = sl + ((((2 + wn) * TN + j) * 4 + (lane >> 4)) * 8);
#pragma unroll
      for (int q = 0; q < 4; ++q) {
        atomicAdd(st + col + q, stat_val(s0[q] + s1[q], blockIdx.x));
        atomicAdd(st + K + col + q, stat_val(s0[4 + q] + s1[4 + q], blockIdx.x));
      }
    }
  }
}

struct Geo {
  int imgs, rows, bands, imgp, plane, zslot, nl, abuf;
  bool ok;
};

static const int kGroups[4][16] = {
    {0, 1, 2, 3, 12, 13, 14, 15, 20, 21, 22, 23, 24, 25, 26, 27},
    {4, 5, 6, 7, 8, 9, 10, 11, 16, 17, 18, 19, 28, 29, 30, 31},
    {32, 33, 34, 35, 44, 45, 46, 47, 52, 53, 54, 55, 56, 57, 58, 59},
    {36, 37, 38, 39, 40, 41, 42, 43, 48, 49, 50, 51, 60, 61, 62, 63}};

static bool conflict_free(int BM, int W, int rows, int imgp, int plane) {
  const int per_img = rows * W;
  for (int m0 = 0; m0 < BM; m0 += 16)
    for (int t = 0; t < 9; ++t) {
      const int r = t / 3, s = t % 3;
      for (int kk = 0; kk < 2; ++kk)
        for (int g = 0; g < 4; ++g) {
          bool used[16] = {false};
          for (int e = 0; e < 16; ++e) {
            const int l = kGroups[g][e];
            const int m = m0 + (l & 15), cp = (l >> 4) + 4 * kk;
            const int img = m / per_img, rem = m % per_img, rr = rem / W, cc = rem % W;
            const bool ok = (s == 1) || (s == 0 && cc >= 1) || (s == 2 && cc <= W - 2);
            if (!ok) continue;
            const int pix = img * imgp + (rr + r) * W + cc + s - 1;
            const int q = (plane_base(cp, plane) + pix) & 15;
            if (used[q]) return false;
            used[q] = true;
          }
        }
    }
  return true;
}

static Geo geometry_uncached(int BM, int N, int H, int W) {
  Geo g{};
  g.ok = false;
  const int hw = H * W;
  if (W < 2 || BM % 16) return g;
  if (hw <= BM) {
    if (BM % hw || N % (BM / hw)) return g;
    g.imgs = BM / hw;
    g.rows = H;
    g.bands = 1;
  } else {
    if (BM % W) return g;
    g.rows = BM / W;
    if (H % g.rows) return g;
    g.imgs = 1;
    g.bands = H / g.rows;
  }
  const int pw = (g.rows + 2) * W;
  for (int imgp = pw; imgp < pw + 32; ++imgp) {
    const int npix = g.imgs * imgp;
    const int plane = (npix + 1 + 15) / 16 * 16;
    if (conflict_free(BM, W, g.rows, imgp, plane)) {
      g.imgp = imgp;
      g.plane = plane;
      g.zslot = npix;
      g.nl = (g.imgs * pw * 8 + 255) / 256;
      g.abuf = (plane_base(7, plane) + plane) * 8;
      g.ok = true;
      return g;
    }
    if (g.imgs == 1) break;
  }
  return g;
}

static Geo geometry(int BM, int N, int H, int W) {
  static std::map<std::tuple<int, int, int, int>, Geo> cache;
  const auto key = std::make_tuple(BM, N, H, W);
  auto it = cache.find(key);
  if (it != cache.end()) return it->second;
  const Geo g = geometry_uncached(BM, N, H, W);
  cache[key] = g;
  return g;
}

static size_t lds_bytes(const Args& a, int nst, int bn, int in) {
  const size_t table = in ? 2 * (size_t)a.C * 4 : 0;
  return 2 * (size_t)a.abuf_elems * 2 + (size_t)nst * bn * 64 * 2 + table;
}

template <int BM, int BN, int NST, int NL, int IN>
static void launch_t(const Args& a, int items, hipStream_t st) {
  const size_t lds = lds_bytes(a, NST, BN, IN);
  static bool attr = false;
  if (!attr) {
    (void)hipFuncSetAttribute(reinterpret_cast<const void*>(conv_tr_fwd_kernel<BM, BN, NST, NL, IN>),
                              hipFuncAttributeMaxDynamicSharedMemorySize, 160 * 1024);
    attr = true;
  }
  hipLaunchKernelGGL((conv_tr_fwd_kernel<BM, BN, NST, NL, IN>), dim3(items), dim3(256), lds, st, a);
}

template <int BM, int BN, int NST, int IN>
static bool launch_nl(const Args& a, int nl, int items, hipStream_t st) {
  if (lds_bytes(a, NST, BN, IN) > 160 * 1024) return false;
  switch (nl) {
    case 1: launch_t<BM, BN, NST, 1, IN>(a, items, st); return true;
    case 2: launch_t<BM, BN, NST, 2, IN>(a, items, st); return true;
    case 3: launch_t<BM, BN, NST, 3, IN>(a, items, st); return true;
    case 4: launch_t<BM, BN, NST, 4, IN>(a, items, st); return true;
    case 5: launch_t<BM, BN, NST, 5, IN>(a, items, st); return true;
    case 6: launch_t<BM, BN, NST, 6, IN>(a, items, st); return true;
    default: return false;
  }
}

template <int BM, int BN>
static bool launch_bmbn(int nst, int in, const Args& a, int nl, int items, hipStream_t st) {
  if (in == 1) return nst == 3 && launch_nl<BM, BN, 3, 1>(a, nl, items, st);
  if (in == 2) return nst == 3 && launch_nl<BM, BN, 3, 2>(a, nl, items, st);
  switch (nst) {
    case 3: return launch_nl<BM, BN, 3, 0>(a, nl, items, st);
    case 5: return launch_nl<BM, BN, 5, 0>(a, nl, items, st);
    case 8: return launch_nl<BM, BN, 8, 0>(a, nl, items, st);
    default: return false;
  }
}

struct Cfg {
  int bm, bn, splits, stages;
};

static bool launch_stages(const Cfg& c, int in, const Args& a, int nl, int items, hipStream_t st) {
  const int n = in ? 3 : (c.stages ? c.stages : 3);
  if (c.bm == 128 && c.bn == 128) return launch_bmbn<128, 128>(n, in, a, nl, items, st);
  if (c.bm == 128 && c.bn == 64) return launch_bmbn<128, 64>(n, in, a, nl, items, st);
  if (c.bm == 64 && c.bn == 128) return launch_bmbn<64, 128>(n, in, a, nl, items, st);
  if (c.bm == 64 && c.bn == 64) return launch_bmbn<64, 64>(n, in, a, nl, items, st);
  return false;
}
static std::map<std::tuple<int, int, int, int>, Cfg> g_tr_tuned;
static int g_tr_mode = 1;
static Cfg g_tr_force{0, 0, 0, 0};

static Cfg heuristic(int N, int H, int W, int C, int K) {
  const int M = N * H * W;
  const int ncb = C / 64;
  Cfg c{128, K % 128 == 0 && K >= 256 ? 128 : 64, 1, 0};
  if (M / 128 * (K / c.bn) < 256) c.bm = 64;
  if (!geometry(c.bm, N, H, W).ok) c.bm = c.bm == 128 ? 64 : 128;
  const int tiles = (M / c.bm) * (K / c.bn);
  int s = 1;
  while (tiles * s < 256 && s * 2 <= ncb) s *= 2;
  c.splits = s;
  return c;
}

}
}

using namespace ddp_amd;

extern "C" int ddp_conv_fwd_finish(const ConvGeom* g, float* ws, int splits, const float* bias,
                                   void* z, float* stats, const BnFwdFuse* bn, int* bn_done,
                                   hipStream_t st);

extern "C" void ddp_conv_tr_set(int mode, int M, int K, int C, int H, int bm, int bn, int splits,
                                int stages) {
  if (mode == -1) { tr::g_tr_tuned.clear(); return; }
  if (mode == 0 || mode == 1 || mode == 4) { tr::g_tr_mode = mode == 4 ? 2 : mode; return; }
  if (mode == 2) { tr::g_tr_tuned[std::make_tuple(M, K, C, H)] = tr::Cfg{bm, bn, splits, stages}; return; }
  if (mode == 3) tr::g_tr_force = tr::Cfg{bm, bn, splits, stages};
}

namespace ddp_amd {
namespace tr {
struct Plan {
  Cfg c;
  Geo geo;
  int splits, cbps;
};

static bool plan(const ConvGeom* g, float* ws, size_t ws_elems, int in_mode, Plan* p) {
  if (!g_tr_mode) return false;
  if (g->R != 3 || g->S != 3 || g->stride != 1 || g->pad != 1 || g->P != g->H || g->Q != g->W)
    return false;
  if (g->C % 64 || g->K % 64 || g->Creal != g->C) return false;
  if (!g_tr_force.bm && ddp_conv_dense2x2_ok(g)) return false;
  const int N = g->N, H = g->H, W = g->W, C = g->C, K = g->K;
  const size_t M = (size_t)N * H * W;
  const size_t xe = M * C * (in_mode == 2 ? 4 : 1), we = (size_t)K * 9 * C;
  if (2 * xe >= kOOB || 2 * we >= kOOB || M * K >= kOOB) return false;
  Cfg c;
  auto it = g_tr_tuned.find(std::make_tuple((int)M, K, C, H));
  if (g_tr_force.bm) c = g_tr_force;
  else if (it != g_tr_tuned.end()) c = it->second;
  else if (g_tr_mode == 2) c = heuristic(N, H, W, C, K);
  else return false;
  if (c.bm == 0) return false;
  if (K % c.bn || M % c.bm) return false;
  const Geo geo = geometry(c.bm, N, H, W);
  if (!geo.ok || geo.nl < 1 || geo.nl > 6) return false;
  const int nst = in_mode ? 3 : (c.stages ? c.stages : 3);
  const size_t lds = 2 * (size_t)geo.abuf * 2 + (size_t)nst * c.bn * 64 * 2 +
                     (in_mode ? 2 * (size_t)C * 4 : 0);
  if (lds > 160 * 1024) return false;
  const int ncb = C / 64;
  int splits = std::max(1, std::min(c.splits, ncb));
  int cbps = (ncb + splits - 1) / splits;
  splits = (ncb + cbps - 1) / cbps;
  if (splits > 1 && (ws == nullptr || (size_t)splits * M * K > ws_elems)) {
    splits = 1;
    cbps = ncb;
  }
  p->c = c;
  p->geo = geo;
  p->splits = splits;
  p->cbps = cbps;
  return true;
}
}
}

extern "C" int ddp_conv_fwd_tr(const ConvGeom* g, const void* x, const void* wc, const float* bias,
                               void* z, float* stats, float* ws, size_t ws_elems,
                               const BnFwdFuse* bn, int* bn_done, const TrFwdIn* in,
                               hipStream_t st) {
  using namespace ddp_amd::tr;
  if (bn_done) *bn_done = 0;
  const int in_mode = in ? (in->pool ? 2 : 1) : 0;
  if (in && (!in->z || !in->stats || !in->gamma || !in->beta || !in->coef || !in->y)) return -1;
  Plan pl;
  if (!plan(g, ws, ws_elems, in_mode, &pl)) return 0;
  const Cfg& c = pl.c;
  const Geo& geo = pl.geo;
  const int N = g->N, H = g->H, W = g->W, C = g->C, K = g->K;
  const size_t M = (size_t)N * H * W;
  Args a{};
  a.N = N; a.H = H; a.W = W; a.C = C; a.K = K;
  a.x = (const unsigned short*)x;
  a.wc = (const unsigned short*)wc;
  a.bias = bias;
  a.z = (unsigned short*)z;
  a.stats = stats;
  a.ws = ws;
  a.splits = pl.splits;
  a.cbps = pl.cbps;
  a.imgs = geo.imgs; a.rows = geo.rows; a.bands = geo.bands;
  a.imgp = geo.imgp; a.plane = geo.plane; a.zslot = geo.zslot;
  a.x_bytes = (int)(2 * M * C);
  a.w_bytes = (int)(2 * (size_t)K * 9 * C);
  a.abuf_elems = geo.abuf;
  a.tiles_m = (int)(M / c.bm);
  a.tiles_n = K / c.bn;
  if (in) {
    a.zin = (const unsigned short*)in->z;
    a.in_stats = in->stats;
    a.in_gamma = in->gamma;
    a.in_beta = in->beta;
    a.in_eps = in->eps;
    a.in_relu = in->relu;
    a.in_coef = in->coef;
    a.y_out = (unsigned short*)in->y;
    a.z_bytes = (int)(2 * M * C * (in->pool ? 4 : 1));
  }
  const int items = a.tiles_m * a.tiles_n * pl.splits;
  if (!launch_stages(c, in_mode, a, geo.nl, items, st)) return 0;
  int e = (int)hipGetLastError();
  if (e) return 2 + e;
  if (pl.splits > 1) {
    e = ddp_conv_fwd_finish(g, ws, pl.splits, bias, z, stats, bn, bn_done, st);
    if (e) return 2 + e;
  }
  return 1;
}

extern "C" int ddp_conv_tr_would_serve(const ConvGeom* g, size_t ws_elems, int in_mode) {
  ddp_amd::tr::Plan pl;
  float dummy;
  if (in_mode < 0) return 0;
  return ddp_amd::tr::plan(g, ws_elems ? &dummy : nullptr, ws_elems, in_mode, &pl) ? 1 : 0;
}

extern "C" int ddp_conv_tr_geometry(int BM, int N, int H, int W, int* out7) {
  const ddp_amd::tr::Geo g = ddp_amd::tr::geometry(BM, N, H, W);
  out7[0] = g.ok; out7[1] = g.imgs; out7[2] = g.rows; out7[3] = g.bands;
  out7[4] = g.imgp; out7[5] = g.plane; out7[6] = g.nl;
  return g.ok ? 1 : 0;
}
```

Before: 364,900 images/s.

## Replace integer divisions with fast-div, add stamp profiling, restructure wgrad epilogue

```diff
diff --git a/distributed-data-parallel-ml-training_amd/_build.py b/distributed-data-parallel-ml-training_amd/_build.py
--- a/distributed-data-parallel-ml-training_amd/_build.py
+++ b/distributed-data-parallel-ml-training_amd/_build.py
@@ -27,7 +27,8 @@
 
 
 VARIANTS = {"release": ("_native", "native", []),
-            "det": ("_native_det", "native_det", ["-DDDP_AMD_DETERMINISTIC"])}
+            "det": ("_native_det", "native_det", ["-DDDP_AMD_DETERMINISTIC"]),
+            "stamps": ("_native_stamps", "native_stamps", ["-DDDP_CONV_STAMPS"])}
 
 
 def ext_path(variant="release"):
@@ -135,5 +136,5 @@
 
 
 if __name__ == "__main__":
-    build(verbose=True)
+    build(verbose=True, variants=tuple(sys.argv[1:]) or ("release", "det"))
     sys.exit(0)
diff --git a/distributed-data-parallel-ml-training_amd/csrc/bind.cpp b/distributed-data-parallel-ml-training_amd/csrc/bind.cpp
--- a/distributed-data-parallel-ml-training_amd/csrc/bind.cpp
+++ b/distributed-data-parallel-ml-training_amd/csrc/bind.cpp
@@ -483,6 +483,9 @@
   });
   m.def("conv_force_tile", [](int t, int stages) { ddp_conv_force_tile(t, stages); },
         py::arg("tile_plus_one"), py::arg("stages") = 0);
+#ifdef DDP_CONV_STAMPS
+  m.def("conv_stamps_set", [](uintptr_t buf, int cap) { ddp_conv_stamps_set(P<void>(buf), cap); });
+#endif
   m.def("pack_conv_weights", [](std::vector<std::tuple<uintptr_t, uintptr_t, uintptr_t, int, int,
                                                        int, int, int, int>> descs, uintptr_t st) {
     std::vector<ddp_amd::PackDesc> d;
diff --git a/distributed-data-parallel-ml-training_amd/csrc/kernels/api.h b/distributed-data-parallel-ml-training_amd/csrc/kernels/api.h
--- a/distributed-data-parallel-ml-training_amd/csrc/kernels/api.h
+++ b/distributed-data-parallel-ml-training_amd/csrc/kernels/api.h
@@ -248,6 +248,9 @@
 void ddp_conv_dense2x2_set(int on);
 void ddp_conv_tune_clear();
 void ddp_conv_force_tile(int tile_plus_one, int stages);
+#ifdef DDP_CONV_STAMPS
+void ddp_conv_stamps_set(void* buf, int cap);
+#endif
 int ddp_pack_conv_weights(const ddp_amd::PackDesc* descs, int n, hipStream_t st);
 int ddp_sgd_pack(const void* items, int n_items, const long long* descs, float* p, float* g,
                  float* buf, float lr, float momentum, float wd, float grad_scale, int nesterov,
diff --git a/distributed-data-parallel-ml-training_amd/csrc/kernels/common.h b/distributed-data-parallel-ml-training_amd/csrc/kernels/common.h
--- a/distributed-data-parallel-ml-training_amd/csrc/kernels/common.h
+++ b/distributed-data-parallel-ml-training_amd/csrc/kernels/common.h
@@ -118,6 +118,48 @@
   return (xcd < r ? xcd * (q + 1) : r * (q + 1) + (xcd - r) * q) + idx;
 }
 
+struct FastDiv {
+  unsigned mul;
+  int sh;
+};
+__device__ __forceinline__ int fast_div(int x, FastDiv d) {
+  return (int)((__umulhi((unsigned)x, d.mul) + (unsigned)x) >> d.sh);
+}
+inline FastDiv make_fastdiv(int d) {
+  FastDiv f;
+  int sh = 0;
+  while ((1ll << sh) < d) ++sh;
+  f.sh = sh;
+  f.mul = (unsigned)((((1ull << sh) - (unsigned long long)d) << 32) / (unsigned long long)d + 1);
+  return f;
+}
+
+#ifdef DDP_CONV_STAMPS
+struct ConvStampBuf {
+  unsigned* buf;
+  int cap;
+};
+extern ConvStampBuf g_conv_stamps;
+__device__ __forceinline__ unsigned long long stamp_now() {
+  __builtin_amdgcn_sched_barrier(0);
+  const unsigned long long t = __builtin_readcyclecounter();
+  __builtin_amdgcn_sched_barrier(0);
+  return t;
+}
+__device__ __forceinline__ void stamp_put(const ConvStampBuf& s, unsigned tag, unsigned long long t0,
+                                          unsigned long long t1, unsigned long long t2,
+                                          unsigned long long t3) {
+  if (!s.buf || threadIdx.x != 0) return;
+  const unsigned i = atomicAdd(s.buf, 1u);
+  if (i >= (unsigned)s.cap) return;
+  unsigned* r = s.buf + 4 + 4 * (size_t)i;
+  r[0] = tag;
+  r[1] = (unsigned)(t1 - t0);
+  r[2] = (unsigned)(t2 - t1);
+  r[3] = (unsigned)(t3 - t2);
+}
+#endif
+
 __host__ __device__ __forceinline__ uint32_t hash_u32(uint32_t x) {
   x ^= x >> 16; x *= 0x7feb352du;
   x ^= x >> 15; x *= 0x846ca68bu;
diff --git a/distributed-data-parallel-ml-training_amd/csrc/kernels/conv_igemm.hip b/distributed-data-parallel-ml-training_amd/csrc/kernels/conv_igemm.hip
--- a/distributed-data-parallel-ml-training_amd/csrc/kernels/conv_igemm.hip
+++ b/distributed-data-parallel-ml-training_amd/csrc/kernels/conv_igemm.hip
@@ -14,13 +14,6 @@
 typedef short short8_t __attribute__((ext_vector_type(8)));
 typedef __attribute__((address_space(3))) v4i16 lds_v4i16;
 
-struct FastDiv {
-  unsigned mul;
-  int sh;
-};
-__device__ __forceinline__ int fast_div(int x, FastDiv d) {
-  return (int)((__umulhi((unsigned)x, d.mul) + (unsigned)x) >> d.sh);
-}
 __global__ __launch_bounds__(256) void zero16_kernel(uint4* __restrict__ p, size_t n16) {
   for (size_t i = blockIdx.x * 256ull + threadIdx.x; i < n16; i += (size_t)gridDim.x * 256)
     p[i] = (uint4){0u, 0u, 0u, 0u};
@@ -64,6 +57,11 @@
   const unsigned char* acc_mask;
   SgdFuse sgd;
   int pixmajor;
+  FastDiv dTiles, dTilesN, dN, dCdim, dKb, dSdec, dS, dC, dNb, dD2C, dD2K, dSplits;
+  int w_dq, w_dp;
+#ifdef DDP_CONV_STAMPS
+  ConvStampBuf stamps;
+#endif
 };
 
 __device__ __forceinline__ uint2 acc_old4(const unsigned short* dx, const unsigned short* acc_dy,
@@ -216,12 +214,13 @@
   int wp[CB], wq[CB];
   int w_rr = 0, w_ss = 0, w_lim = 0;
   const bool wsame = MODE == MODE_WGRAD && gg.stride == 1 && gg.P == gg.H && gg.Q == gg.W;
-  const int w_dq = wsame ? BK % gg.Q : 0;
-  const int w_dp = wsame ? (BK / gg.Q) % gg.P : 0;
+  const int w_dq = args.w_dq;
+  const int w_dp = args.w_dp;
   const int w_dm = wsame ? 2 * BK * gg.C : 0;
   const bool pm = MODE == MODE_WGRAD && args.pixmajor;
   const bool pmr = MODE != MODE_WGRAD && args.pixmajor;
   int pmr_pq = 0, pmr_n0 = 0, pmr_row0 = 0, pmr_t = 0;
+  int pmr_pp = 0, pmr_qq = 0;
   unsigned pmr_mask = 0;
   int pm_p = 0, pm_q = 0, pm_qlo = 0, pm_qhi = 0, pm_n0 = 0, pm_r = 0, pm_s = 0;
   int row0 = 0, col0 = 0, zsplit = 0, ks_begin = 0, ks_end = 0, cur_tile = 0;
@@ -238,10 +237,10 @@
   const __amdgpu_buffer_rsrc_t rsB = make_rsrc(args.b, args.b_bytes);
 
   auto setup = [&](int item) {
-    zsplit = item / tiles;
+    zsplit = fast_div(item, args.dTiles);
     const int tile = xcd_remap(item - zsplit * tiles, tiles);
     cur_tile = tile;
-    const int tm = tile / tiles_n;
+    const int tm = fast_div(tile, args.dTilesN);
     const int tn = tile - tm * tiles_n;
     row0 = tm * BM;
     col0 = tn * BN;
@@ -249,9 +248,11 @@
     ks_end = min(ksteps, ks_begin + args.ksteps_per_split);
     if (MODE != MODE_WGRAD) {
       if (pmr) {
-        pmr_pq = row0 / gg.N;
+        pmr_pq = fast_div(row0, args.dN);
         pmr_n0 = row0 - pmr_pq * gg.N;
         pmr_row0 = row0;
+        pmr_pp = fast_div(pmr_pq, args.dQ);
+        pmr_qq = pmr_pq - pmr_pp * gg.Q;
         const int img = MODE == MODE_FWD ? gg.H * gg.W * gg.C : gg.P * gg.Q * gg.K;
 #pragma unroll
         for (int i = 0; i < CA; ++i) a_off[i] = 2 * (((tid >> 3) + 32 * i) * img + lcA * 8);
@@ -267,7 +268,7 @@
         }
       }
       if (MODE == MODE_FWD && args.d2x2) {
-        d2pos = col0 / args.d2K;
+        d2pos = fast_div(col0, args.dD2K);
 #pragma unroll
         for (int i = 0; i < CB; ++i) {
           const int col = col0 + (tid >> 3) + 32 * i;
@@ -281,7 +282,7 @@
           b_off[i] = col < args.Ng ? 2 * (col * args.Kg + lcB * 8) : (int)kOOB;
         }
       } else if (args.d2x2) {
-        d2pos = col0 / args.d2C;
+        d2pos = fast_div(col0, args.dD2C);
 #pragma unroll
         for (int i = 0; i < CB; ++i) {
           const int col = col0 + (lcB ^ swz_row_step<BN>(i)) * 8;
@@ -298,7 +299,7 @@
         }
       }
       if (pmr) {
-        const int pp = pmr_pq / gg.Q, qq = pmr_pq - pp * gg.Q, kb = cdim / BK;
+        const int pp = pmr_pp, qq = pmr_qq, kb = cdim / BK;
         unsigned m = 0;
         for (int r = 0; r < gg.R; ++r)
           for (int s2 = 0; s2 < gg.S; ++s2) {
@@ -309,21 +310,22 @@
           }
         pmr_mask = m;
         const int V = __builtin_popcount(m) * kb;
-        const int per = (V + args.splits - 1) / args.splits;
+        const int per = fast_div(V + args.splits - 1, args.dSplits);
         ks_begin = min(V, zsplit * per);
         ks_end = min(V, ks_begin + per);
-        int jv = ks_begin / kb;
+        const int jv0 = fast_div(ks_begin, args.dKb);
+        int jv = jv0;
         unsigned mm = m;
         for (; jv > 0 && mm; --jv) mm &= mm - 1;
         pmr_t = mm ? __builtin_ctz(mm) : 0;
-        kc = (ks_begin - (ks_begin / kb) * kb) * BK;
-        kr = pmr_t / gg.S;
+        kc = (ks_begin - jv0 * kb) * BK;
+        kr = fast_div(pmr_t, args.dS);
         ks_ = pmr_t - kr * gg.S;
       } else {
         const int kk = ks_begin * BK + (fast ? 0 : lcA * 8);
-        const int rs = kk / cdim;
+        const int rs = fast_div(kk, args.dCdim);
         kc = kk - rs * cdim;
-        kr = rs / Sdec;
+        kr = fast_div(rs, args.dSdec);
         ks_ = rs - kr * Sdec;
       }
     } else {
@@ -334,14 +336,14 @@
         a_off[i] = kout < args.Mg ? 2 * (((tid + i * 256) / NCA) * gg.K + kout) : (int)kOOB;
       }
       const int j = col0 + lcB * 8;
-      const int rs = j / gg.C;
+      const int rs = fast_div(j, args.dC);
       xk.c = j - rs * gg.C;
-      xk.r = rs / gg.S;
+      xk.r = fast_div(rs, args.dS);
       xk.s = rs - xk.r * gg.S;
       xk.ok = j < args.Ng;
       if (pm) {
-        const int t = col0 / gg.C;
-        pm_r = t / gg.S;
+        const int t = fast_div(col0, args.dC);
+        pm_r = fast_div(t, args.dS);
         pm_s = t - pm_r * gg.S;
         const int PQ = gg.P * gg.Q, nb = gg.N / BK;
         const int p_lo = max(0, gg.pad - pm_r), p_hi = min(gg.P, gg.H + gg.pad - pm_r);
@@ -349,12 +351,13 @@
         pm_qhi = min(gg.Q, gg.W + gg.pad - pm_s);
         const int nq = max(0, pm_qhi - pm_qlo);
         const int V = max(0, p_hi - p_lo) * nq * nb;
-        const int per = (V + args.splits - 1) / args.splits;
+        const int per = fast_div(V + args.splits - 1, args.dSplits);
         ks_begin = min(V, zsplit * per);
         ks_end = min(V, ks_begin + per);
-        const int jv = ks_begin / nb;
-        pm_p = p_lo + (nq ? jv / nq : 0);
-        pm_q = pm_qlo + (nq ? jv - (jv / nq) * nq : 0);
+        const int jv = fast_div(ks_begin, args.dNb);
+        const int jp = nq ? jv / nq : 0;
+        pm_p = p_lo + jp;
+        pm_q = pm_qlo + (nq ? jv - jp * nq : 0);
         pm_n0 = (ks_begin - jv * nb) * BK;
         constexpr int NCA = BM / 8;
         constexpr int NCB = BN / 8;
@@ -378,8 +381,8 @@
 #pragma unroll
         for (int i = 0; i < CB; ++i) {
           const int m = ks_begin * BK + (tid + i * 256) / NCB;
-          const int rem = m % pq;
-          wp[i] = rem / gg.Q;
+          const int rem = m - fast_div(m, args.dPQ) * pq;
+          wp[i] = fast_div(rem, args.dQ);
           wq[i] = rem - wp[i] * gg.Q;
           b_off[i] = m * (2 * gg.C) + xk_same;
         }
@@ -392,7 +395,7 @@
     unsigned short* Bs = As + TILE_A;
     const int k0 = ks * BK;
     if (MODE != MODE_WGRAD && pmr) {
-      const int pp = pmr_pq / gg.Q, qq = pmr_pq - pp * gg.Q;
+      const int pp = pmr_pp, qq = pmr_qq;
       const int hh = MODE == MODE_FWD ? pp + kr - gg.pad : pp - kr + gg.pad;
       const int ww = MODE == MODE_FWD ? qq + ks_ - gg.pad : qq - ks_ + gg.pad;
       const int sa = MODE == MODE_FWD ? 2 * (((pmr_n0 * gg.H + hh) * gg.W + ww) * cdim + kc)
@@ -408,7 +411,7 @@
         kc = 0;
         const unsigned rest = pmr_mask & ~((2u << pmr_t) - 1u);
         pmr_t = rest ? __builtin_ctz(rest) : pmr_t;
-        kr = pmr_t / gg.S;
+        kr = fast_div(pmr_t, args.dS);
         ks_ = pmr_t - kr * gg.S;
       }
     } else if (MODE != MODE_WGRAD) {
@@ -426,7 +429,7 @@
         }
         int boff;
         if (args.d2x2) {
-          const int pix = MODE == MODE_FWD ? kc / args.d2C : kc / args.d2K;
+          const int pix = fast_div(kc, MODE == MODE_FWD ? args.dD2C : args.dD2K);
           const int ch = kc - pix * (MODE == MODE_FWD ? args.d2C : args.d2K);
           const int pq = MODE == MODE_FWD ? d2pos : pix, hw = MODE == MODE_FWD ? pix : d2pos;
           const int tap = ((hw >> 1) - (pq >> 1) + 1) * 3 + ((hw & 1) - (pq & 1) + 1);
@@ -467,8 +470,8 @@
           for (int i = 0; i < CB; ++i) {
             const int m = (tid + i * 256) / (BN / 8);
             const int kkr = k0 + m;
-            const int tap = kkr / gg.K, kout = kkr - tap * gg.K;
-            const int tr = tap / Sdec, ts = tap - tr * Sdec;
+            const int tap = fast_div(kkr, args.dCdim), kout = kkr - tap * gg.K;
+            const int tr = fast_div(tap, args.dSdec), ts = tap - tr * Sdec;
             const int rr = phase ? args.r0 + gg.stride * tr : tr, ss = phase ? args.s0 + gg.stride * ts : ts;
             const int off = b_off[i] - 2 * m * RSC + 2 * ((kout * gg.R * gg.S + rr * gg.S + ss) * gg.C);
             dma_buf(rsB, (kkr < args.Kg && b_off[i] != (int)kOOB) ? off : (int)kOOB,
@@ -841,8 +844,41 @@
     }
     int wrs = 0, wc = 0;
     if (MODE == MODE_WGRAD) {
-      wrs = col / g.C;
+      wrs = fast_div(col, args.dC);
       wc = col - wrs * g.C;
+    }
+    if (MODE == MODE_WGRAD && !split && g.wkrsc && g.Creal == g.C) {
+      const bool sgd = SGDM && args.sgd.p;
+      float* const pb = sgd ? args.sgd.p : args.dw;
+      size_t e[TM];
+      bool ok[TM];
+      float4 pv[TM], bv[TM];
+#pragma unroll
+      for (int i = 0; i < TM; ++i) {
+        const int row = row0 + wm * WTM + i * 16 + rl;
+        ok[i] = cok && row < args.Mg;
+        e[i] = ((size_t)row * g.R * g.S + wrs) * g.C + wc;
+        if (!ok[i]) continue;
+        pv[i] = *reinterpret_cast<const float4*>(pb + e[i]);
+        if (sgd) bv[i] = *reinterpret_cast<const float4*>(args.sgd.buf + e[i]);
+      }
+#pragma unroll
+      for (int i = 0; i < TM; ++i) {
+        if (!ok[i]) continue;
+        const f32x4 v = acc[i][j];
+        if (sgd) {
+          const SgdFuse& h = args.sgd;
+          pv[i].x = sgd_update1(pv[i].x, v[0], bv[i].x, sgd_lr, h.momentum, h.wd, h.grad_scale, h.nesterov);
+          pv[i].y = sgd_update1(pv[i].y, v[1], bv[i].y, sgd_lr, h.momentum, h.wd, h.grad_scale, h.nesterov);
+          pv[i].z = sgd_update1(pv[i].z, v[2], bv[i].z, sgd_lr, h.momentum, h.wd, h.grad_scale, h.nesterov);
+          pv[i].w = sgd_update1(pv[i].w, v[3], bv[i].w, sgd_lr, h.momentum, h.wd, h.grad_scale, h.nesterov);
+          *reinterpret_cast<float4*>(args.sgd.buf + e[i]) = bv[i];
+        } else {
+          pv[i].x += v[0]; pv[i].y += v[1]; pv[i].z += v[2]; pv[i].w += v[3];
+        }
+        *reinterpret_cast<float4*>(pb + e[i]) = pv[i];
+      }
+      continue;
     }
 #pragma unroll
     for (int i = 0; i < TM; ++i) {
@@ -850,30 +886,12 @@
       if (!cok || row >= args.Mg) continue;
       const f32x4 v = acc[i][j];
       if (MODE == MODE_WGRAD && !split) {
-        if (SGDM && g.wkrsc && g.Creal == g.C && args.sgd.p) {
-          const size_t e = ((size_t)row * g.R * g.S + wrs) * g.C + wc;
-          float4 pv = *reinterpret_cast<const float4*>(args.sgd.p + e);
-          float4 bv = *reinterpret_cast<const float4*>(args.sgd.buf + e);
-          const SgdFuse& h = args.sgd;
-          pv.x = sgd_update1(pv.x, v[0], bv.x, sgd_lr, h.momentum, h.wd, h.grad_scale, h.nesterov);
-          pv.y = sgd_update1(pv.y, v[1], bv.y, sgd_lr, h.momentum, h.wd, h.grad_scale, h.nesterov);
-          pv.z = sgd_update1(pv.z, v[2], bv.z, sgd_lr, h.momentum, h.wd, h.grad_scale, h.nesterov);
-          pv.w = sgd_update1(pv.w, v[3], bv.w, sgd_lr, h.momentum, h.wd, h.grad_scale, h.nesterov);
-          *reinterpret_cast<float4*>(args.sgd.p + e) = pv;
-          *reinterpret_cast<float4*>(args.sgd.buf + e) = bv;
-        } else if (g.wkrsc && g.Creal == g.C) {
-          float* d = args.dw + ((size_t)row * g.R * g.S + wrs) * g.C + wc;
-          float4 o = *reinterpret_cast<float4*>(d);
-          o.x += v[0]; o.y += v[1]; o.z += v[2]; o.w += v[3];
-          *reinterpret_cast<float4*>(d) = o;
-        } else {
-#pragma unroll
-          for (int t = 0; t < 4; ++t) {
-            if (wc + t >= g.Creal) break;
-            const size_t di = g.wkrsc ? ((size_t)row * g.R * g.S + wrs) * g.Creal + wc + t
-                                      : ((size_t)row * g.Creal + wc + t) * g.R * g.S + wrs;
-            args.dw[di] += v[t];
-          }
+#pragma unroll
+        for (int t = 0; t < 4; ++t) {
+          if (wc + t >= g.Creal) break;
+          const size_t di = g.wkrsc ? ((size_t)row * g.R * g.S + wrs) * g.Creal + wc + t
+                                    : ((size_t)row * g.Creal + wc + t) * g.R * g.S + wrs;
+          args.dw[di] += v[t];
         }
       } else if (split) {
         const size_t srow = pmr ? (size_t)(pmr_n0 + row - pmr_row0) * (g.P * g.Q) + pmr_pq : (size_t)row;
@@ -987,7 +1005,13 @@
 
   constexpr int DMA = CA + CB;
   for (int item = bid; item < nitems; item += nblk) {
+#ifdef DDP_CONV_STAMPS
+    const unsigned long long st0 = stamp_now();
+#endif
     setup(item);
+#ifdef DDP_CONV_STAMPS
+    const unsigned long long st1 = stamp_now();
+#endif
 #pragma unroll
     for (int i = 0; i < TM; ++i)
 #pragma unroll
@@ -1010,7 +1034,13 @@
       mma(fa1, fb1);
       stage = stage + 1 == NST ? 0 : stage + 1;
     }
+#ifdef DDP_CONV_STAMPS
+    const unsigned long long st2 = stamp_now();
+#endif
     epilogue(row0, col0, zsplit, args.splits > 1);
+#ifdef DDP_CONV_STAMPS
+    stamp_put(args.stamps, (unsigned)MODE, st0, st1, st2, stamp_now());
+#endif
     if (item + nblk < nitems) wait_dma_barrier<0>();
   }
   if constexpr (XSTAT) {
@@ -1697,14 +1727,14 @@
 
 using namespace ddp_amd;
 
-static FastDiv make_fastdiv(int d) {
-  FastDiv f;
-  int sh = 0;
-  while ((1ll << sh) < d) ++sh;
-  f.sh = sh;
-  f.mul = (unsigned)((((1ull << sh) - (unsigned long long)d) << 32) / (unsigned long long)d + 1);
-  return f;
-}
+#ifdef DDP_CONV_STAMPS
+namespace ddp_amd {
+ConvStampBuf g_conv_stamps{nullptr, 0};
+}
+extern "C" void ddp_conv_stamps_set(void* buf, int cap) {
+  g_conv_stamps = ConvStampBuf{(unsigned*)buf, buf ? std::max(0, cap) : 0};
+}
+#endif
 
 static bool fits_buffer(size_t elems) { return elems * 2 < (size_t)kOOB; }
 
@@ -1829,6 +1859,28 @@
     a.dPQ = make_fastdiv(std::max(1, a.g.P * a.g.Q));
     a.dQ = make_fastdiv(std::max(1, a.g.Q));
   }
+  {
+    const ConvGeom& g = a.g;
+    const int cdim = MODE == MODE_FWD ? g.C : g.K;
+    const bool wsame = MODE == MODE_WGRAD && g.stride == 1 && g.P == g.H && g.Q == g.W;
+    a.dTiles = make_fastdiv(std::max(1, tiles));
+    a.dTilesN = make_fastdiv(std::max(1, (a.Ng + BN - 1) / BN));
+    a.dN = make_fastdiv(std::max(1, g.N));
+    a.dCdim = make_fastdiv(std::max(1, cdim));
+    a.dKb = make_fastdiv(std::max(1, cdim / BK));
+    a.dSdec = make_fastdiv(std::max(1, MODE == MODE_DGRAD && a.phase ? a.St : g.S));
+    a.dS = make_fastdiv(std::max(1, g.S));
+    a.dC = make_fastdiv(std::max(1, g.C));
+    a.dNb = make_fastdiv(std::max(1, g.N / BK));
+    a.dD2C = make_fastdiv(std::max(1, a.d2C));
+    a.dD2K = make_fastdiv(std::max(1, a.d2K));
+    a.dSplits = make_fastdiv(splits);
+    a.w_dq = wsame ? BK % g.Q : 0;
+    a.w_dp = wsame ? (BK / g.Q) % g.P : 0;
+  }
+#ifdef DDP_CONV_STAMPS
+  a.stamps = g_conv_stamps;
+#endif
   return tiles * splits;
 }
 
@@ -2032,20 +2084,23 @@
 
 constexpr int kNumTiles = 8;
 
+static const int kTileBN[kNumTiles] = {128, 64, 128, 64, 64, 256, 128, 256};
 template <int MODE>
-static bool tile_ok(int tile) {
+static bool tile_ok(int tile, const ConvArgs& a) {
+  if (tile < 0 || tile >= kNumTiles) return false;
   if (MODE == MODE_WGRAD && (tile == 5 || tile == 7)) return false;
-  return tile >= 0 && tile < kNumTiles;
+  if (MODE != MODE_WGRAD && a.d2x2 && (MODE == MODE_FWD ? a.d2K : a.d2C) % kTileBN[tile]) return false;
+  return true;
 }
 
 template <int MODE>
 static void plan_mode(ConvArgs& a, size_t ws_elems, int* best_out, int* sp, int* nst_out) {
   const double c[4] = {tile_cost(128, 128, a, ws_elems, &sp[0]), tile_cost(128, 64, a, ws_elems, &sp[1]),
                        tile_cost(64, 128, a, ws_elems, &sp[2]), tile_cost(64, 64, a, ws_elems, &sp[3])};
-  int best = 0, nst = g_force_stages;
-  for (int i = 1; i < 4; ++i)
-    if (c[i] < c[best]) best = i;
-  if (g_force_tile >= 1 && g_force_tile <= kNumTiles && tile_ok<MODE>(g_force_tile - 1)) {
+  int best = 3, nst = g_force_stages;
+  for (int i = 2; i >= 0; --i)
+    if (tile_ok<MODE>(i, a) && c[i] <= c[best]) best = i;
+  if (g_force_tile >= 1 && g_force_tile <= kNumTiles && tile_ok<MODE>(g_force_tile - 1, a)) {
     best = g_force_tile - 1;
     if (best >= 4) {
       static const int bmn[4][2] = {{256, 64}, {64, 256}, {256, 128}, {128, 256}};
@@ -2053,7 +2108,7 @@
     }
   } else if (a.splits <= 0) {
     auto it = g_tuned.find(TuneKey{MODE, a.Mg, a.Ng, a.Kg});
-    if (it != g_tuned.end() && tile_ok<MODE>(it->second.tile)) {
+    if (it != g_tuned.end() && tile_ok<MODE>(it->second.tile, a)) {
       const size_t slab = (size_t)a.Mg * a.Ng;
       const int ksteps = (a.Kg + 63) / 64;
       int spl = std::max(1, std::min(it->second.splits, ksteps));
diff --git a/distributed-data-parallel-ml-training_amd/csrc/kernels/conv_tr.hip b/distributed-data-parallel-ml-training_amd/csrc/kernels/conv_tr.hip
--- a/distributed-data-parallel-ml-training_amd/csrc/kernels/conv_tr.hip
+++ b/distributed-data-parallel-ml-training_amd/csrc/kernels/conv_tr.hip
@@ -69,6 +69,10 @@
   float* in_coef;
   unsigned short* y_out;
   int z_bytes;
+  FastDiv dTiles, dTilesN, dBands, dPw, dW, dPerImg;
+#ifdef DDP_CONV_STAMPS
+  ConvStampBuf stamps;
+#endif
 };
 
 template <int BM, int BN, int NST, int NL, int IN>
@@ -95,19 +99,23 @@
   const int wm = wid >> 1, wn = wid & 1;
   const int W = a.W, H = a.H, C = a.C, K = a.K;
   const int M = a.N * H * W;
+#ifdef DDP_CONV_STAMPS
+  const unsigned long long st0 = stamp_now();
+#endif
   const int ncb = C / 64;
 
   const int tiles = a.tiles_m * a.tiles_n;
   const int item = blockIdx.x;
-  const int sp = item / tiles;
+  const int sp = fast_div(item, a.dTiles);
   const int tile = xcd_remap(item - sp * tiles, tiles);
-  const int tm = tile / a.tiles_n;
+  const int tm = fast_div(tile, a.dTilesN);
   const int tn = tile - tm * a.tiles_n;
   const int row0 = tm * BM, col0 = tn * BN;
   const int cb0 = sp * a.cbps, cb1 = min(ncb, cb0 + a.cbps);
   const int nsteps = (cb1 - cb0) * 9;
-  const int n0 = (tm / a.bands) * a.imgs;
-  const int h0 = (tm % a.bands) * a.rows;
+  const int tband = fast_div(tm, a.dBands);
+  const int n0 = tband * a.imgs;
+  const int h0 = (tm - tband * a.bands) * a.rows;
 
   const __amdgpu_buffer_rsrc_t rsA = IN ? make_rsrc(a.zin, a.z_bytes) : make_rsrc(a.x, a.x_bytes);
   if (BNIN) {
@@ -151,8 +159,8 @@
       unsigned off = kOOB;
       int dst = -1, yd = -1;
       if (px < npix) {
-        const int img = px / pw, loc = px - img * pw;
-        const int hr = loc / W, wc = loc - hr * W;
+        const int img = fast_div(px, a.dPw), loc = px - img * pw;
+        const int hr = fast_div(loc, a.dW), wc = loc - hr * W;
         const int h = h0 + hr - 1;
         if (h >= 0 && h < H) {
           const int n = n0 + img;
@@ -245,8 +253,8 @@
   for (int i = 0; i < TM; ++i) {
     const int m = wm * WTM + i * 16 + (lane & 15);
     const int per_img = a.rows * W;
-    const int img = m / per_img, rem = m - img * per_img;
-    const int rr = rem / W, cc = rem - rr * W;
+    const int img = fast_div(m, a.dPerImg), rem = m - img * per_img;
+    const int rr = fast_div(rem, a.dW), cc = rem - rr * W;
     const int pix = img * a.imgp + rr * W + cc;
     fa_base[i] = (plane_base(lane >> 4, a.plane) + pix) * 16;
     col_ok[i] = (cc >= 1 ? 1u : 0u) | (cc <= W - 2 ? 2u : 0u);
@@ -287,6 +295,9 @@
     }
   };
 
+#ifdef DDP_CONV_STAMPS
+  const unsigned long long st1 = stamp_now();
+#endif
   load_a(cb0);
 #pragma unroll
   for (int s = 0; s < NST - 1; ++s)
@@ -312,6 +323,12 @@
     }
   }
 
+#ifdef DDP_CONV_STAMPS
+  const unsigned long long st2 = stamp_now();
+#define DDP_TR_STAMP_END() stamp_put(a.stamps, 3u, st0, st1, st2, stamp_now())
+#else
+#define DDP_TR_STAMP_END() ((void)0)
+#endif
   const int rl = lane & 15, cq = 4 * (lane >> 4);
   const int cbase = col0 + wn * WTN + cq;
   if (a.splits > 1) {
@@ -328,6 +345,7 @@
         *reinterpret_cast<float4*>(slab + (size_t)row * K + col) = (float4){v[0], v[1], v[2], v[3]};
       }
     }
+    DDP_TR_STAMP_END();
     return;
   }
   const bool red = a.stats != nullptr;
@@ -371,7 +389,10 @@
       }
     }
   }
-  if (!red) return;
+  if (!red) {
+    DDP_TR_STAMP_END();
+    return;
+  }
   __syncthreads();
   if (wm == 0 && rl == 0) {
     float* st = a.stats + stat_rep(blockIdx.x) * 2 * K;
@@ -388,6 +409,7 @@
       }
     }
   }
+  DDP_TR_STAMP_END();
 }
 
 struct Geo {
@@ -639,6 +661,12 @@
   a.abuf_elems = geo.abuf;
   a.tiles_m = (int)(M / c.bm);
   a.tiles_n = K / c.bn;
+  a.dTiles = make_fastdiv(std::max(1, a.tiles_m * a.tiles_n));
+  a.dTilesN = make_fastdiv(std::max(1, a.tiles_n));
+  a.dBands = make_fastdiv(std::max(1, geo.bands));
+  a.dPw = make_fastdiv((geo.rows + 2) * W);
+  a.dW = make_fastdiv(W);
+  a.dPerImg = make_fastdiv(geo.rows * W);
   if (in) {
     a.zin = (const unsigned short*)in->z;
     a.in_stats = in->stats;
@@ -650,6 +678,9 @@
     a.y_out = (unsigned short*)in->y;
     a.z_bytes = (int)(2 * M * C * (in->pool ? 4 : 1));
   }
+#ifdef DDP_CONV_STAMPS
+  a.stamps = g_conv_stamps;
+#endif
   const int items = a.tiles_m * a.tiles_n * pl.splits;
   if (!launch_stages(c, in_mode, a, geo.nl, items, st)) return 0;
   int e = (int)hipGetLastError();
```

After: 371,700 images/s, median of 6. 1.8% higher.
